# yongduosui/CAL

Hardware: AMD Instinct MI355X
Metric: graphs/sec (train step) on SPMotif b=0.9 batch=128 (higher is better)
Workload: dtype f32; 1 GPU; spmotif_b0.9_causalgcn_h128_l3_bs128; model=CausalGCN, batch_per_gpu=128, global_batch=128, hidden=128, layers=3, node_num=7, launch=graph(8 steps per graph launch, remainder 3), parallelism=dp1, resident_batches=8

## Files before the change

cal_amd/csrc/engine.hip:

```cpp
#include <string.h>
#include <hip/hip_ext.h>

#include <algorithm>
#include <type_traits>
#include <vector>

#include "engine_kernels.hpp"
#include "engine_readout.hpp"
#include "engine_gconv.hpp"
#include "engine_gconv_bwd.hpp"
#include "engine_ggat.hpp"
#include "engine_plan.hpp"
#include "engine_attbwd.hpp"
#include "engine_ro_step.hpp"
#include "engine_gin.hpp"
#include "engine_ggin.hpp"
#include "engine_feat.hpp"
#include "engine_gwide.hpp"
#include "engine_attwide.hpp"

namespace cal {

constexpr int MAX_LAYERS = 6;
constexpr int MAX_SLABS = 24;
constexpr int MAX_COMMITS = 64;

struct FinishArgs {
    SlabTask st[MAX_SLABS];
    CommitTask ct[MAX_COMMITS];
    int nst, nct;
    float* stats;
    float wc, wo, wco;
    float* tick;
    float* ticked;
    unsigned long long* perm_ctr;
    AdamArgs adam;
    AdamRange ar[MAX_ADAM_RANGES];
    int nar;
    double* bn0z; int bn0z_n;
    int* dirty;
    int* host_status;
    const int* status;
    int blk0[MAX_SLABS + MAX_COMMITS + MAX_ADAM_RANGES + 1];
};
__global__ void __launch_bounds__(256) k_finish(const FinishArgs fa, float* __restrict__ grad) {
    int task = 0;
    const int ntask = fa.nst + fa.nct + fa.nar;
    AdamArgs A = fa.adam;
    float adam_t = 0.f, adam_lr = 0.f;
    const bool flagged = fa.status && (fa.status[0] | fa.status[1]) != 0;
    if (fa.ticked && flagged && blockIdx.x == 0 && threadIdx.x == 0) fa.ticked[0] -= 1.f;
    if (A.on && flagged) A.on = 0;
    if (A.on) { adam_t = A.step[0]; adam_lr = A.lr[0]; }
    while (task + 1 < ntask && (int)blockIdx.x >= fa.blk0[task + 1]) ++task;
    const int bx = blockIdx.x - fa.blk0[task], nbx = fa.blk0[task + 1] - fa.blk0[task];
    if (fa.stats && blockIdx.x == 0 && threadIdx.x == 0)
        fa.stats[0] = fa.wc * fa.stats[1] + fa.wo * fa.stats[2] + fa.wco * fa.stats[3];
    if (fa.tick && !flagged && blockIdx.x == 0 && threadIdx.x == 0) fa.tick[0] += 1.f;
    if (fa.perm_ctr && blockIdx.x == 0 && threadIdx.x == 0) fa.perm_ctr[0] += 1;
    if (fa.bn0z && blockIdx.x == 0) {
        for (int i = threadIdx.x; i < fa.bn0z_n; i += 256) fa.bn0z[i] = 0.0;
        if (threadIdx.x == 0) *fa.dirty = 0;
    }
    if (fa.host_status && fa.status && blockIdx.x == 0 && threadIdx.x == 0)
        __hip_atomic_store(fa.host_status, fa.status[0] | fa.status[1], __ATOMIC_RELAXED, __HIP_MEMORY_SCOPE_SYSTEM);
    if (task < fa.nst) {
        const SlabTask t = fa.st[task];
        __shared__ float sred[256];
        const int el = threadIdx.x & 63, grp = threadIdx.x >> 6;
        const int per = (t.S + 3) / 4, z_lo = grp * per, z_hi = min(t.S, z_lo + per);
        for (int i0 = bx * 64; i0 < t.n; i0 += nbx * 64) {
            const int i = min(i0 + el, t.n - 1);
            float s0 = 0.f, s1 = 0.f;
            for (int z0 = z_lo; z0 < z_hi; z0 += 8) {
                float v[8];
#pragma unroll
                for (int u = 0; u < 8; ++u) v[u] = t.slabs[(size_t)max(min(z0 + u, z_hi - 1), 0) * t.n + i];
#pragma unroll
                for (int u = 0; u < 8; ++u) asm volatile("" : "+v"(v[u]));
#pragma unroll
                for (int u = 0; u < 8; u += 2) {
                    s0 += z0 + u < z_hi ? v[u] : 0.f;
                    s1 += z0 + u + 1 < z_hi ? v[u + 1] : 0.f;
                }
            }
            sred[threadIdx.x] = s0 + s1;
            __syncthreads();
            if (grp == 0 && i0 + el < t.n) {
                const float gsum = (sred[el] + sred[64 + el]) + (sred[128 + el] + sred[192 + el]);
                t.dst[i] = gsum;
                if (A.on) adam_update(A, (t.dst - grad) + i, gsum, adam_t, adam_lr);
            }
            __syncthreads();
        }
    } else if (task - fa.nst < fa.nct) {
        const CommitTask t = fa.ct[task - fa.nst];
        __shared__ double red[256];
        const int pl = threadIdx.x >> 4, cl = threadIdx.x & 15;
        for (int c0 = bx * 16; c0 < t.n; c0 += nbx * 16) {
            const int c = c0 + cl, cc = min(c, t.n - 1);
            double sacc = 0.0;
            for (int q0 = pl; q0 < t.P; q0 += 16 * 8) {
                double v[8];
#pragma unroll
                for (int u = 0; u < 8; ++u) v[u] = t.src[(size_t)max(min(q0 + 16 * u, t.P - 1), 0) * t.stride + cc];
#pragma unroll
                for (int u = 0; u < 8; ++u) asm volatile("" : "+v"(v[u]));
#pragma unroll
                for (int u = 0; u < 8; ++u) sacc += q0 + 16 * u < t.P ? v[u] : 0.0;
            }
            red[threadIdx.x] = sacc;
            __syncthreads();
            if (pl == 0 && c < t.n) {
                double tot = 0.0;
#pragma unroll
                for (int k = 0; k < 16; ++k) tot += red[k * 16 + cl];
                const float gv = t.scale * (float)tot;
                grad[t.dst + c] = gv;
                if (A.on) adam_update(A, t.dst + c, gv, adam_t, adam_lr);
            }
            __syncthreads();
        }
    } else if (A.on) {
        const AdamRange r = fa.ar[task - fa.nst - fa.nct];
        const int64_t i = r.begin + (int64_t)bx * 256 + threadIdx.x;
        if (i < r.end) adam_update(A, i, grad[i], adam_t, adam_lr);
    }
}

struct BNSlot { int gamma, beta; int width; float* rm; float* rv; int64_t* nbt; int arena; };

struct Engine {
    int F, H, C, L;
    int cat;
    int no_node_att, no_edge_att;
    int gin;
    int o_gin_w2[MAX_LAYERS], o_gin_b2[MAX_LAYERS];
    float *gagg, *gt1, *gy, *ones;
    float loop_w;
    float *P, *G, *M1, *M2, *step, *lr;
    int64_t nparam;
    float beta1, beta2, eps, wd;
    unsigned long long perm_seed; unsigned long long* perm_ctr;
    int64_t* perm_dev;
    P2PArgs p2p; int p2p_on;
    int num_cus;
    int* host_status;
    int* p2p_host_status;
    int p2p_max_polls;
    float grad_scale;
    int o_feat_w;
    int o_conv_w[MAX_LAYERS], o_conv_b[MAX_LAYERS];
    int o_eatt_w, o_eatt_b, o_natt_w, o_natt_b;
    int o_cw, o_cb, o_ow, o_ob;
    int o_fc1_w[3], o_fc1_b[3], o_fc2_w[3], o_fc2_b[3];
    BNSlot bn[MAX_LAYERS + 9];
    int nbn;
    int a_convb[MAX_LAYERS], a_cb, a_ob, a_dwn, a_dwe, a_db1, a_db2, a_sync, arena_n, bn_plane;
    char* ws; size_t ws_bytes;
    int64_t capN, capE, capB;
    float *h, *z, *zco, *hco, *anode, *pq, *att, *dis_unit, *dis_co, *pooled, *pcnt, *xco, *y1, *zl, *logp, *stats, *zpart;
    int adam_fused;
    int ro_rows;
    int striped;
    int fold_zero;
    int bn0_dirty_host;
    int gwide;
    int ro_step;
    float *dzl, *dyh1, *dy1, *dxh, *dpool, *dZco, *gn, *gself, *ddeg, *dl, *dzco, *dXhco, *dZ, *dzi, *dXh, *slabs;
    size_t slab_floats;
    double* arena;
    double* parts; size_t parts_doubles;
    hipStream_t side; hipEvent_t ev_fork[24], ev_join[24];
    int *rowptr_dst, *nbr_dst, *eid_dst, *rowptr_src, *nbr_src, *eid_src, *row32, *col32, *work, *status, *gptr, *iperm, *eptr;
    float* wslot;
    float* coef_src;
    float* coef;
    int max_nodes, max_edges;
    const int64_t *node_ptr, *edge_ptr;
    const int64_t* tile_gptr; int ntiles;
    int K; float gat_p, gat_slope;
    uint64_t gat_seed[MAX_LAYERS];
    unsigned long long* gat_ctr;
    int o_conv_att[MAX_LAYERS];
    float *gz, *gsc, *gws;
};

static size_t al(size_t n) { return (n + 63) / 64 * 64; }

}

using namespace cal;

namespace cal {
int gat_forward(const int32_t* rowptr_dst, const int32_t* nbr_dst, const int32_t* eid_dst, const float* z,
                const float* att, const float* bias, int relu, float slope, float p, uint64_t seed, const uint64_t* ctr,
                float* out, float* adst, float* asrc, float* mx, float* den, int64_t N, int64_t E,
                int64_t K, int64_t D, hipStream_t stream);
int gat_backward(const int32_t* rowptr_dst, const int32_t* nbr_dst, const int32_t* eid_dst,
                 const int32_t* rowptr_src, const int32_t* nbr_src, const int32_t* eid_src, const float* z,
                 const float* att, const float* adst, const float* asrc, const float* mx, const float* den,
                 const float* gout, float slope, float p, uint64_t seed, const uint64_t* ctr, float* dz, float* datt,
                 float* ws, int64_t N, int64_t E, int64_t K, int64_t D, hipStream_t stream, float* part_out, int* nparts);
int gat_datt_parts(int64_t N);
int plan_build(const int64_t* edge_index, int64_t E, int64_t N, int32_t* rowptr_dst, int32_t* nbr_dst, int32_t* eid_dst,
               int32_t* rowptr_src, int32_t* nbr_src, int32_t* eid_src, int32_t* row32, int32_t* col32, int32_t* work,
               int32_t* status, bool prezeroed, hipStream_t stream);
int plan_rank(int64_t E, int64_t N, const int32_t* rowptr_dst, int32_t* nbr_dst, int32_t* eid_dst, const int32_t* rowptr_src,
              int32_t* nbr_src, int32_t* eid_src, const int32_t* row32, const int32_t* col32, const int32_t* scratch,
              hipStream_t stream);
}

extern "C" int64_t cal_gat_bwd_ws(int64_t N, int64_t E, int64_t K, int64_t D);

CAL_EXPORT void* cal_engine_create(int64_t F, int64_t H, int64_t C, int64_t L) {
    if (H % 4 != 0 || H > 256 || H < 4 || L < 0 || L > MAX_LAYERS || F < 1 || C < 1 || C > 64) {
        set_error("cal_engine_create: unsupported shape (need hidden %% 4 == 0, hidden <= 256, layers <= %d, classes <= 64)", MAX_LAYERS);
        return nullptr;
    }
    Engine* e = new Engine();
    memset(e, 0, sizeof(Engine));
    if (hipHostMalloc((void**)&e->host_status, 64, hipHostMallocMapped | hipHostMallocCoherent) == hipSuccess) *e->host_status = 0;
    else { (void)hipGetLastError(); e->host_status = nullptr; }
    { const char* v = getenv("CAL_AMD_RO_STEP"); e->ro_step = !(v && v[0] == '0'); }
    { const char* v = getenv("CAL_AMD_RO_ROWS"); e->ro_rows = !(v && v[0] == '0'); }
    { const char* v = getenv("CAL_AMD_STRIPED"); e->striped = !(v && v[0] == '0'); }
    { const char* v = getenv("CAL_AMD_GWIDE"); e->gwide = !(v && v[0] == '0'); }
    { const char* v = getenv("CAL_AMD_FOLD_ZERO"); e->fold_zero = !(v && v[0] == '0'); }
    e->bn0_dirty_host = 1;
    {
        int dev = 0, cus = 0;
        if (hipGetDevice(&dev) != hipSuccess || hipDeviceGetAttribute(&cus, hipDeviceAttributeMultiprocessorCount, dev) != hipSuccess) cus = 0;
        if (cus < 3 * ((int)H / RO_CW) + 8) e->ro_step = 0;
        e->num_cus = cus > 0 ? cus : 256;
        if (cus < 3 * ((int)H / RO_CW) * RBK_MAXRB + 8) e->ro_rows = 0;
    }
    { const char* v = getenv("CAL_AMD_ADAM_FUSED"); e->adam_fused = !(v && v[0] == '0'); }
    e->F = (int)F; e->H = (int)H; e->C = (int)C; e->L = (int)L;
    e->loop_w = 1.f;
    e->grad_scale = 1.f;
    e->p2p_max_polls = 1 << 22;
    e->nbn = (int)L + 9;
    if (hipStreamCreateWithFlags(&e->side, hipStreamNonBlocking) != hipSuccess) { set_error("cal_engine_create: side stream"); delete e; return nullptr; }
    for (int i = 0; i < 24; ++i) {
        hipEventCreateWithFlags(&e->ev_fork[i], hipEventDisableTiming);
        hipEventCreateWithFlags(&e->ev_join[i], hipEventDisableTiming);
    }
    return e;
}

CAL_EXPORT void cal_engine_destroy(void* h) {
    Engine* e = (Engine*)h;
    if (!e) return;
    for (int i = 0; i < 24; ++i) { hipEventDestroy(e->ev_fork[i]); hipEventDestroy(e->ev_join[i]); }
    hipStreamDestroy(e->side);
    if (e->p2p_host_status) hipHostFree(e->p2p_host_status);
    if (e->host_status) hipHostFree(e->host_status);
    delete e;
}

CAL_EXPORT int64_t cal_engine_num_param_slots(void* h) { Engine* e = (Engine*)h; return 3 + (e->gin ? 6 : 4) * e->L + 12 + 24; }
CAL_EXPORT int64_t cal_engine_num_bn(void* h) { return ((Engine*)h)->nbn; }

CAL_EXPORT int cal_engine_bind(void* h, float* P, float* G, float* M1, float* M2, float* step, float* lr,
                               int64_t nparam, const int64_t* offs, const int64_t* bn_ptrs, float beta1, float beta2,
                               float eps, float weight_decay) {
    Engine* e = (Engine*)h;
    e->P = P; e->G = G; e->M1 = M1; e->M2 = M2; e->step = step; e->lr = lr; e->nparam = nparam;
    e->beta1 = beta1; e->beta2 = beta2; e->eps = eps; e->wd = weight_decay;
    const int L = e->L, H = e->H, F = e->F, C = e->C;
    int s = 0;
    int bn_g[MAX_LAYERS + 9], bn_b[MAX_LAYERS + 9], bn_w[MAX_LAYERS + 9];
    int k = 0;
    bn_g[k] = (int)offs[s++]; bn_b[k] = (int)offs[s++]; bn_w[k] = F; ++k;
    e->o_feat_w = (int)offs[s++];
    for (int i = 0; i < L; ++i) {
        bn_g[k] = (int)offs[s++]; bn_b[k] = (int)offs[s++]; bn_w[k] = H; ++k;
        e->o_conv_w[i] = (int)offs[s++]; e->o_conv_b[i] = (int)offs[s++];
        if (e->gin) { e->o_gin_w2[i] = (int)offs[s++]; e->o_gin_b2[i] = (int)offs[s++]; }
    }
    e->o_eatt_w = (int)offs[s++]; e->o_eatt_b = (int)offs[s++];
    e->o_natt_w = (int)offs[s++]; e->o_natt_b = (int)offs[s++];
    bn_g[k] = (int)offs[s++]; bn_b[k] = (int)offs[s++]; bn_w[k] = H; ++k;
    bn_g[k] = (int)offs[s++]; bn_b[k] = (int)offs[s++]; bn_w[k] = H; ++k;
    e->o_cw = (int)offs[s++]; e->o_cb = (int)offs[s++];
    e->o_ow = (int)offs[s++]; e->o_ob = (int)offs[s++];
    for (int hd = 0; hd < 3; ++hd) {
        bn_g[k] = (int)offs[s++]; bn_b[k] = (int)offs[s++]; bn_w[k] = (hd == 2 && e->cat) ? 2 * H : H; ++k;
        e->o_fc1_w[hd] = (int)offs[s++]; e->o_fc1_b[hd] = (int)offs[s++];
        bn_g[k] = (int)offs[s++]; bn_b[k] = (int)offs[s++]; bn_w[k] = H; ++k;
        e->o_fc2_w[hd] = (int)offs[s++]; e->o_fc2_b[hd] = (int)offs[s++];
    }
    int a = 0;
    for (int i = 0; i < L; ++i) { e->a_convb[i] = a; a += H; }
    e->a_cb = a; a += H;
    e->a_ob = a; a += H;
    e->a_dwn = a; a += H + 4;
    e->a_dwe = a; a += 2 * H + 4;
    e->a_db1 = a; a += 3 * H;
    e->a_db2 = a; a += (3 * C + 3) / 4 * 4;
    e->a_sync = a; a += (RBK_SYNC_INTS + 1) / 2 + 2;
    a = (a + 3) / 4 * 4;
    const int a_bn = a;
    for (int i = 0; i < e->nbn; ++i) {
        BNSlot& b = e->bn[i];
        b.gamma = bn_g[i]; b.beta = bn_b[i]; b.width = bn_w[i];
        b.rm = (float*)bn_ptrs[3 * i]; b.rv = (float*)bn_ptrs[3 * i + 1]; b.nbt = (int64_t*)bn_ptrs[3 * i + 2];
        b.arena = a;
        a += 4 * ((b.width + 3) / 4 * 4);
    }
    e->bn_plane = a - a_bn;
    a = a_bn + NSTRIPE * e->bn_plane;
    e->arena_n = a;
    (void)C;
    return 0;
}

static size_t engine_layout(Engine* e, int64_t N, int64_t E, int64_t B, bool assign) {
    const size_t H = e->H, C = e->C, L = e->L, F = e->F;
    size_t off = 0;
    auto F32 = [&](float*& p, size_t n) { if (assign) p = (float*)(e->ws) + off; off += al(n); };
    auto I32 = [&](int*& p, size_t n) { if (assign) p = (int*)(e->ws) + off; off += al(n); };
    F32(e->h, (L + 1) * N * H); F32(e->z, N * H); F32(e->zco, 2 * N * H); F32(e->hco, 2 * N * H);
    F32(e->anode, 2 * N); F32(e->pq, 4 * N); F32(e->att, 2 * E); F32(e->dis_unit, N); F32(e->dis_co, 2 * N);
    F32(e->pooled, 2 * B * H); F32(e->pcnt, 2 * B * H); F32(e->xco, 2 * B * H); F32(e->y1, 3 * B * H); F32(e->zl, 3 * B * C); F32(e->logp, 3 * B * C);
    F32(e->stats, 8); F32(e->zpart, 3 * ((H + 15) / 16) * B * C);
    F32(e->dzl, 3 * B * C); F32(e->dyh1, 3 * B * H); F32(e->dy1, 3 * B * H); F32(e->dxh, 4 * B * H); F32(e->dpool, 2 * B * H);
    F32(e->dZco, 2 * N * H); F32(e->gn, 4 * E); F32(e->gself, 4 * N); F32(e->ddeg, 2 * N); F32(e->dl, E);
    F32(e->dzco, 2 * N * H); F32(e->dXhco, 2 * N * H); F32(e->dZ, N * H); F32(e->dzi, (L > 0 ? L : 1) * N * H); F32(e->dXh, N * H);
    size_t slab = 0;
    auto slab_of = [&](size_t M, size_t Nn) {
        const size_t big = gemm_wres_grad((int)M, (int)Nn, (int)N) ? (size_t)gemm_wres_grad_splits((int)N, 1) * M * Nn
                         : gemm_big_grad((int)M, (int)Nn, (int)N) ? (size_t)gemm_big_grad_splits((int)N) * M * Nn : 0;
        return std::max<size_t>(std::max<size_t>(512 * 64 * 64, (size_t)B * M * Nn), big) + 2 * M * Nn;
    };
    slab += slab_of(F, H) + (L + 2) * slab_of(H, H) + 2 * slab_of(H, H) + slab_of(H, 2 * H) + 3 * slab_of(C, H);
    if (e->gin) slab += L * slab_of(H, H);
    if (e->K > 0) slab += L * (size_t)1024 * H;
    if (assign) e->slab_floats = slab;
    F32(e->slabs, slab);
    {
        float* tmp = nullptr;
        F32(tmp, 2 * (size_t)e->arena_n);
        if (assign) e->arena = (double*)tmp;
        size_t pcap = std::max<size_t>((N + 15) / 16 + 1, (std::min<int64_t>(N, 16384) + 7) / 8 + 1);
        size_t pd = pcap * (size_t)H * 2 * (3 * L + 20);
        F32(tmp, 2 * pd);
        if (assign) { e->parts = (double*)tmp; e->parts_doubles = pd; }
    }
    I32(e->rowptr_dst, N + 1); I32(e->nbr_dst, E); I32(e->eid_dst, E);
    I32(e->rowptr_src, N + 1); I32(e->nbr_src, E); I32(e->eid_src, E);
    I32(e->row32, E); I32(e->col32, E); I32(e->work, 4 * (N + 1) + 4 * E); I32(e->status, 4); I32(e->gptr, B + 1);
    I32(e->iperm, B);
    { int* tmp = nullptr; I32(tmp, 2 * B + 2); if (assign) e->perm_dev = (int64_t*)tmp; }
    I32(e->eptr, B + 1);
    F32(e->coef, 3 * E);
    F32(e->coef_src, E);
    F32(e->wslot, 2 * E);
    if (e->gin) {
        const size_t Lg = L > 0 ? L : 1;
        F32(e->gagg, Lg * N * H); F32(e->gt1, Lg * N * H); F32(e->gy, Lg * N * H); F32(e->ones, N);
    }
    if (e->K > 0) {
        const size_t K = e->K;
        F32(e->gz, (L > 0 ? L : 1) * N * H); F32(e->gsc, (L > 0 ? L : 1) * 4 * al(N * K));
        F32(e->gws, (size_t)cal_gat_bwd_ws(N, E, K, H / K));
    }
    return off * 4;
}

CAL_EXPORT int cal_engine_set_gat(void* h, int64_t heads, float p, float slope, const int64_t* att_offs,
                                  const uint64_t* seeds, void* ctr) {
    Engine* e = (Engine*)h;
    CAL_REQUIRE(heads > 0 && e->H % heads == 0, "heads must divide hidden");
    const int64_t D = e->H / heads;
    CAL_REQUIRE(D % 4 == 0 && ((D / 4) & (D / 4 - 1)) == 0, "head dim must be 4 * a power of two");
    CAL_REQUIRE(p >= 0.f && p < 1.f, "dropout p must be in [0,1)");
    e->K = (int)heads; e->gat_p = p; e->gat_slope = slope; e->gat_ctr = (unsigned long long*)ctr;
    for (int i = 0; i < e->L; ++i) { e->o_conv_att[i] = (int)att_offs[i]; e->gat_seed[i] = seeds[i]; }
    return 0;
}

CAL_EXPORT int64_t cal_engine_workspace_bytes(void* h, int64_t N, int64_t E, int64_t B) {
    return (int64_t)engine_layout((Engine*)h, N, E, B, false) + 256;
}

CAL_EXPORT int cal_engine_set_workspace(void* h, void* ws, int64_t bytes, int64_t capN, int64_t capE, int64_t capB) {
    Engine* e = (Engine*)h;
    CAL_REQUIRE(((uintptr_t)ws & 255) == 0, "workspace must be 256-byte aligned");
    e->ws = (char*)ws;
    e->capN = capN; e->capE = capE; e->capB = capB;
    size_t need = engine_layout(e, capN, capE, capB, true);
    CAL_REQUIRE((int64_t)need <= bytes, "workspace too small");
    e->ws_bytes = bytes;
    e->bn0_dirty_host = 1;
    return 0;
}

CAL_EXPORT int64_t cal_engine_buffer_offset(void* h, const char* name) {
    Engine* e = (Engine*)h;
    struct { const char* n; void* p; } tab[] = {
        {"h", e->h}, {"z", e->z}, {"zco", e->zco}, {"hco", e->hco}, {"anode", e->anode}, {"pq", e->pq}, {"att", e->att},
        {"dis_unit", e->dis_unit}, {"dis_co", e->dis_co}, {"pooled", e->pooled}, {"xco", e->xco}, {"y1", e->y1},
        {"zl", e->zl}, {"logp", e->logp}, {"stats", e->stats}, {"dzl", e->dzl}, {"dyh1", e->dyh1}, {"dy1", e->dy1},
        {"dxh", e->dxh}, {"dpool", e->dpool}, {"dZco", e->dZco}, {"gn", e->gn}, {"gself", e->gself}, {"ddeg", e->ddeg},
        {"dl", e->dl}, {"dzco", e->dzco}, {"dXhco", e->dXhco}, {"dZ", e->dZ}, {"dzi", e->dzi}, {"dXh", e->dXh},
        {"arena", e->arena}, {"gptr", e->gptr}, {"status", e->status}, {"eptr", e->eptr},
        {"gt1", e->gin ? e->gt1 : nullptr}, {"gy", e->gin ? e->gy : nullptr},
        {"rowptr_dst", e->rowptr_dst}, {"nbr_dst", e->nbr_dst}, {"eid_dst", e->eid_dst},
        {"rowptr_src", e->rowptr_src}, {"nbr_src", e->nbr_src}, {"eid_src", e->eid_src}, {"perm", e->perm_dev}, {"ones", e->ones},
    };
    for (auto& t : tab)
        if (!strcmp(t.n, name)) return t.p ? ((char*)t.p - e->ws) / 4 : -1;
    return -1;
}

namespace {

enum class Plan { Node, Graph256, Graph1024, Big };
enum class Conv { Node, Graph64, Graph128, Wide };
enum class Att { Node, Graph, Wide };
enum class FeatFwd { Gemm, Rows };
enum class FeatBwd { Gemm, Rows, Units };
enum class Readout { Gemm, FourKernel, OneLaunch, Rows };
struct Route {
    Plan plan;
    bool plan_stats;
    bool plan_coef;
    FeatFwd feat_fwd;
    FeatBwd feat_bwd;
    bool feat_chunks;
    Conv bb_fwd, bb_bwd;
    int gw_cols_bb, gw_cols_co;
    int nsplit_bb, nsplit_co;
    bool lean_bb, lean_co;
    Att att_fwd, att_bwd;
    int ag_split;
    Conv co_fwd, co_bwd;
    Readout ro;
    bool st_feat;
    bool st_bb;
    bool st_bb1;
    bool st_co;
    bool st_node;
};

struct Ctx {
    Engine* e;
    hipStream_t st;
    int N, B;
    const int64_t* batch;
    int T;
    int64_t E;
    int training;
    int rpb_n, rpb_b;
    int nfork;
    const int64_t* y; const int64_t* perm; float wc, wo, wco; int want_grad;
    int draw_perm;
    int tick_in_finish;
    int adam_in_finish;
    size_t parts_off;
    FinalArgs fin;
    Route r;
};

struct Deferred { double* p; int P; int stride; };
struct Bwd {
    FinishArgs fa;
    size_t slab_off;
    Deferred d_convb[MAX_LAYERS], d_gin_b1[MAX_LAYERS], d_cb, d_ob, d_dwn, d_dwe, d_bn0;
};

BNRef bnref(const Ctx& c, int k, int rows, int update) {
    const Engine* e = c.e;
    const BNSlot& b = e->bn[k];
    BNRef r;
    const int wp = (b.width + 3) / 4 * 4;
    r.sum = e->arena + b.arena; r.sq = e->arena + b.arena + wp;
    r.gamma = e->P + b.gamma; r.beta = e->P + b.beta;
    r.inv_n = 1.0 / (double)rows; r.eps = 1e-5f;
    r.run_mean = b.rm; r.run_var = b.rv; r.nbt = b.nbt;
    r.unbias = rows > 1 ? (float)rows / (float)(rows - 1) : 1.f;
    r.update = (update && c.training) ? 1 : 0;
    r.use_running = c.training ? 0 : 1;
    r.ss = e->bn_plane;
    return r;
}
double* bn_stsum(const Ctx& c, int k) { return c.e->arena + c.e->bn[k].arena; }
double* bn_stsq(const Ctx& c, int k) { return c.e->arena + c.e->bn[k].arena + (c.e->bn[k].width + 3) / 4 * 4; }
double* bn_dsum(const Ctx& c, int k) { return c.e->arena + c.e->bn[k].arena + 2 * ((c.e->bn[k].width + 3) / 4 * 4); }
double* bn_dprod(const Ctx& c, int k) { return c.e->arena + c.e->bn[k].arena + 3 * ((c.e->bn[k].width + 3) / 4 * 4); }

double* parts_alloc(Ctx& c, size_t n) {
    n = (n + 1) & ~(size_t)1;
    if (c.parts_off + n > c.e->parts_doubles) return nullptr;
    double* p = c.e->parts + c.parts_off;
    c.parts_off += n;
    return p;
}
void final_task(Ctx& c, const double* parts, int P, int stride, int n, double* dst) {
    c.fin.t[c.fin.nt++] = FinalTask{parts, P, stride, n, dst};
}
int flush_finals(Ctx& c) {
    if (c.fin.nt == 0) return 0;
    int nmax = 0;
    for (int i = 0; i < c.fin.nt; ++i) nmax = std::max(nmax, c.fin.t[i].n);
    hipLaunchKernelGGL(k_stats_final, dim3(cdiv(nmax, 8), c.fin.nt), dim3(256), 0, c.st, c.fin);
    c.fin.nt = 0;
    cal::g_last_launch = "k_stats_final";
    hipError_t e_ = hipGetLastError();
    if (e_ != hipSuccess) { set_error("k_stats_final: %s", hipGetErrorString(e_)); return 1; }
    return 0;
}
int spmm_rpb(int H, bool stats, int N = 1 << 30) {
    const int rows = 256 / group_for(H, 4);
    return stats && N > 16384 ? std::min(8, std::max(2, N / (rows * 4096))) * rows : rows;
}
Acc spmm_acc(Ctx& c, double* dst, int cols, int rpb) {
    const int P = cdiv(c.N, rpb);
    double* p = parts_alloc(c, (size_t)P * cols);
    if (!p) return Acc(dst);
    final_task(c, p, P, cols, cols, dst);
    return Acc(dst, p, cols);
}

Acc node_acc(Ctx& c, double* dst, int cols) {
    const int P = cdiv(c.N, c.rpb_n);
    if ((size_t)P * cols <= 4096) return Acc(dst);
    double* p = parts_alloc(c, (size_t)P * cols);
    if (!p) return Acc(dst);
    final_task(c, p, P, cols, cols, dst);
    return Acc(dst, p, cols);
}
bool use_ks(int M) { return M <= 2048; }
int fwd_gemm(Ctx& c, bool transB, const GemmArgs& a, int nbatch) {
    return use_ks(a.M) ? launch_gemm_ks(transB, a, nbatch, c.st) : launch_gemm(false, transB, a, nbatch, c.st);
}
void gemm_stats(Ctx& c, GemmProb& pr, int M, int N, double* d0, double* d1, bool dot, int K = 0, bool st = false) {
    if (dot) { pr.dot_sum = d0; pr.dot_prod = d1; } else { pr.st_sum = d0; pr.st_sq = d1; }
    if (st && (use_ks(M) || (!gemm_wres_rows(M, N, K) && !gemm_big_rows(M, K)))) { pr.st_ss = c.e->bn_plane; return; }
    const int P = use_ks(M) ? gemm_ks_row_tiles(M) : gemm_row_tiles(M, N, K);
    if ((size_t)P * N * 2 <= 4096) return;
    double* p = parts_alloc(c, (size_t)P * 2 * N);
    if (!p) return;
    pr.parts = p;
    final_task(c, p, P, 2 * N, N, d0);
    final_task(c, p + N, P, 2 * N, N, d1);
}

GemmArgs gemm_args(int M, int N, int K, bool transA, bool transB, int relu) {
    GemmArgs a;
    memset(&a, 0, sizeof(a));
    a.M = M; a.N = N; a.K = K;
    a.lda = transA ? M : K; a.ldb = transB ? K : N; a.ldc = N;
    a.relu = relu;
    gemm_set_split(a, 1);
    return a;
}

template <typename F>
int with_g(int H, F f) {
    int g = group_for(H, 4);
    if (g <= 8) return f(std::integral_constant<int, 8>());
    if (g == 16) return f(std::integral_constant<int, 16>());
    if (g == 32) return f(std::integral_constant<int, 32>());
    return f(std::integral_constant<int, 64>());
}

int pow2ceil(int v) { int p = 1; while (p < v) p <<= 1; return p; }

int launch_espmm(hipStream_t st, const CSR& csr, const SpmmBranch2& bb, int nbranch, int relu, float loop_w, int N, int H, int rpb);

#define RC(x) do { int rc_ = (x); if (rc_) return rc_; } while (0)
int no_parts() { set_error("engine: partial-row workspace exhausted"); return 2; }
int no_slabs() { set_error("engine: slab workspace exhausted"); return 2; }
float* slab_take(Ctx& c, Bwd& b, size_t need, float* dst, int n, int S) {
    if (b.slab_off + need > c.e->slab_floats || b.fa.nst >= MAX_SLABS) return nullptr;
    float* p = c.e->slabs + b.slab_off;
    b.fa.st[b.fa.nst++] = SlabTask{p, dst, n, S};
    b.slab_off += need;
    return p;
}
Acc defer(Ctx& c, Deferred& d, int P, int cols) {
    d.p = parts_alloc(c, (size_t)P * cols); d.P = P; d.stride = cols;
    return d.p ? Acc(nullptr, d.p, cols) : Acc();
}
int grad_slabs(Ctx& c, Bwd& b, GemmArgs& a, int nbatch, float** dst) {
    gemm_set_split(a, splitk_for(a.M, a.N, a.K, nbatch));
    for (int q = 0; q < nbatch; ++q) {
        a.p[q].C = a.nsplit > 1 ? slab_take(c, b, (size_t)a.nsplit * a.M * a.N, dst[q], a.M * a.N, a.nsplit) : dst[q];
        if (!a.p[q].C) return no_slabs();
    }
    return 0;
}
int grad_gemm(Ctx& c, Bwd& b, GemmArgs& a, int nbatch, float** dst) {
    RC(grad_slabs(c, b, a, nbatch, dst));
    hipStream_t s = c.st;
    constexpr bool kForkWeightGrads = false;
    if (kForkWeightGrads && c.nfork < 24) {
        hipEventRecord(c.e->ev_fork[c.nfork], c.st);
        hipStreamWaitEvent(c.e->side, c.e->ev_fork[c.nfork], 0);
        s = c.e->side;
    }
    int rc = launch_gemm(true, false, a, nbatch, s);
    if (s != c.st) { hipEventRecord(c.e->ev_join[c.nfork], s); c.nfork++; }
    return rc;
}
void join_side(Ctx& c) {
    for (int i = 0; i < c.nfork; ++i) hipStreamWaitEvent(c.st, c.e->ev_join[i], 0);
    c.nfork = 0;
}

int dual_gemm(Ctx& c, Bwd& b, GemmArgs& ax, int nbx, GemmArgs& aw, int nbw, float** dst) {
    if (use_ks(ax.M)) {
        RC(grad_gemm(c, b, aw, nbw, dst));
        return fwd_gemm(c, true, ax, nbx);
    }
    RC(grad_slabs(c, b, aw, nbw, dst));
    return launch_gemm_dual(ax, nbx, aw, nbw, c.st);
}

struct ProfRec { hipEvent_t e0, e1; int cls; double work; };
static bool g_prof_on = false;
static std::vector<ProfRec> g_prof;
struct ProfScope;
static ProfScope* g_prof_cur = nullptr;
struct ProfScope {
    hipStream_t st; bool on, single, used; ProfRec r;
    ProfScope(hipStream_t s, int cls, double work, bool single_kernel = false) : st(s), on(g_prof_on), single(single_kernel), used(false) {
        if (!on) return;
        r.cls = cls; r.work = work;
        hipEventCreate(&r.e0); hipEventCreate(&r.e1);
        if (single) g_prof_cur = this; else hipEventRecord(r.e0, st);
    }
    ~ProfScope() {
        if (!on) return;
        if (single) { g_prof_cur = nullptr; if (used) g_prof.push_back(r); }
        else { hipEventRecord(r.e1, st); g_prof.push_back(r); }
    }
};
#define PROF_LAUNCH(kernel, grid, block, shmem, stream, ...) do { \
        if (g_prof_cur) { hipExtLaunchKernelGGL(kernel, grid, block, shmem, stream, g_prof_cur->r.e0, g_prof_cur->r.e1, 0, __VA_ARGS__); g_prof_cur->used = true; } \
        else hipLaunchKernelGGL(kernel, grid, block, shmem, stream, __VA_ARGS__); } while (0)

int launch_espmm(hipStream_t st, const CSR& csr, const SpmmBranch2& bb, int nbranch, int relu, float loop_w, int N, int H, int rpb) {
    const bool wt = bb.b[0].w != nullptr, stt = bb.b[0].st_sum.on(), sd = bb.b[0].sd_z != nullptr;
    if (wt != (bb.b[nbranch - 1].w != nullptr) || stt != bb.b[nbranch - 1].st_sum.on() || sd != (bb.b[nbranch - 1].sd_z != nullptr) || rpb % 4 != 0 || H > 256) {
        set_error("k_espmm: branches differ in kind"); return 2;
    }
    const dim3 grid(cdiv(N, rpb), nbranch);
    if (sd) {
        if (!wt || stt) { set_error("k_espmm: the fused SDDMM is built for the weighted branches without statistics"); return 2; }
        const bool pb = bb.b[0].pb_g != nullptr;
        if (pb != (bb.b[nbranch - 1].pb_g != nullptr)) { set_error("k_espmm: branches differ in kind"); return 2; }
        return with_g(H, [&](auto g) {
            constexpr int G = decltype(g)::value;
            if (pb) PROF_LAUNCH((k_espmm<4, G, true, false, true, true>), grid, dim3(256), 0, st, csr, bb, relu, loop_w, N, H, rpb);
            else PROF_LAUNCH((k_espmm<4, G, true, false, true>), grid, dim3(256), 0, st, csr, bb, relu, loop_w, N, H, rpb);
            return 0;
        });
    }
    return with_g(H, [&](auto g) {
        constexpr int G = decltype(g)::value;
        if (wt && stt) PROF_LAUNCH((k_espmm<4, G, true, true>), grid, dim3(256), 0, st, csr, bb, relu, loop_w, N, H, rpb);
        else if (wt) PROF_LAUNCH((k_espmm<4, G, true, false>), grid, dim3(256), 0, st, csr, bb, relu, loop_w, N, H, rpb);
        else if (stt) PROF_LAUNCH((k_espmm<4, G, false, true>), grid, dim3(256), 0, st, csr, bb, relu, loop_w, N, H, rpb);
        else PROF_LAUNCH((k_espmm<4, G, false, false>), grid, dim3(256), 0, st, csr, bb, relu, loop_w, N, H, rpb);
        return 0;
    });
}

Acc graph_acc(Ctx& c, double* dst, int cols, bool st = false) {
    if (st) return Acc(dst, nullptr, c.e->bn_plane);
    double* p = parts_alloc(c, (size_t)c.T * cols);
    if (!p) return Acc(dst);
    final_task(c, p, c.T, cols, cols, dst);
    return Acc(dst, p, cols);
}
CSR csr_dst(const Ctx& c) { return CSR{c.e->rowptr_dst, c.e->nbr_dst, c.e->eid_dst, (int)c.E}; }
CSR csr_src(const Ctx& c) { return CSR{c.e->rowptr_src, c.e->nbr_src, c.e->eid_src, (int)c.E}; }

template <typename Args>
int bn_bwd_sums(Ctx& c, Args& a, int P, double* dsum, double* dprod, bool st) {
    if (st) { a.dacc_sum = dsum; a.dacc_prod = dprod; a.dacc_ss = c.e->bn_plane; return 0; }
    const int H = c.e->H;
    double* p = parts_alloc(c, (size_t)P * 2 * H);
    if (!p) return no_parts();
    a.dot_parts = p;
    final_task(c, p, P, 2 * H, H, dsum);
    final_task(c, p + H, P, 2 * H, H, dprod);
    return 0;
}

int gconv_bwd(Ctx& c, Bwd& b, GconvBwdBranch* gb, int nb, float** dst, double** dsum, double** dprod, bool st) {
    Engine* e = c.e;
    const bool co = nb == 2;
    const bool wide = (co ? c.r.co_bwd : c.r.bb_bwd) == Conv::Wide;
    const int nsplit = co ? c.r.nsplit_co : c.r.nsplit_bb;
    const bool lean = co ? c.r.lean_co : c.r.lean_bb;
    const int H = e->H, B = c.T, nsl = H / GC_N;
    const int np2 = nsplit == 4 ? 2 : 1;
    for (int k = 0; k < nb; ++k) {
        gb[k].batch = c.batch; gb[k].tile_gptr = e->ntiles > 0 ? e->tile_gptr : nullptr;
        gb[k].slab = slab_take(c, b, (size_t)B * H * H, dst[k], H * H, B);
        if (!gb[k].slab) return no_slabs();
        RC(bn_bwd_sums(c, gb[k], B * nsl * np2, dsum[k], dprod[k], st));
    }
    const GconvBwdBranch2 b2{{gb[0], gb[nb - 1]}};
    if (wide) {
        const CSR gs = csr_src(c);
        const dim3 gridw(B, nsl * nsplit, nb);
        if (co) PROF_LAUNCH((k_gw_bwd<true, 2>), gridw, dim3(GW_NT), 0, c.st, gs, e->gptr, e->eptr, b2, e->loop_w, c.N, H, H, nsplit, e->status);
        else if (gb[0].dout) PROF_LAUNCH((k_gw_bwd<false, 0>), gridw, dim3(GW_NT), 0, c.st, gs, e->gptr, e->eptr, b2, e->loop_w, c.N, H, H, nsplit, e->status);
        else PROF_LAUNCH((k_gw_bwd<false, 1>), gridw, dim3(GW_NT), 0, c.st, gs, e->gptr, e->eptr, b2, e->loop_w, c.N, H, H, nsplit, e->status);
        CAL_CHECK_LAUNCH("k_gw_bwd");
        return 0;
    }
    const CSR gd = csr_dst(c);
    const dim3 grid(B, nsl, nb);
    if (co && lean && e->ntiles > 0) PROF_LAUNCH((k_gconv_bwd<true, 2, true, true>), grid, dim3(GB_NT), 0, c.st, gd, e->gptr, e->eptr, b2, e->loop_w, c.N, H, H, e->status);
    else if (co && lean) PROF_LAUNCH((k_gconv_bwd<true, 2, false, true>), grid, dim3(GB_NT), 0, c.st, gd, e->gptr, e->eptr, b2, e->loop_w, c.N, H, H, e->status);
    else if (co && e->ntiles > 0) PROF_LAUNCH((k_gconv_bwd<true, 2, true>), grid, dim3(GB_NT), 0, c.st, gd, e->gptr, e->eptr, b2, e->loop_w, c.N, H, H, e->status);
    else if (co) PROF_LAUNCH((k_gconv_bwd<true, 2>), grid, dim3(GB_NT), 0, c.st, gd, e->gptr, e->eptr, b2, e->loop_w, c.N, H, H, e->status);
    else if (gb[0].dout && lean) PROF_LAUNCH((k_gconv_bwd<false, 0, false, true>), grid, dim3(GB_NT), 0, c.st, gd, e->gptr, e->eptr, b2, e->loop_w, c.N, H, H, e->status);
    else if (gb[0].dout) PROF_LAUNCH((k_gconv_bwd<false, 0>), grid, dim3(GB_NT), 0, c.st, gd, e->gptr, e->eptr, b2, e->loop_w, c.N, H, H, e->status);
    else if (lean) PROF_LAUNCH((k_gconv_bwd<false, 1, false, true>), grid, dim3(GB_NT), 0, c.st, gd, e->gptr, e->eptr, b2, e->loop_w, c.N, H, H, e->status);
    else PROF_LAUNCH((k_gconv_bwd<false, 1>), grid, dim3(GB_NT), 0, c.st, gd, e->gptr, e->eptr, b2, e->loop_w, c.N, H, H, e->status);
    CAL_CHECK_LAUNCH("k_gconv_bwd");
    return 0;
}

RoArgs make_ro(const Ctx& c) {
    Engine* e = c.e;
    const int L = e->L, H = e->H, C = e->C, B = c.B;
    RoArgs a;
    memset(&a, 0, sizeof(a));
    for (int hd = 0; hd < 3; ++hd) {
        RoHead& h = a.h[hd];
        const int k1 = L + 3 + 2 * hd, k2 = L + 4 + 2 * hd;
        h.W1 = e->P + e->o_fc1_w[hd]; h.b1 = e->P + e->o_fc1_b[hd];
        h.W2 = e->P + e->o_fc2_w[hd]; h.b2 = e->P + e->o_fc2_b[hd];
        h.bn1 = bnref(c, k1, B, 1); h.bn2 = bnref(c, k2, B, 1);
        h.st2_sum = bn_stsum(c, k2); h.st2_sq = bn_stsq(c, k2);
        h.d1_sum = bn_dsum(c, k1); h.d1_prod = bn_dprod(c, k1);
        h.d2_sum = bn_dsum(c, k2); h.d2_prod = bn_dprod(c, k2);
        h.db1 = e->arena + e->a_db1 + hd * H; h.db2 = e->arena + e->a_db2 + hd * C;
        h.gW1 = e->G + e->o_fc1_w[hd]; h.gW2 = e->G + e->o_fc2_w[hd];
    }
    a.pooled = e->pooled; a.perm = c.perm; a.iperm = e->iperm; a.xco = e->xco; a.y1 = e->y1;
    a.zl = e->zl; a.logp = e->logp; a.dzl = e->dzl; a.dy1 = e->dy1; a.dxin = e->dxh;
    a.rowloss = e->dyh1;
    a.y = c.y; a.stats = e->stats; a.B = B; a.H = H; a.C = C;
    a.wc = c.wc; a.wo = c.wo; a.wco = c.wco; a.training = c.training; a.want_grad = c.want_grad;
    return a;
}

static int g_stop_after = 0;
static int g_stage = 0;
static std::vector<const char*> g_stage_names;
#define STAGE() do { if (g_stop_after == 0) g_stage_names.push_back(cal::g_last_launch); \
                     if (g_stop_after > 0 && ++g_stage >= g_stop_after) return -12345; } while (0)

int gin_rows(Ctx& c, int mode, const GinRowArgs& ga) {
    const int N = c.N, H = c.e->H;
    hipStream_t st = c.st;
    return with_g(H, [&](auto g) {
        constexpr int G = decltype(g)::value;
        const dim3 grid(cdiv(N, c.rpb_n));
        if (mode == 0) hipLaunchKernelGGL((k_gin_rows<4, G, 0>), grid, dim3(256), 0, st, ga, N, H, c.rpb_n);
        else if (mode == 1) hipLaunchKernelGGL((k_gin_rows<4, G, 1>), grid, dim3(256), 0, st, ga, N, H, c.rpb_n);
        else if (mode == 2) hipLaunchKernelGGL((k_gin_rows<4, G, 2>), grid, dim3(256), 0, st, ga, N, H, c.rpb_n);
        else hipLaunchKernelGGL((k_gin_rows<4, G, 3>), grid, dim3(256), 0, st, ga, N, H, c.rpb_n);
        return 0;
    });
}

template <typename Fn>
int with_g_fp(int H, int F, Fn f) {
    return with_g(H, [&](auto g) {
        constexpr int G = decltype(g)::value;
        if constexpr (G >= FEAT_FMAX) {
            if (F <= 4) return f(g, std::integral_constant<int, 4>());
            if (F <= 8) return f(g, std::integral_constant<int, 8>());
            if (F <= 12) return f(g, std::integral_constant<int, 12>());
            return f(g, std::integral_constant<int, 16>());
        } else {
            set_error("feature row kernels: hidden width too small"); return 2;
        }
    });
}

int pool2_slices(int N, int B) { return std::max(1, std::min(32, N / std::max(1, B * 128))); }
int launch_pool2(hipStream_t st, const float* hc, const float* ho, const int* gptr, float* pooled, float* cnt, float* slices,
                 int N, int B, int H) {
    const int tc = std::min(256, pow2ceil(H / 4));
    const int S = pool2_slices(N, B);
    hipLaunchKernelGGL((k_pool2<4>), dim3(B, 2, S), dim3(256), 0, st, hc, ho, gptr, pooled, pooled + (size_t)B * H, H, tc, slices, cnt);
    CAL_CHECK_LAUNCH("k_pool2");
    if (S > 1) {
        hipLaunchKernelGGL(k_pool2_sum, dim3(cdiv(4 * (int64_t)B * H, 256)), dim3(256), 0, st, slices, S, 2 * (int64_t)B * H, pooled, cnt);
        CAL_CHECK_LAUNCH("k_pool2_sum");
    }
    return 0;
}
int launch_pool2(Ctx& c) {
    Engine* e = c.e;
    const size_t NH = (size_t)c.N * e->H;
    return launch_pool2(c.st, e->hco, e->hco + NH, e->gptr, e->pooled, e->pcnt, e->dZco, (int)c.N, (int)c.B, e->H);
}
int launch_pool_cnt(hipStream_t st, const float* hc, const float* ho, const int64_t* batch, float* cnt, int N, int B, int H, int rpb_n) {
    hipLaunchKernelGGL(k_zero_f32, dim3(cdiv(2 * (int64_t)B * H, 256)), dim3(256), 0, st, cnt, 2 * (int64_t)B * H);
    CAL_CHECK_LAUNCH("k_zero_f32");
    return with_g(H, [&](auto g) {
        constexpr int G = decltype(g)::value;
        hipLaunchKernelGGL((k_pool_cnt<4, G>), dim3(cdiv(N, rpb_n), 2), dim3(256), 0, st, hc, ho, batch, cnt, N, B, H, rpb_n);
        CAL_CHECK_LAUNCH("k_pool_cnt");
        return 0;
    });
}
int launch_pool_cnt(Ctx& c) {
    Engine* e = c.e;
    const size_t NH = (size_t)c.N * e->H;
    return launch_pool_cnt(c.st, e->hco, e->hco + NH, c.batch, e->pcnt, (int)c.N, (int)c.B, e->H, c.rpb_n);
}

Route make_route(const Ctx& c, bool want_grad) {
    const Engine* e = c.e;
    const int N = c.N, B = c.B, T = c.T, H = e->H, F = e->F, C = e->C, L = e->L, mn = e->max_nodes, me = e->max_edges;
    const bool gin = e->gin, gat = e->K > 0, gcn = !gin && !gat;
    Route r;
    memset(&r, 0, sizeof(r));
    const bool layout = e->node_ptr && e->edge_ptr && B > 0 && mn > 0;
    if (layout && mn <= GP_T2 && me <= GP_E2) r.plan = mn > GP_T || me > GP_E ? Plan::Graph1024 : Plan::Graph256;
    else if (layout && e->ntiles == 0 && mn <= GPB_T) r.plan = Plan::Big;
    else r.plan = Plan::Node;
    const bool graph_plan = r.plan == Plan::Graph256 || r.plan == Plan::Graph1024;
    r.plan_stats = r.plan != Plan::Node && c.training && F <= 64;
    const bool gc = mn > 0 && mn <= GC_T && me <= GC_E && H % GC_N == 0 && H <= GC_K && B > 0;
    const bool small = mn <= 64 && me <= gc_edge_cap(64);
    const bool gcb = gc && small && T <= 128 * 4;
    const bool gw = e->gwide && mn > GC_T && mn <= GW_T && me <= GW_E && H % GC_N == 0 && H <= GW_K && B > 0 && e->ntiles == 0 && gcn;
    r.plan_coef = graph_plan && gw;
    if (gin) {
        r.bb_fwd = gc && small && (!c.training || (gcb && me <= GB_E)) ? Conv::Graph64 : Conv::Node;
        r.bb_bwd = gcb && me <= GB_E ? Conv::Graph64 : Conv::Node;
    } else if (gat) {
        const int D = H / e->K;
        r.bb_fwd = gc && small && (D == 32 || D == 64) && me <= GG_E ? Conv::Graph64 : Conv::Node;
        r.bb_bwd = gcb && (D == 32 || D == 64) && me <= GGB_E ? Conv::Graph64 : Conv::Node;
    } else {
        r.bb_fwd = gw ? Conv::Wide : !gc ? Conv::Node : small ? Conv::Graph64 : Conv::Graph128;
        r.bb_bwd = gw ? Conv::Wide : gcb ? Conv::Graph64 : Conv::Node;
    }
    r.co_fwd = gw ? Conv::Wide : !gc ? Conv::Node : small ? Conv::Graph64 : Conv::Graph128;
    r.co_bwd = gw ? Conv::Wide : gcb ? Conv::Graph64 : Conv::Node;
    const int64_t w1 = (int64_t)T * (H / GC_N), w2 = 2 * w1;
    r.gw_cols_bb = w1 * 2 <= e->num_cus ? 32 : 64;
    r.gw_cols_co = w2 * 2 <= e->num_cus ? 32 : 64;
    auto nsplit = [&](int64_t w) { return !gw ? 1 : w * 4 <= e->num_cus ? 4 : w * 2 <= e->num_cus ? 2 : 1; };
    r.nsplit_bb = nsplit(w1); r.nsplit_co = nsplit(w2);
    const bool aw = gw && e->node_ptr && e->edge_ptr && mn <= AW_T && me <= AW_E && H <= 256 && T <= 512;
    const bool ag = gc && mn <= 4 * (512 / group_for(H, 4)) && me <= GP_E;
    r.att_fwd = aw && 3 * T >= e->num_cus ? Att::Wide : ag ? Att::Graph : Att::Node;
    r.att_bwd = aw ? Att::Wide : gcb && T <= 256 ? Att::Graph : Att::Node;
    r.ag_split = aw ? std::max(1, std::min(8, e->num_cus / std::max(T, 1))) : 2;
    r.lean_bb = w1 > e->num_cus;
    r.lean_co = w2 > e->num_cus && r.att_bwd == Att::Graph;
    const bool feat_rows = F <= FEAT_FMAX && N > 16384 && H % 4 == 0 && H <= 256 && group_for(H, 4) >= FEAT_FMAX;
    r.feat_fwd = feat_rows ? FeatFwd::Rows : FeatFwd::Gemm;
    r.feat_chunks = r.bb_bwd == Conv::Wide;
    const bool rides = H <= FB_H && (r.feat_chunks ? F <= FB_F : F <= FM_F);
    if (L == 0) r.feat_bwd = FeatBwd::Gemm;
    else if (r.bb_bwd != Conv::Node) r.feat_bwd = rides ? FeatBwd::Units : FeatBwd::Gemm;
    else r.feat_bwd = feat_rows && !gin ? FeatBwd::Rows : FeatBwd::Gemm;
    const bool st = e->striped && c.training;
    r.st_bb = st && r.bb_fwd == r.bb_bwd && r.bb_bwd != Conv::Node;
    r.st_bb1 = r.st_bb && (gin || gw || r.feat_bwd == FeatBwd::Units);
    r.st_node = st && gcn && !gc && N > 0 && N < 16384;
    r.st_feat = (r.st_bb && !gin && !gw && r.feat_bwd == FeatBwd::Units) || r.st_node;
    r.st_co = gw ? st : st && ag && gcb && T <= 256;
    const int B4 = (B + 15) & ~15;
    const bool ro = !e->cat && (size_t)B4 * (H + 4) <= (size_t)RO_LDS && B * H <= 16384 && H % RO_CW == 0 && B4 <= 256 && H <= 256 &&
                    B * C <= 2048 && C <= 64;
    const bool ro_rows = e->ro_rows && e->ro_step && !e->cat && B > RS_B && B <= RBK_MAXRB * RS_B && H <= RS_K && H % RO_CW == 0 &&
                         RS_B * C <= 2048 && C <= 64 && (size_t)3 * cdiv(B, RS_B) * ((size_t)H * H + (size_t)C * H) <= e->slab_floats;
    const bool step = want_grad && c.training;
    r.ro = ro && step && B <= RS_B && H <= RS_K && e->ro_step ? Readout::OneLaunch : ro_rows && step ? Readout::Rows
         : ro ? Readout::FourKernel : Readout::Gemm;
    return r;
}

int fwd_plan(Ctx& c, const float* x0, const int64_t* edge_index) {
    Engine* e = c.e;
    const Route& r = c.r;
    const int N = c.N, B = c.B, T = c.T, F = e->F;
    const int64_t E = c.E;
    hipStream_t st = c.st;
    const bool graph_plan = r.plan == Plan::Graph256 || r.plan == Plan::Graph1024;
    const bool fold = e->fold_zero && graph_plan && c.training && c.want_grad && !e->bn0_dirty_host && g_stop_after == 0;
    if (c.training) e->bn0_dirty_host = 1;
    if (!fold) {
        const int64_t ni = r.plan != Plan::Node ? 0 : 4 * ((int64_t)N + 1);
        hipLaunchKernelGGL(k_zero_f64, dim3(cdiv(std::max<int64_t>(e->arena_n, ni), 256) + (c.draw_perm ? cdiv(B, ZP_EPB) : 0)), dim3(256), 0, st,
                           e->arena, (int64_t)e->arena_n, e->work, ni, e->status, (e->K > 0 && c.training) ? e->gat_ctr : nullptr,
                           c.draw_perm ? e->perm_dev : nullptr, B, e->perm_seed, e->perm_ctr, c.adam_in_finish ? e->step : nullptr,
                           c.training ? e->status + 3 : nullptr);
        CAL_CHECK_LAUNCH("k_zero_f64"); STAGE();
    }
    if (graph_plan) {
        const bool wide = r.plan == Plan::Graph1024;
        auto kern = wide ? k_plan_graph<GP_T2, GP_E2, 1024> : k_plan_graph<GP_T, GP_E, 256>;
        const int nt = wide ? 1024 : 256;
        PlanFold pf;
        memset(&pf, 0, sizeof(pf));
        if (fold) {
            const int wp0 = (e->bn[0].width + 3) / 4 * 4;
            pf.on = 1; pf.arena = e->arena; pf.n = e->arena_n; pf.skip_lo = e->bn[0].arena; pf.skip_hi = e->bn[0].arena + 2 * wp0;
            pf.gat_tick = e->K > 0 ? e->gat_ctr : nullptr; pf.adam_step = c.adam_in_finish ? e->step : nullptr;
            pf.perm = c.draw_perm ? e->perm_dev : nullptr; pf.permB = B; pf.seed = e->perm_seed; pf.perm_ctr = e->perm_ctr;
            pf.dirty = e->status + 3;
        }
        hipLaunchKernelGGL(kern, dim3(T + ((fold && c.draw_perm) ? cdiv(B, nt / 4) : 0)), dim3(nt), 0, st, edge_index, E, N, T, e->node_ptr, e->edge_ptr,
                           c.batch, e->ntiles > 0 ? e->tile_gptr : nullptr, B, e->loop_w,
                           e->rowptr_dst, e->nbr_dst, e->eid_dst, e->rowptr_src, e->nbr_src, e->eid_src, e->row32, e->col32,
                           e->gptr, e->eptr, e->dis_unit, e->status, r.plan_stats ? x0 : nullptr, F, bn_stsum(c, 0), bn_stsq(c, 0),
                           r.plan_coef ? e->coef : nullptr, r.plan_coef ? e->coef_src : nullptr, pf);
        CAL_CHECK_LAUNCH("k_plan_graph"); STAGE();
    } else if (r.plan == Plan::Big) {
        int* scratch = e->work + 4 * ((size_t)e->capN + 1);
        hipLaunchKernelGGL(k_plan_big, dim3(B, 2), dim3(1024), 0, st, edge_index, E, N, B, e->node_ptr, e->edge_ptr, c.batch, e->loop_w,
                           e->rowptr_dst, e->rowptr_src, e->row32, e->col32, e->gptr, e->eptr, e->dis_unit, e->status, scratch,
                           r.plan_stats ? x0 : nullptr, F, bn_stsum(c, 0), bn_stsq(c, 0));
        CAL_CHECK_LAUNCH("k_plan_big"); STAGE();
        RC(plan_rank(E, N, e->rowptr_dst, e->nbr_dst, e->eid_dst, e->rowptr_src, e->nbr_src, e->eid_src, e->row32, e->col32, scratch, st)); STAGE();
    } else {
        RC(plan_build(edge_index, E, N, e->rowptr_dst, e->nbr_dst, e->eid_dst, e->rowptr_src, e->nbr_src, e->eid_src,
                      e->row32, e->col32, e->work, e->status, true, st)); STAGE();
        hipLaunchKernelGGL(k_gptr_dis, dim3(cdiv(N + 1, 256)), dim3(256), 0, st, c.batch, N, B, e->gptr, e->rowptr_src, e->loop_w,
                           e->dis_unit, e->status, e->rowptr_dst, e->eptr);
        CAL_CHECK_LAUNCH("k_gptr_dis"); STAGE();
    }
    return 0;
}

int fwd_feat(Ctx& c, const float* x0) {
    Engine* e = c.e;
    const int N = c.N, H = e->H, F = e->F, L = e->L;
    hipStream_t st = c.st;
    if (c.training && !c.r.plan_stats) {
        int tc = std::min(256, pow2ceil(F));
        const bool wide = (size_t)cdiv(N, 32) * F > 16384;
        int rpb = wide ? std::max(32, cdiv(N, 1024)) : std::max(128, cdiv(N, 256));
        const Acc a0 = wide ? spmm_acc(c, bn_stsum(c, 0), F, rpb) : Acc(bn_stsum(c, 0));
        const Acc a1 = wide ? spmm_acc(c, bn_stsq(c, 0), F, rpb) : Acc(bn_stsq(c, 0));
        hipLaunchKernelGGL(k_colstats, dim3(cdiv(N, rpb)), dim3(256), 0, st, x0, N, F, tc, rpb, a0, a1);
        CAL_CHECK_LAUNCH("k_colstats"); STAGE();
        if (wide) { RC(flush_finals(c)); STAGE(); }
    }
    if (c.r.feat_fwd == FeatFwd::Rows) {
        FeatFwdArgs fw;
        fw.x0 = x0; fw.W = e->P + e->o_feat_w; fw.out = e->h; fw.bn0 = bnref(c, 0, N, 1);
        if (c.training && L > 0 && !e->gin) { fw.st_sum = node_acc(c, bn_stsum(c, 1), H); fw.st_sq = node_acc(c, bn_stsq(c, 1), H); }
        RC(with_g_fp(H, F, [&](auto g, auto fp) {
            hipLaunchKernelGGL((k_feat_fwd_rows<decltype(g)::value, decltype(fp)::value>), dim3(cdiv(N, c.rpb_n)), dim3(256), 0, st, fw, N, H, F, c.rpb_n);
            return 0;
        }));
        CAL_CHECK_LAUNCH("k_feat_fwd_rows"); STAGE();
    } else {
        GemmArgs a = gemm_args(N, H, F, false, false, 1);
        a.p[0].A = x0; a.p[0].B = e->P + e->o_feat_w; a.p[0].C = e->h;
        a.p[0].xa.has_bn = 1; a.p[0].xa.bn = bnref(c, 0, N, 1);
        if (c.training && L > 0 && !e->gin) gemm_stats(c, a.p[0], N, H, bn_stsum(c, 1), bn_stsq(c, 1), false, F, c.r.st_feat);
        RC(fwd_gemm(c, false, a, 1)); STAGE();
    }
    RC(flush_finals(c)); STAGE();
    return 0;
}

int fwd_backbone(Ctx& c) {
    Engine* e = c.e;
    const Route& r = c.r;
    const int N = c.N, T = c.T, H = e->H, L = e->L;
    const int64_t E = c.E;
    hipStream_t st = c.st;
    const size_t NH = (size_t)N * H;
    const CSR gd = csr_dst(c);
    for (int i = 1; i <= L; ++i) {
        const float* hin = e->h + (size_t)(i - 1) * NH;
        float* hout = e->h + (size_t)i * NH;
        if (e->gin && r.bb_fwd == Conv::Graph64) {
            float* t1 = e->gt1 + (size_t)(i - 1) * NH;
            GginFwdArgs ga;
            memset(&ga, 0, sizeof(ga));
            ga.x = hin; ga.W = e->P + e->o_conv_w[i - 1]; ga.bias = e->P + e->o_conv_b[i - 1]; ga.out = t1;
            if (c.training) { ga.st_sum = graph_acc(c, bn_stsum(c, i), H, r.st_bb); ga.st_sq = graph_acc(c, bn_stsq(c, i), H, r.st_bb); }
            {
                ProfScope ps(st, 9, 2.0 * N * H * H + 2.0 * (double)(E + N) * H, true);
                PROF_LAUNCH((k_ggin_fwd<1>), dim3(T, H / GC_N), dim3(512), 0, st, gd, e->gptr, e->eptr, ga, H, H, e->status);
            }
            CAL_CHECK_LAUNCH("k_ggin_fwd<1>"); STAGE();
            RC(flush_finals(c)); STAGE();
            memset(&ga, 0, sizeof(ga));
            ga.x = t1; ga.W = e->P + e->o_gin_w2[i - 1]; ga.bias = e->P + e->o_gin_b2[i - 1]; ga.out = hout;
            ga.bn = bnref(c, i, N, 1);
            hipLaunchKernelGGL((k_ggin_fwd<2>), dim3(T, H / GC_N), dim3(512), 0, st, gd, e->gptr, e->eptr, ga, H, H, e->status);
            CAL_CHECK_LAUNCH("k_ggin_fwd<2>"); STAGE();
        } else if (e->gin) {
            float* agg = e->gagg + (size_t)(i - 1) * NH;
            float* t1 = e->gt1 + (size_t)(i - 1) * NH;
            float* yy = e->gy + (size_t)(i - 1) * NH;
            {
                SpmmBranch br{hin, agg, nullptr, nullptr, e->ones, Acc(), Acc(), nullptr, nullptr, nullptr};
                RC(launch_espmm(st, gd, SpmmBranch2{{br, br}}, 1, 0, 1.0f, N, H, spmm_rpb(H, false)));
                CAL_CHECK_LAUNCH("k_espmm(gin)"); STAGE();
            }
            {
                GemmArgs a = gemm_args(N, H, H, false, true, 0);
                a.p[0].A = agg; a.p[0].B = e->P + e->o_conv_w[i - 1]; a.p[0].bias = e->P + e->o_conv_b[i - 1]; a.p[0].C = t1;
                if (c.training) gemm_stats(c, a.p[0], N, H, bn_stsum(c, i), bn_stsq(c, i), false, H);
                RC(fwd_gemm(c, true, a, 1)); STAGE();
                RC(flush_finals(c)); STAGE();
            }
            {
                GinRowArgs ga;
                memset(&ga, 0, sizeof(ga));
                ga.a = t1; ga.out = yy; ga.bn = bnref(c, i, N, 1);
                RC(gin_rows(c, 0, ga));
                CAL_CHECK_LAUNCH("k_gin_bn_relu"); STAGE();
            }
            {
                GemmArgs a = gemm_args(N, H, H, false, true, 1);
                a.p[0].A = yy; a.p[0].B = e->P + e->o_gin_w2[i - 1]; a.p[0].bias = e->P + e->o_gin_b2[i - 1]; a.p[0].C = hout;
                RC(fwd_gemm(c, true, a, 1)); STAGE();
            }
        } else if (e->K > 0) {
            const int K = e->K, D = H / K;
            float* zi = e->gz + (size_t)(i - 1) * NH;
            const size_t nk = al((size_t)e->capN * K);
            float* sc = e->gsc + (size_t)(i - 1) * 4 * nk;
            if (r.bb_fwd == Conv::Graph64) {
                GgatArgs ga;
                memset(&ga, 0, sizeof(ga));
                ga.x = hin; ga.W = e->P + e->o_conv_w[i - 1]; ga.bias = e->P + e->o_conv_b[i - 1];
                ga.att = e->P + e->o_conv_att[i - 1]; ga.bn = bnref(c, i, N, 1); ga.out = hout; ga.z = zi;
                ga.adst = sc; ga.asrc = sc + nk; ga.mx = sc + 2 * nk; ga.den = sc + 3 * nk;
                if (c.training && i < L) { ga.st_sum = graph_acc(c, bn_stsum(c, i + 1), H, r.st_bb); ga.st_sq = graph_acc(c, bn_stsq(c, i + 1), H, r.st_bb); }
                ga.heads = K; ga.D = D; ga.slope = e->gat_slope; ga.p = c.training ? e->gat_p : 0.f;
                ga.seed = e->gat_seed[i - 1]; ga.ctr = (const uint64_t*)e->gat_ctr; ga.E = E;
                {
                    ProfScope ps(st, 7, 2.0 * N * H * H + 2.0 * (double)(E + N) * H, true);
                    PROF_LAUNCH(k_ggat_fwd, dim3(T, H / GC_N), dim3(256), 0, st, gd, e->gptr, e->eptr, ga, H, H, e->status);
                }
                CAL_CHECK_LAUNCH("k_ggat_fwd"); STAGE();
                RC(flush_finals(c)); STAGE();
                continue;
            }
            GemmArgs a = gemm_args(N, H, H, false, false, 0);
            a.p[0].A = hin; a.p[0].B = e->P + e->o_conv_w[i - 1]; a.p[0].C = zi;
            a.p[0].xa.has_bn = 1; a.p[0].xa.bn = bnref(c, i, N, 1);
            { ProfScope ps(st, 0, 2.0 * N * H * H); RC(fwd_gemm(c, false, a, 1)); } STAGE();
            {
                ProfScope ps(st, 5, 2.0 * N * H * 4 + (double)(E + N) * (8 + 12.0 * K) + (N + 1) * 4.0);
                RC(gat_forward(e->rowptr_dst, e->nbr_dst, e->eid_dst, zi, e->P + e->o_conv_att[i - 1], e->P + e->o_conv_b[i - 1], 1,
                               e->gat_slope, c.training ? e->gat_p : 0.f, e->gat_seed[i - 1], (const uint64_t*)e->gat_ctr, hout,
                               sc, sc + nk, sc + 2 * nk, sc + 3 * nk, N, E, K, D, st));
            }
            STAGE();
            if (c.training && i < L) {
                int tc = std::min(256, pow2ceil(H));
                int rpb = std::max(32, cdiv(N, 1024));
                if (H == 256 && aligned16(hout))
                    hipLaunchKernelGGL(k_colstats4, dim3(cdiv(N, rpb)), dim3(256), 0, st, hout, N, rpb, Acc(bn_stsum(c, i + 1)), Acc(bn_stsq(c, i + 1)));
                else
                    hipLaunchKernelGGL(k_colstats, dim3(cdiv(N, rpb)), dim3(256), 0, st, hout, N, H, tc, rpb, Acc(bn_stsum(c, i + 1)), Acc(bn_stsq(c, i + 1)));
                CAL_CHECK_LAUNCH("k_colstats"); STAGE();
            }
        } else if (r.bb_fwd != Conv::Node) {
            GconvBranch gb;
            memset(&gb, 0, sizeof(gb));
            gb.x = hin; gb.W = e->P + e->o_conv_w[i - 1]; gb.bias = e->P + e->o_conv_b[i - 1];
            gb.dis = e->dis_unit; gb.bn = bnref(c, i, N, 1); gb.out = hout;
            if (i == 1 && !r.plan_coef) gb.coef_out = e->coef; else gb.coef_in = e->coef;
            if (c.training && i < L) { gb.st_sum = graph_acc(c, bn_stsum(c, i + 1), H, r.st_bb); gb.st_sq = graph_acc(c, bn_stsq(c, i + 1), H, r.st_bb); }
            const GconvBranch2 b2{{gb, gb}};
            {
                ProfScope ps(st, 2, 2.0 * N * H * H + 2.0 * (double)(E + N) * H, true);
                if (r.bb_fwd == Conv::Wide && r.gw_cols_bb == 32) PROF_LAUNCH((k_gw_fwd<false, 32>), dim3(T, H / 32, 1), dim3(GW_NT), 0, st, gd, e->gptr, e->eptr, b2, 1, e->loop_w, H, H, e->status);
                else if (r.bb_fwd == Conv::Wide) PROF_LAUNCH((k_gw_fwd<false, 64>), dim3(T, H / GC_N, 1), dim3(GW_NT), 0, st, gd, e->gptr, e->eptr, b2, 1, e->loop_w, H, H, e->status);
                else if (r.bb_fwd == Conv::Graph64) PROF_LAUNCH((k_gconv_fwd<false, 64, 512>), dim3(T, H / GC_N, 1), dim3(512), 0, st, gd, e->gptr, e->eptr, b2, 1, e->loop_w, H, H, e->status);
                else PROF_LAUNCH((k_gconv_fwd<false, GC_T>), dim3(T, H / GC_N, 1), dim3(256), 0, st, gd, e->gptr, e->eptr, b2, 1, e->loop_w, H, H, e->status);
            }
            CAL_CHECK_LAUNCH(r.bb_fwd == Conv::Wide ? "k_gw_fwd" : "k_gconv_fwd"); STAGE();
            RC(flush_finals(c)); STAGE();
        } else {
            GemmArgs a = gemm_args(N, H, H, false, false, 0);
            a.p[0].A = hin; a.p[0].B = e->P + e->o_conv_w[i - 1]; a.p[0].C = e->z;
            a.p[0].xa.has_bn = 1; a.p[0].xa.bn = bnref(c, i, N, 1);
            { ProfScope ps(st, 0, 2.0 * N * H * H); RC(fwd_gemm(c, false, a, 1)); } STAGE();
            SpmmBranch br{e->z, hout, e->P + e->o_conv_b[i - 1], nullptr, e->dis_unit, Acc(), Acc(), nullptr, nullptr, nullptr};
            const bool wst = c.training && i < L;
            const int rpb = spmm_rpb(H, wst, N);
            if (wst) { br.st_sum = spmm_acc(c, bn_stsum(c, i + 1), H, rpb); br.st_sq = spmm_acc(c, bn_stsq(c, i + 1), H, rpb); }
            {
                ProfScope ps(st, 1, 2.0 * N * H * 4 + (double)(E + N) * 8 + (N + 1) * 4.0, true);
                RC(launch_espmm(st, gd, SpmmBranch2{{br, br}}, 1, 1, e->loop_w, N, H, rpb));
            }
            CAL_CHECK_LAUNCH("k_espmm"); STAGE();
            RC(flush_finals(c)); STAGE();
        }
    }
    return 0;
}

int fwd_att(Ctx& c) {
    Engine* e = c.e;
    const Route& r = c.r;
    const int N = c.N, H = e->H, L = e->L;
    const int64_t E = c.E;
    hipStream_t st = c.st;
    const float* x = e->h + (size_t)L * N * H;
    const CSR gs = csr_src(c);
    if (r.att_fwd != Att::Node) {
        const bool wide = r.att_fwd == Att::Wide;
        const Acc a0 = graph_acc(c, bn_stsum(c, L + 1), H, r.st_co), a1 = graph_acc(c, bn_stsq(c, L + 1), H, r.st_co);
        const Acc a2 = graph_acc(c, bn_stsum(c, L + 2), H, r.st_co), a3 = graph_acc(c, bn_stsq(c, L + 2), H, r.st_co);
        auto launch = [&](auto kernel_of) {
            return with_g(H, [&](auto g) {
                hipLaunchKernelGGL(kernel_of(g), dim3(c.T), dim3(512), 0, st, e->gptr, gs, x, e->P + e->o_natt_w, e->P + e->o_natt_b,
                                   e->P + e->o_eatt_w, e->P + e->o_eatt_b, e->anode, e->pq, e->att, e->dis_co, e->dis_co + N, a0, a1, a2, a3,
                                   e->loop_w, H, E, e->status, e->no_node_att ? 0.f : 1.f, e->no_edge_att ? 0.f : 1.f, e->eptr);
                return 0;
            });
        };
        if (wide) RC(launch([](auto g) { return k_att_fwd_wide<4, decltype(g)::value>; }));
        else RC(launch([](auto g) { return k_att_fwd_graph<4, decltype(g)::value>; }));
        CAL_CHECK_LAUNCH(wide ? "k_att_fwd_wide" : "k_att_fwd_graph"); STAGE();
        RC(flush_finals(c)); STAGE();
        return 0;
    }
    const Acc a0 = node_acc(c, bn_stsum(c, L + 1), H), a1 = node_acc(c, bn_stsq(c, L + 1), H);
    const Acc a2 = node_acc(c, bn_stsum(c, L + 2), H), a3 = node_acc(c, bn_stsq(c, L + 2), H);
    RC(with_g(H, [&](auto g) {
        constexpr int G = decltype(g)::value;
        hipLaunchKernelGGL((k_node_att_fwd<4, G>), dim3(cdiv(N, c.rpb_n)), dim3(256), 0, st, x, e->P + e->o_natt_w,
                           e->P + e->o_natt_b, e->P + e->o_eatt_w, e->anode, e->pq, a0, a1, a2, a3, N, H, c.rpb_n, e->no_node_att ? 0.f : 1.f);
        return 0;
    }));
    CAL_CHECK_LAUNCH("k_node_att_fwd"); STAGE();
    RC(flush_finals(c)); STAGE();
    hipLaunchKernelGGL(k_edge_att_deg, dim3(cdiv(N, 32)), dim3(256), 0, st, gs, e->pq, e->P + e->o_eatt_b, e->att, e->dis_co,
                       e->dis_co + N, e->loop_w, N, E, e->no_edge_att ? 0.f : 1.f);
    CAL_CHECK_LAUNCH("k_edge_att_deg"); STAGE();
    return 0;
}

int fwd_co(Ctx& c) {
    Engine* e = c.e;
    const Route& r = c.r;
    const int N = c.N, B = c.B, T = c.T, H = e->H, L = e->L;
    const int64_t E = c.E;
    hipStream_t st = c.st;
    const size_t NH = (size_t)N * H;
    const float* x = e->h + (size_t)L * NH;
    const CSR gd = csr_dst(c);
    if (r.co_fwd != Conv::Node) {
        const bool wide = r.co_fwd == Conv::Wide;
        const int64_t* tgp = e->ntiles > 0 ? e->tile_gptr : nullptr;
        GconvBranch gb[2];
        memset(gb, 0, sizeof(gb));
        for (int k = 0; k < 2; ++k) {
            gb[k].x = x; gb[k].W = e->P + (k ? e->o_ow : e->o_cw); gb[k].bias = e->P + (k ? e->o_ob : e->o_cb);
            gb[k].ew = e->att + (size_t)k * E; gb[k].dis = e->dis_co + (size_t)k * N;
            gb[k].rs = e->anode + k; gb[k].rs_stride = 2; gb[k].bn = bnref(c, L + 1 + k, N, 1);
            gb[k].out = e->hco + (size_t)k * NH; gb[k].z = e->zco + (size_t)k * NH; gb[k].pooled = e->pooled + (size_t)k * B * H;
            if (wide) continue;
            gb[k].coef_out = e->coef + (size_t)(1 + k) * E;
            gb[k].w_out = e->wslot + (size_t)k * E;
            gb[k].batch = c.batch; gb[k].tile_gptr = tgp;
        }
        const GconvBranch2 b2{{gb[0], gb[1]}};
        if (tgp) hipLaunchKernelGGL((k_gconv_fwd<true, 64, 512, true>), dim3(T, H / GC_N, 2), dim3(512), 0, st, gd, e->gptr, e->eptr, b2, 1, e->loop_w, H, H, e->status);
        else if (r.co_fwd == Conv::Graph64) hipLaunchKernelGGL((k_gconv_fwd<true, 64, 512>), dim3(T, H / GC_N, 2), dim3(512), 0, st, gd, e->gptr, e->eptr, b2, 1, e->loop_w, H, H, e->status);
        else if (r.co_fwd == Conv::Graph128) hipLaunchKernelGGL((k_gconv_fwd<true, GC_T>), dim3(T, H / GC_N, 2), dim3(256), 0, st, gd, e->gptr, e->eptr, b2, 1, e->loop_w, H, H, e->status);
        else if (r.gw_cols_co == 32) hipLaunchKernelGGL((k_gw_fwd<true, 32>), dim3(T, H / 32, 2), dim3(GW_NT), 0, st, gd, e->gptr, e->eptr, b2, 1, e->loop_w, H, H, e->status);
        else hipLaunchKernelGGL((k_gw_fwd<true, 64>), dim3(T, H / GC_N, 2), dim3(GW_NT), 0, st, gd, e->gptr, e->eptr, b2, 1, e->loop_w, H, H, e->status);
        CAL_CHECK_LAUNCH(wide ? "k_gw_fwd(co)" : "k_gconv_fwd(co)"); STAGE();
        return 0;
    }
    GemmArgs a = gemm_args(N, H, H, false, false, 0);
    for (int k = 0; k < 2; ++k) {
        a.p[k].A = x; a.p[k].B = e->P + (k ? e->o_ow : e->o_cw); a.p[k].C = e->zco + (size_t)k * NH;
        a.p[k].xa.rs = e->anode + k; a.p[k].xa.rs_stride = 2;
        a.p[k].xa.has_bn = 1; a.p[k].xa.bn = bnref(c, L + 1 + k, N, 1);
    }
    RC(fwd_gemm(c, false, a, 2)); STAGE();
    SpmmBranch b0{e->zco, e->hco, e->P + e->o_cb, e->att, e->dis_co, Acc(), Acc(), nullptr, nullptr, nullptr};
    SpmmBranch b1{e->zco + NH, e->hco + NH, e->P + e->o_ob, e->att + E, e->dis_co + N, Acc(), Acc(), nullptr, nullptr, nullptr};
    RC(launch_espmm(st, gd, SpmmBranch2{{b0, b1}}, 2, 1, e->loop_w, N, H, spmm_rpb(H, false)));
    CAL_CHECK_LAUNCH("k_espmm(co)"); STAGE();
    RC(launch_pool2(c)); STAGE();
    return 0;
}

int fwd_readout(Ctx& c) {
    Engine* e = c.e;
    const int B = c.B, H = e->H, C = e->C, L = e->L;
    hipStream_t st = c.st;
    if (c.r.ro == Readout::OneLaunch || c.r.ro == Readout::Rows) {
        RoStepArgs sa;
        memset(&sa, 0, sizeof(sa));
        sa.a = make_ro(c); sa.zpart = e->zpart; sa.sync = reinterpret_cast<int*>(e->arena + e->a_sync); sa.status = e->status;
        if (c.r.ro == Readout::OneLaunch) {
            hipLaunchKernelGGL(k_ro_step<false>, dim3(3, H / RO_CW), dim3(256), 0, st, sa);
        } else {
            const int nrb = cdiv(B, RS_B), nch = H / RO_CW;
            sa.nrb = nrb;
            sa.xch = parts_alloc(c, (size_t)3 * nch * RBK_XCH);
            if (!sa.xch) return no_parts();
            sa.gw1_slab = e->slabs; sa.gw2_slab = e->slabs + (size_t)3 * nrb * H * H;
            hipLaunchKernelGGL(k_ro_step<true>, dim3(3, nch, nrb), dim3(256), 0, st, sa);
        }
        CAL_CHECK_LAUNCH("k_ro_step"); STAGE();
        return 0;
    }
    if (c.r.ro == Readout::FourKernel) {
        const RoArgs ra = make_ro(c);
        hipLaunchKernelGGL(k_ro_fwd_a, dim3(3, H / RO_CW), dim3(256), 0, st, ra);
        CAL_CHECK_LAUNCH("k_ro_fwd_a"); STAGE();
        hipLaunchKernelGGL(k_ro_fwd_b, dim3(3, cdiv(B, RO_RB)), dim3(256), 0, st, ra);
        CAL_CHECK_LAUNCH("k_ro_fwd_b"); STAGE();
        if (!c.want_grad) {
            hipLaunchKernelGGL(k_ro_loss, dim3(3), dim3(256), 0, st, ra);
            CAL_CHECK_LAUNCH("k_ro_loss");
        }
        return 0;
    }
    const int bn_fc1 = L + 3, bn_fc2 = L + 4;
    {
        int tc = std::min(256, pow2ceil(H));
        hipLaunchKernelGGL(k_readout_prep, dim3(cdiv(B, c.rpb_b)), dim3(256), 0, st, e->pooled, c.perm, e->iperm, e->xco, B, H, tc,
                           c.rpb_b, bn_stsum(c, bn_fc1), bn_stsq(c, bn_fc1), bn_stsum(c, bn_fc1 + 2), bn_stsq(c, bn_fc1 + 2),
                           bn_stsum(c, bn_fc1 + 4), bn_stsq(c, bn_fc1 + 4), e->cat);
        CAL_CHECK_LAUNCH("k_readout_prep"); STAGE();
    }
    const float* xin[3] = {e->pooled, e->pooled + (size_t)B * H, e->xco};
    const int Wco = e->cat ? 2 * H : H;
    {
        auto fc1 = [&](int hd0, int nh, int Kin) -> int {
            GemmArgs a = gemm_args(B, H, Kin, false, true, 1);
            for (int q = 0; q < nh; ++q) {
                const int hd = hd0 + q;
                a.p[q].A = xin[hd]; a.p[q].B = e->P + e->o_fc1_w[hd]; a.p[q].bias = e->P + e->o_fc1_b[hd];
                a.p[q].C = e->y1 + (size_t)hd * B * H;
                a.p[q].xa.has_bn = 1; a.p[q].xa.bn = bnref(c, bn_fc1 + 2 * hd, B, 1);
                if (c.training) gemm_stats(c, a.p[q], B, H, bn_stsum(c, bn_fc2 + 2 * hd), bn_stsq(c, bn_fc2 + 2 * hd), false);
            }
            return fwd_gemm(c, true, a, nh);
        };
        if (e->cat) { RC(fc1(0, 2, H)); STAGE(); RC(fc1(2, 1, Wco)); STAGE(); }
        else { RC(fc1(0, 3, H)); STAGE(); }
        RC(flush_finals(c)); STAGE();
    }
    {
        GemmArgs a = gemm_args(B, C, H, false, true, 0);
        for (int hd = 0; hd < 3; ++hd) {
            a.p[hd].A = e->y1 + (size_t)hd * B * H; a.p[hd].B = e->P + e->o_fc2_w[hd]; a.p[hd].bias = e->P + e->o_fc2_b[hd];
            a.p[hd].C = e->zl + (size_t)hd * B * C;
            a.p[hd].xa.has_bn = 1; a.p[hd].xa.bn = bnref(c, bn_fc2 + 2 * hd, B, 1);
        }
        RC(fwd_gemm(c, true, a, 3)); STAGE();
    }
    if (B > 256) hipLaunchKernelGGL(k_loss<1024>, dim3(1), dim3(1024), 0, st, e->zl, c.y, e->logp, e->dzl, e->stats, e->arena + e->a_db2, B, C, c.wc, c.wo,
                                    c.wco, c.want_grad);
    else hipLaunchKernelGGL(k_loss<256>, dim3(1), dim3(256), 0, st, e->zl, c.y, e->logp, e->dzl, e->stats, e->arena + e->a_db2, B, C, c.wc, c.wo,
                            c.wco, c.want_grad);
    CAL_CHECK_LAUNCH("k_loss"); STAGE();
    return 0;
}

int engine_forward(Ctx& c, const float* x0, const int64_t* edge_index) {
    RC(fwd_plan(c, x0, edge_index));
    RC(fwd_feat(c, x0));
    RC(fwd_backbone(c));
    RC(fwd_att(c));
    RC(fwd_co(c));
    return fwd_readout(c);
}

int bwd_readout(Ctx& c, Bwd& b) {
    Engine* e = c.e;
    const int B = c.B, H = e->H, C = e->C, L = e->L;
    const size_t BH = (size_t)B * H;
    hipStream_t st = c.st;
    FinishArgs& fa = b.fa;
    if (c.r.ro == Readout::Rows) {
        const int nrb = cdiv(B, RS_B);
        for (int hd = 0; hd < 3; ++hd) {
            fa.st[fa.nst++] = SlabTask{e->slabs + (size_t)hd * nrb * H * H, e->G + e->o_fc1_w[hd], H * H, nrb};
            fa.st[fa.nst++] = SlabTask{e->slabs + (size_t)3 * nrb * H * H + (size_t)hd * nrb * C * H, e->G + e->o_fc2_w[hd], C * H, nrb};
        }
        b.slab_off = (size_t)3 * nrb * ((size_t)H * H + (size_t)C * H);
        b.slab_off = (b.slab_off + 63) & ~(size_t)63;
    }
    if (c.r.ro != Readout::Gemm) {
        if (c.r.ro == Readout::FourKernel) {
            const RoArgs ra = make_ro(c);
            hipLaunchKernelGGL(k_ro_bwd_a, dim3(3, H / RO_CW), dim3(256), 0, st, ra);
            CAL_CHECK_LAUNCH("k_ro_bwd_a"); STAGE();
            hipLaunchKernelGGL(k_ro_bwd_b, dim3(3, H / RO_CW), dim3(256), 0, st, ra);
            CAL_CHECK_LAUNCH("k_ro_bwd_b"); STAGE();
        }
        fa.stats = e->stats; fa.wc = c.wc; fa.wo = c.wo; fa.wco = c.wco;
        return 0;
    }
    const int bn_fc1 = L + 3, bn_fc2 = L + 4;
    const float* xin[3] = {e->pooled, e->pooled + BH, e->xco};
    {
        GemmArgs a = gemm_args(C, H, B, true, false, 0);
        float* dst[3];
        for (int hd = 0; hd < 3; ++hd) {
            a.p[hd].A = e->dzl + (size_t)hd * B * C; a.p[hd].B = e->y1 + hd * BH;
            a.p[hd].xb.has_bn = 1; a.p[hd].xb.bn = bnref(c, bn_fc2 + 2 * hd, B, 0);
            dst[hd] = e->G + e->o_fc2_w[hd];
        }
        RC(grad_gemm(c, b, a, 3, dst)); STAGE();
    }
    {
        GemmArgs a = gemm_args(B, H, C, false, false, 0);
        for (int hd = 0; hd < 3; ++hd) {
            a.p[hd].A = e->dzl + (size_t)hd * B * C; a.p[hd].B = e->P + e->o_fc2_w[hd]; a.p[hd].C = e->dyh1 + hd * BH;
            a.p[hd].aux = e->y1 + hd * BH; a.p[hd].has_aux = 1; a.p[hd].aux_bn = bnref(c, bn_fc2 + 2 * hd, B, 0);
            gemm_stats(c, a.p[hd], B, H, bn_dsum(c, bn_fc2 + 2 * hd), bn_dprod(c, bn_fc2 + 2 * hd), true);
        }
        RC(fwd_gemm(c, false, a, 3)); STAGE();
        RC(flush_finals(c)); STAGE();
    }
    {
        BnBwdProb p[3];
        for (int hd = 0; hd < 3; ++hd)
            p[hd] = BnBwdProb{e->dyh1 + hd * BH, e->y1 + hd * BH, e->dy1 + hd * BH, bnref(c, bn_fc2 + 2 * hd, B, 0),
                              bn_dsum(c, bn_fc2 + 2 * hd), bn_dprod(c, bn_fc2 + 2 * hd), e->arena + e->a_db1 + hd * H};
        RC(with_g(H, [&](auto g) {
            constexpr int G = decltype(g)::value;
            hipLaunchKernelGGL((k_bn_bwd<4, G>), dim3(cdiv(B, c.rpb_b), 3), dim3(256), 0, st, BnBwdProb3{{p[0], p[1], p[2]}}, 1, B, H, c.rpb_b);
            return 0;
        }));
        CAL_CHECK_LAUNCH("k_bn_bwd(readout)"); STAGE();
    }
    const int Wco = e->cat ? 2 * H : H;
    float* const dxh_hd[3] = {e->dxh, e->dxh + BH, e->dxh + 2 * BH};
    {
        auto r4 = [&](int hd0, int nh, int Kin) -> int {
            GemmArgs a = gemm_args(H, Kin, B, true, false, 0);
            float* dst[3];
            for (int q = 0; q < nh; ++q) {
                const int hd = hd0 + q;
                a.p[q].A = e->dy1 + hd * BH; a.p[q].B = xin[hd];
                a.p[q].xb.has_bn = 1; a.p[q].xb.bn = bnref(c, bn_fc1 + 2 * hd, B, 0);
                dst[q] = e->G + e->o_fc1_w[hd];
            }
            return grad_gemm(c, b, a, nh, dst);
        };
        if (e->cat) { RC(r4(0, 2, H)); STAGE(); RC(r4(2, 1, Wco)); STAGE(); }
        else { RC(r4(0, 3, H)); STAGE(); }
    }
    {
        auto r5 = [&](int hd0, int nh, int Kin) -> int {
            GemmArgs a = gemm_args(B, Kin, H, false, false, 0);
            for (int q = 0; q < nh; ++q) {
                const int hd = hd0 + q;
                a.p[q].A = e->dy1 + hd * BH; a.p[q].B = e->P + e->o_fc1_w[hd]; a.p[q].C = dxh_hd[hd];
                a.p[q].aux = xin[hd]; a.p[q].has_aux = 1; a.p[q].aux_bn = bnref(c, bn_fc1 + 2 * hd, B, 0);
                gemm_stats(c, a.p[q], B, Kin, bn_dsum(c, bn_fc1 + 2 * hd), bn_dprod(c, bn_fc1 + 2 * hd), true);
            }
            return fwd_gemm(c, false, a, nh);
        };
        if (e->cat) { RC(r5(0, 2, H)); STAGE(); RC(r5(2, 1, Wco)); STAGE(); }
        else { RC(r5(0, 3, H)); STAGE(); }
        RC(flush_finals(c)); STAGE();
    }
    BnIn in[3];
    for (int hd = 0; hd < 3; ++hd)
        in[hd] = BnIn{dxh_hd[hd], xin[hd], bnref(c, bn_fc1 + 2 * hd, B, 0), bn_dsum(c, bn_fc1 + 2 * hd), bn_dprod(c, bn_fc1 + 2 * hd)};
    hipLaunchKernelGGL(k_readout_bwd_tail, dim3(cdiv((int64_t)BH, 256)), dim3(256), 0, st, in[0], in[1], in[2], e->iperm, e->dpool, B, H, e->cat);
    CAL_CHECK_LAUNCH("k_readout_bwd_tail"); STAGE();
    return 0;
}

int norm_bwd(Ctx& c, const float* gn2, const float* gself2) {
    Engine* e = c.e;
    const int N = c.N;
    const int64_t E = c.E;
    hipLaunchKernelGGL(k_normbwd_node2, dim3(cdiv(N, 32), 2), dim3(256), 0, c.st, csr_src(c), csr_dst(c), e->att, e->dis_co, e->gn, e->gself,
                       e->ddeg, e->loop_w, N, E, gn2, gself2);
    CAL_CHECK_LAUNCH("k_normbwd_node2"); STAGE();
    if (E > 0) {
        hipLaunchKernelGGL(k_normbwd_edge, dim3(cdiv(E, 256)), dim3(256), 0, c.st, e->row32, e->col32, e->att, e->dis_co, e->gn, e->ddeg,
                           e->dl, N, E, gn2, e->no_edge_att ? 0.f : 1.f);
        CAL_CHECK_LAUNCH("k_normbwd_edge"); STAGE();
    }
    return 0;
}

int bwd_co(Ctx& c, Bwd& b) {
    Engine* e = c.e;
    const Route& r = c.r;
    const int N = c.N, B = c.B, T = c.T, H = e->H, L = e->L;
    const int64_t E = c.E;
    hipStream_t st = c.st;
    const size_t NH = (size_t)N * H;
    const bool ro = r.ro != Readout::Gemm;
    const float* x = e->h + (size_t)L * NH;
    if (r.co_bwd != Conv::Node) {
        GconvBwdBranch gb[2];
        memset(gb, 0, sizeof(gb));
        float* dst[2]; double* dsum[2]; double* dprod[2];
        for (int k = 0; k < 2; ++k) {
            gb[k].x = x; gb[k].W = e->P + (k ? e->o_ow : e->o_cw);
            gb[k].y = e->hco + (size_t)k * NH; gb[k].z = e->zco + (size_t)k * NH;
            if (ro) { gb[k].gp0 = e->dxh + (size_t)k * B * H; gb[k].gp1 = e->dxh + (size_t)2 * B * H; gb[k].iperm = k == 0 ? e->iperm : nullptr; }
            else gb[k].gp0 = e->dpool + (size_t)k * B * H;
            gb[k].gn = e->gn + (size_t)k * E; gb[k].gself = e->gself + (size_t)k * N;
            gb[k].gn_stride = 2 * (size_t)E; gb[k].gself_stride = 2 * (size_t)N;
            Deferred& db = k ? b.d_ob : b.d_cb;
            if (!defer(c, db, T, H).on()) return no_parts();
            gb[k].bias_parts = db.p;
            gb[k].ew = e->att + (size_t)k * E; gb[k].dis = e->dis_co + (size_t)k * N;
            gb[k].rs = e->anode + k; gb[k].rs_stride = 2; gb[k].bn = bnref(c, L + 1 + k, N, 0);
            gb[k].dxp0 = e->dXhco + (size_t)k * NH; gb[k].dxp1 = e->dzco + (size_t)k * NH;
            gb[k].coef_in = r.co_bwd == Conv::Wide ? nullptr : e->coef + (size_t)(1 + k) * E;
            gb[k].gn_slot = r.att_bwd == Att::Graph ? 1 : 0;
            dst[k] = e->G + (k ? e->o_ow : e->o_cw); dsum[k] = bn_dsum(c, L + 1 + k); dprod[k] = bn_dprod(c, L + 1 + k);
        }
        RC(gconv_bwd(c, b, gb, 2, dst, dsum, dprod, r.st_co)); STAGE();
        RC(flush_finals(c)); STAGE();
        if (r.att_bwd == Att::Node) {
            const bool two = H > GC_N;
            RC(norm_bwd(c, two ? e->gn + 2 * (size_t)E : nullptr, two ? e->gself + 2 * (size_t)N : nullptr));
        }
        return 0;
    }
    if (r.co_fwd != Conv::Node) { RC(launch_pool_cnt(c)); STAGE(); }
    b.d_cb.p = parts_alloc(c, (size_t)B * H); b.d_cb.P = B; b.d_cb.stride = H;
    b.d_ob.p = parts_alloc(c, (size_t)B * H); b.d_ob.P = B; b.d_ob.stride = H;
    if (!b.d_cb.p || !b.d_ob.p) return no_parts();
    hipLaunchKernelGGL(k_pool_bias_grad, dim3(B, 2), dim3(256), 0, st, e->pcnt, ro ? e->dxh : e->dpool, ro ? e->dxh + 2 * (size_t)B * H : nullptr,
                       e->iperm, e->dpool, b.d_cb.p, b.d_ob.p, B, H);
    CAL_CHECK_LAUNCH("k_pool_bias_grad"); STAGE();
    {
        SpmmBranch b0{e->hco, e->dzco, nullptr, e->att, e->dis_co, Acc(), Acc(), nullptr, nullptr, nullptr};
        SpmmBranch b1{e->hco + NH, e->dzco + NH, nullptr, e->att + E, e->dis_co + N, Acc(), Acc(), nullptr, nullptr, nullptr};
        b0.sd_z = e->zco; b0.sd_gn = e->gn; b0.sd_gself = e->gself;
        b1.sd_z = e->zco + NH; b1.sd_gn = e->gn + E; b1.sd_gself = e->gself + N;
        b0.pb_g = e->dpool; b0.pb_batch = c.batch;
        b1.pb_g = e->dpool + (size_t)B * H; b1.pb_batch = c.batch;
        RC(launch_espmm(st, csr_src(c), SpmmBranch2{{b0, b1}}, 2, 0, e->loop_w, N, H, spmm_rpb(H, false)));
        CAL_CHECK_LAUNCH("k_espmm(co,T)"); STAGE();
        RC(norm_bwd(c, nullptr, nullptr));
    }
    GemmArgs aw = gemm_args(H, H, N, true, false, 0);
    float* dst[2];
    for (int k = 0; k < 2; ++k) {
        aw.p[k].A = x; aw.p[k].B = e->dzco + (size_t)k * NH;
        aw.p[k].xa.rs = e->anode + k; aw.p[k].xa.rs_stride = 2;
        aw.p[k].xa.has_bn = 1; aw.p[k].xa.bn = bnref(c, L + 1 + k, N, 0);
        dst[k] = e->G + (k ? e->o_ow : e->o_cw);
    }
    GemmArgs a = gemm_args(N, H, H, false, true, 0);
    for (int k = 0; k < 2; ++k) {
        a.p[k].A = e->dzco + (size_t)k * NH; a.p[k].B = e->P + (k ? e->o_ow : e->o_cw); a.p[k].C = e->dXhco + (size_t)k * NH;
        a.p[k].aux = x; a.p[k].aux_rs = e->anode + k; a.p[k].aux_rs_stride = 2; a.p[k].has_aux = 1;
        a.p[k].aux_bn = bnref(c, L + 1 + k, N, 0);
        gemm_stats(c, a.p[k], N, H, bn_dsum(c, L + 1 + k), bn_dprod(c, L + 1 + k), true, H, r.st_node);
    }
    RC(dual_gemm(c, b, a, 2, aw, 2, dst)); STAGE();
    RC(flush_finals(c)); STAGE();
    return 0;
}

int bwd_att(Ctx& c, Bwd& b) {
    Engine* e = c.e;
    const Route& r = c.r;
    const int N = c.N, T = c.T, H = e->H, L = e->L;
    const int64_t E = c.E;
    hipStream_t st = c.st;
    const size_t NH = (size_t)N * H;
    AttBwdArgs aa;
    aa.x = e->h + (size_t)L * NH; aa.anode = e->anode; aa.dxhc = e->dXhco; aa.dxho = e->dXhco + NH;
    const bool two = r.co_bwd != Conv::Node && H > GC_N;
    aa.dxhc2 = two ? e->dzco : nullptr; aa.dxho2 = two ? e->dzco + NH : nullptr;
    aa.bnc = bnref(c, L + 1, N, 0); aa.bno = bnref(c, L + 2, N, 0);
    aa.dsc = bn_dsum(c, L + 1); aa.dpc = bn_dprod(c, L + 1); aa.dso = bn_dsum(c, L + 2); aa.dpo = bn_dprod(c, L + 2); aa.dss = e->bn_plane;
    aa.Wn = e->P + e->o_natt_w; aa.We = e->P + e->o_eatt_w; aa.dl = e->dl;
    aa.fnode = e->no_node_att ? 0.f : 1.f; aa.fedge = e->no_edge_att ? 0.f : 1.f;
    aa.gs = csr_src(c); aa.gd = csr_dst(c); aa.dZ = e->dZ;
    const int P = r.att_bwd == Att::Node ? cdiv(N, c.rpb_n) : r.ag_split * T;
    aa.dbias = L > 0 ? defer(c, b.d_convb[L - 1], P, H) : Acc();
    aa.dWn = defer(c, b.d_dwn, P, H + 4); aa.dWe = defer(c, b.d_dwe, P, 2 * H + 4);
    if (!aa.dWn.on() || !aa.dWe.on()) return no_parts();
    if (r.att_bwd == Att::Wide) {
        AttBwdWideArgs ag;
        ag.a = aa; ag.gptr = e->gptr; ag.eptr = e->eptr; ag.row32 = e->row32; ag.col32 = e->col32; ag.att = e->att; ag.dis = e->dis_co;
        ag.gn = e->gn; ag.gn2 = two ? e->gn + 2 * (size_t)E : nullptr;
        ag.gself = e->gself; ag.gself2 = two ? e->gself + 2 * (size_t)N : nullptr;
        ag.loop_w = e->loop_w; ag.E = E; ag.N = N; ag.status = e->status;
        RC(with_g(H, [&](auto g) {
            constexpr int G = decltype(g)::value;
            hipLaunchKernelGGL((k_att_bwd_wide<4, G>), dim3(r.ag_split * T), dim3(512), 0, st, ag, 1, H, r.ag_split);
            return 0;
        }));
        CAL_CHECK_LAUNCH("k_att_bwd_wide"); STAGE();
    } else if (r.att_bwd == Att::Graph) {
        AttBwdGraphArgs ag;
        ag.a = aa; ag.gptr = e->gptr; ag.eptr = e->eptr; ag.att = e->wslot; ag.dis = e->dis_co;
        ag.gn = e->gn; ag.gn2 = two ? e->gn + 2 * (size_t)E : nullptr;
        ag.gself = e->gself; ag.gself2 = two ? e->gself + 2 * (size_t)N : nullptr;
        ag.loop_w = e->loop_w; ag.E = E; ag.N = N; ag.status = e->status;
        RC(with_g(H, [&](auto g) {
            constexpr int G = decltype(g)::value;
            hipLaunchKernelGGL((k_att_bwd_graph<4, G>), dim3(r.ag_split * T), dim3(512), 0, st, ag, 1, H, r.ag_split);
            return 0;
        }));
        CAL_CHECK_LAUNCH("k_att_bwd_graph"); STAGE();
    } else {
        const bool sr = r.st_node || r.st_co;
        RC(with_g(H, [&](auto g) {
            constexpr int G = decltype(g)::value;
            if (sr) hipLaunchKernelGGL((k_att_bwd<4, G, true>), dim3(cdiv(N, c.rpb_n)), dim3(256), 0, st, aa, 1, N, H, c.rpb_n);
            else hipLaunchKernelGGL((k_att_bwd<4, G>), dim3(cdiv(N, c.rpb_n)), dim3(256), 0, st, aa, 1, N, H, c.rpb_n);
            return 0;
        }));
        CAL_CHECK_LAUNCH("k_att_bwd"); STAGE();
    }
    return 0;
}

int bwd_feat_units(Ctx& c, Bwd& b, const float* x0, const float* p0, const float* p1, bool nobn) {
    Engine* e = c.e;
    const int N = c.N, H = e->H, F = e->F;
    hipStream_t st = c.st;
    FeatBwdArgs fb;
    memset(&fb, 0, sizeof(fb));
    fb.dy0 = p0; fb.dy1 = p1; fb.y = e->h;
    if (!nobn) { fb.ubn = bnref(c, 1, N, 0); fb.udot_sum = bn_dsum(c, 1); fb.udot_prod = bn_dprod(c, 1); }
    fb.x0 = x0; fb.W = e->P + e->o_feat_w; fb.bn0 = bnref(c, 0, N, 0);
    const bool chunks = c.r.feat_chunks;
    const int U = chunks ? cdiv(N, FB_T) : c.T;
    fb.slab = slab_take(c, b, (size_t)U * F * H, e->G + e->o_feat_w, F * H, U);
    if (!fb.slab) return no_slabs();
    b.d_bn0.p = parts_alloc(c, (size_t)U * 2 * F); b.d_bn0.P = U; b.d_bn0.stride = 2 * F;
    if (!b.d_bn0.p) return no_parts();
    fb.parts = b.d_bn0.p;
    const dim3 grid(U), blk(GB_NT);
    if (F <= FB_F && !nobn) {
        if (F <= 16) hipLaunchKernelGGL(k_feat_bwd<16>, grid, blk, 0, st, chunks ? (const int*)nullptr : (const int*)e->gptr, fb, H, F, e->status, N);
        else hipLaunchKernelGGL(k_feat_bwd<FB_F>, grid, blk, 0, st, chunks ? (const int*)nullptr : (const int*)e->gptr, fb, H, F, e->status, N);
    } else if (F <= 64) {
        hipLaunchKernelGGL((k_feat_bwd_mma<8, true>), grid, blk, 0, st, e->gptr, fb, H, F, e->status);
    } else {
        if (nobn) hipLaunchKernelGGL((k_feat_bwd_mma<20, true>), grid, blk, 0, st, e->gptr, fb, H, F, e->status);
        else hipLaunchKernelGGL((k_feat_bwd_mma<20, false>), grid, blk, 0, st, e->gptr, fb, H, F, e->status);
    }
    CAL_CHECK_LAUNCH("k_feat_bwd");
    return 0;
}

int bwd_backbone(Ctx& c, Bwd& b, const float* x0) {
    Engine* e = c.e;
    const Route& r = c.r;
    const int N = c.N, T = c.T, H = e->H, F = e->F, L = e->L;
    const int64_t E = c.E;
    hipStream_t st = c.st;
    const size_t NH = (size_t)N * H;
    const CSR gd = csr_dst(c), gs = csr_src(c);
    const int PN = cdiv(N, c.rpb_n);
    const bool units = r.feat_bwd == FeatBwd::Units, two = H > GC_N;
    for (int i = L; i >= 1; --i) {
        float* dzi = e->dzi + (size_t)(i - 1) * NH;
        const float* hin = e->h + (size_t)(i - 1) * NH;
        const bool st_i = i > 1 ? r.st_bb : r.st_bb1;
        if (e->gin && r.bb_bwd == Conv::Graph64) {
            const int nsl = H / GC_N;
            float* c0 = e->dXh; float* c1 = e->gy + (size_t)(i - 1) * NH;
            float* d0 = e->z; float* d1 = e->gagg + (size_t)(i - 1) * NH;
            const float* t1 = e->gt1 + (size_t)(i - 1) * NH;
            if (b.slab_off + 2 * (size_t)T * H * H > e->slab_floats || b.fa.nst + 2 > MAX_SLABS) return no_slabs();
            GginBwdArgs ga;
            memset(&ga, 0, sizeof(ga));
            if (i == L) ga.dout = e->dZ;
            else {
                ga.dy0 = e->z; ga.dy1 = two ? e->gagg + (size_t)i * NH : nullptr; ga.hmask = e->h + (size_t)i * NH;
                if (!defer(c, b.d_convb[i - 1], T, H).on()) return no_parts();
                ga.bias_parts = b.d_convb[i - 1].p;
            }
            ga.x = t1; ga.W = e->P + e->o_gin_w2[i - 1]; ga.bn = bnref(c, i, N, 0);
            ga.dxp0 = c0; ga.dxp1 = c1;
            ga.slab = slab_take(c, b, (size_t)T * H * H, e->G + e->o_gin_w2[i - 1], H * H, T);
            RC(bn_bwd_sums(c, ga, T * nsl, bn_dsum(c, i), bn_dprod(c, i), st_i));
            hipLaunchKernelGGL((k_ggin_bwd<2>), dim3(T, nsl), dim3(GB_NT), 0, st, gd, e->gptr, e->eptr, ga, N, H, H, e->status);
            CAL_CHECK_LAUNCH("k_ggin_bwd<2>"); STAGE();
            RC(flush_finals(c)); STAGE();
            memset(&ga, 0, sizeof(ga));
            ga.dy0 = c0; ga.dy1 = two ? c1 : nullptr; ga.t1 = t1;
            ga.dot_sum = bn_dsum(c, i); ga.dot_prod = bn_dprod(c, i);
            if (!defer(c, b.d_gin_b1[i - 1], T, H).on()) return no_parts();
            ga.bias_parts = b.d_gin_b1[i - 1].p;
            ga.x = hin; ga.W = e->P + e->o_conv_w[i - 1]; ga.bn = bnref(c, i, N, 0);
            ga.dxp0 = d0; ga.dxp1 = d1;
            ga.slab = slab_take(c, b, (size_t)T * H * H, e->G + e->o_conv_w[i - 1], H * H, T);
            {
                ProfScope ps(st, 10, 4.0 * N * H * H + 2.0 * (double)(E + N) * H, true);
                PROF_LAUNCH((k_ggin_bwd<1>), dim3(T, nsl), dim3(GB_NT), 0, st, gd, e->gptr, e->eptr, ga, N, H, H, e->status);
            }
            CAL_CHECK_LAUNCH("k_ggin_bwd<1>"); STAGE();
            if (i == 1 && units) {
                RC(bwd_feat_units(c, b, x0, d0, two ? d1 : nullptr, true)); STAGE();
            } else if (i == 1) {
                GinRowArgs gr;
                memset(&gr, 0, sizeof(gr));
                gr.a = d0; gr.a2 = two ? d1 : nullptr; gr.y = e->h; gr.out = e->dZ;
                RC(gin_rows(c, 3, gr));
                CAL_CHECK_LAUNCH("k_gin_mask"); STAGE();
            }
            continue;
        }
        if (e->gin) {
            const float* agg = e->gagg + (size_t)(i - 1) * NH;
            const float* t1 = e->gt1 + (size_t)(i - 1) * NH;
            const float* yy = e->gy + (size_t)(i - 1) * NH;
            {
                GemmArgs a = gemm_args(H, H, N, true, false, 0);
                a.p[0].A = e->dZ; a.p[0].B = yy;
                float* dst[1] = {e->G + e->o_gin_w2[i - 1]};
                RC(grad_gemm(c, b, a, 1, dst)); STAGE();
            }
            {
                GemmArgs a = gemm_args(N, H, H, false, false, 0);
                a.p[0].A = e->dZ; a.p[0].B = e->P + e->o_gin_w2[i - 1]; a.p[0].C = e->dXh;
                RC(fwd_gemm(c, false, a, 1)); STAGE();
            }
            {
                GinRowArgs ga;
                memset(&ga, 0, sizeof(ga));
                ga.a = e->dXh; ga.y = yy; ga.t1 = t1; ga.bn = bnref(c, i, N, 0);
                ga.acc0 = node_acc(c, bn_dsum(c, i), H); ga.acc1 = node_acc(c, bn_dprod(c, i), H);
                RC(gin_rows(c, 1, ga));
                CAL_CHECK_LAUNCH("k_gin_dots"); STAGE();
                RC(flush_finals(c)); STAGE();
            }
            {
                GinRowArgs ga;
                memset(&ga, 0, sizeof(ga));
                ga.a = e->dXh; ga.y = yy; ga.t1 = t1; ga.out = dzi; ga.bn = bnref(c, i, N, 0);
                ga.dot_sum = bn_dsum(c, i); ga.dot_prod = bn_dprod(c, i);
                ga.acc0 = defer(c, b.d_gin_b1[i - 1], PN, H);
                if (!ga.acc0.on()) return no_parts();
                RC(gin_rows(c, 2, ga));
                CAL_CHECK_LAUNCH("k_gin_bn_bwd"); STAGE();
            }
            {
                GemmArgs a = gemm_args(H, H, N, true, false, 0);
                a.p[0].A = dzi; a.p[0].B = agg;
                float* dst[1] = {e->G + e->o_conv_w[i - 1]};
                RC(grad_gemm(c, b, a, 1, dst)); STAGE();
            }
            {
                GemmArgs a = gemm_args(N, H, H, false, false, 0);
                a.p[0].A = dzi; a.p[0].B = e->P + e->o_conv_w[i - 1]; a.p[0].C = e->dXh;
                RC(fwd_gemm(c, false, a, 1)); STAGE();
            }
            {
                SpmmBranch br{e->dXh, e->z, nullptr, nullptr, e->ones, Acc(), Acc(), nullptr, nullptr, nullptr};
                RC(launch_espmm(st, gs, SpmmBranch2{{br, br}}, 1, 0, 1.0f, N, H, spmm_rpb(H, false)));
                CAL_CHECK_LAUNCH("k_espmm(gin,T)"); STAGE();
            }
            {
                GinRowArgs ga;
                memset(&ga, 0, sizeof(ga));
                ga.a = e->z; ga.y = hin; ga.out = e->dZ;
                ga.acc0 = i >= 2 ? defer(c, b.d_convb[i - 2], PN, H) : Acc();
                RC(gin_rows(c, 3, ga));
                CAL_CHECK_LAUNCH("k_gin_mask"); STAGE();
            }
            continue;
        }
        float* p0 = ((L - i) & 1) ? e->z : e->dXh;
        if (r.bb_bwd != Conv::Node && i < L && !defer(c, b.d_convb[i - 1], T, H).on()) return no_parts();
        if (e->K > 0 && r.bb_bwd == Conv::Graph64) {
            const int K = e->K, D = H / K, nsl = H / GC_N;
            const size_t nk = al((size_t)e->capN * K);
            const float* sc = e->gsc + (size_t)(i - 1) * 4 * nk;
            GgatBwdArgs ga;
            memset(&ga, 0, sizeof(ga));
            ga.x = hin; ga.W = e->P + e->o_conv_w[i - 1]; ga.att = e->P + e->o_conv_att[i - 1];
            ga.z = e->gz + (size_t)(i - 1) * NH; ga.adst = sc; ga.asrc = sc + nk; ga.mx = sc + 2 * nk; ga.den = sc + 3 * nk;
            ga.bn = bnref(c, i, N, 0); ga.dxp0 = p0; ga.dxp1 = dzi;
            ga.heads = K; ga.D = D; ga.slope = e->gat_slope; ga.p = c.training ? e->gat_p : 0.f;
            ga.seed = e->gat_seed[i - 1]; ga.ctr = (const uint64_t*)e->gat_ctr; ga.E = E;
            if (i == L) ga.dout = e->dZ;
            else {
                ga.dy0 = ((L - i - 1) & 1) ? e->z : e->dXh;
                ga.dy1 = two ? e->dzi + (size_t)i * NH : nullptr;
                ga.y = e->h + (size_t)i * NH;
                ga.ubn = bnref(c, i + 1, N, 0); ga.udot_sum = bn_dsum(c, i + 1); ga.udot_prod = bn_dprod(c, i + 1);
                ga.bias_parts = b.d_convb[i - 1].p;
            }
            const size_t need_w = (size_t)T * H * H, need_a = (size_t)T * 2 * H;
            if (b.slab_off + need_w + need_a > e->slab_floats || b.fa.nst + 2 > MAX_SLABS) return no_slabs();
            ga.slab = slab_take(c, b, need_w, e->G + e->o_conv_w[i - 1], H * H, T);
            ga.att_slab = slab_take(c, b, need_a, e->G + e->o_conv_att[i - 1], 2 * H, T);
            RC(bn_bwd_sums(c, ga, T * nsl, bn_dsum(c, i), bn_dprod(c, i), st_i));
            {
                ProfScope ps(st, 8, 4.0 * N * H * H + 4.0 * (double)(E + N) * H, true);
                if (i == L) PROF_LAUNCH((k_ggat_bwd<false>), dim3(T, nsl), dim3(GB_NT), 0, st, gd, e->gptr, e->eptr, ga, N, H, H, e->status);
                else PROF_LAUNCH((k_ggat_bwd<true>), dim3(T, nsl), dim3(GB_NT), 0, st, gd, e->gptr, e->eptr, ga, N, H, H, e->status);
            }
            CAL_CHECK_LAUNCH("k_ggat_bwd"); STAGE();
            RC(flush_finals(c)); STAGE();
        } else if (r.bb_bwd != Conv::Node) {
            GconvBwdBranch gb;
            memset(&gb, 0, sizeof(gb));
            gb.x = hin; gb.W = e->P + e->o_conv_w[i - 1]; gb.dis = e->dis_unit; gb.bn = bnref(c, i, N, 0);
            gb.dxp0 = p0; gb.dxp1 = dzi;
            gb.coef_in = r.bb_bwd != Conv::Wide ? e->coef : r.plan_coef ? e->coef_src : nullptr;
            if (i == L) gb.dout = e->dZ;
            else {
                gb.dy0 = ((L - i - 1) & 1) ? e->z : e->dXh;
                gb.dy1 = two ? e->dzi + (size_t)i * NH : nullptr;
                gb.y = e->h + (size_t)i * NH;
                gb.ubn = bnref(c, i + 1, N, 0); gb.udot_sum = bn_dsum(c, i + 1); gb.udot_prod = bn_dprod(c, i + 1);
                gb.bias_parts = b.d_convb[i - 1].p;
            }
            float* dst[1] = {e->G + e->o_conv_w[i - 1]};
            double* dsum[1] = {bn_dsum(c, i)}; double* dprod[1] = {bn_dprod(c, i)};
            { ProfScope ps(st, 4, 4.0 * N * H * H + 2.0 * (double)(E + N) * H, true); RC(gconv_bwd(c, b, &gb, 1, dst, dsum, dprod, st_i)); } STAGE();
            RC(flush_finals(c)); STAGE();
        }
        auto bn_bwd_dz = [&](const float* q0, const float* q1, Acc acc, bool st_rd) -> int {
            BnBwdProb p{q0, hin, e->dZ, bnref(c, i, N, 0), bn_dsum(c, i), bn_dprod(c, i), acc, q1};
            RC(with_g(H, [&](auto g) {
                constexpr int G = decltype(g)::value;
                if (st_rd) hipLaunchKernelGGL((k_bn_bwd<4, G, true>), dim3(PN, 1), dim3(256), 0, st, BnBwdProb3{{p, p, p}}, 1, N, H, c.rpb_n);
                else hipLaunchKernelGGL((k_bn_bwd<4, G>), dim3(PN, 1), dim3(256), 0, st, BnBwdProb3{{p, p, p}}, 1, N, H, c.rpb_n);
                return 0;
            }));
            CAL_CHECK_LAUNCH("k_bn_bwd"); STAGE();
            return 0;
        };
        if (r.bb_bwd != Conv::Node) {
            if (i > 1) continue;
            if (units) { RC(bwd_feat_units(c, b, x0, p0, two ? dzi : nullptr, false)); STAGE(); }
            else RC(bn_bwd_dz(p0, two ? dzi : nullptr, Acc(), r.st_bb1));
            continue;
        }
        if (e->K > 0) {
            const int K = e->K, D = H / K;
            const size_t nk = al((size_t)e->capN * K);
            const float* sc = e->gsc + (size_t)(i - 1) * 4 * nk;
            ProfScope ps(st, 6, 4.0 * N * H * 4 + (double)(E + N) * (16 + 24.0 * K));
            const size_t need = (size_t)gat_datt_parts(N) * 2 * H;
            if (b.slab_off + need > e->slab_floats || b.fa.nst >= MAX_SLABS) return no_slabs();
            float* part = e->slabs + b.slab_off;
            int nparts = 0;
            RC(gat_backward(e->rowptr_dst, e->nbr_dst, e->eid_dst, e->rowptr_src, e->nbr_src, e->eid_src,
                            e->gz + (size_t)(i - 1) * NH, e->P + e->o_conv_att[i - 1], sc, sc + nk, sc + 2 * nk, sc + 3 * nk, e->dZ,
                            e->gat_slope, c.training ? e->gat_p : 0.f, e->gat_seed[i - 1], (const uint64_t*)e->gat_ctr, dzi,
                            e->G + e->o_conv_att[i - 1], e->gws, N, E, K, D, st, part, &nparts));
            b.fa.st[b.fa.nst++] = SlabTask{part, e->G + e->o_conv_att[i - 1], 2 * H, nparts};
            b.slab_off += need;
        } else {
            SpmmBranch br{e->dZ, dzi, nullptr, nullptr, e->dis_unit, Acc(), Acc(), nullptr, nullptr, nullptr};
            ProfScope ps(st, 1, 2.0 * N * H * 4 + (double)(E + N) * 8 + (N + 1) * 4.0, true);
            RC(launch_espmm(st, gs, SpmmBranch2{{br, br}}, 1, 0, e->loop_w, N, H, spmm_rpb(H, false)));
            CAL_CHECK_LAUNCH("k_espmm(T)");
        }
        STAGE();
        {
            GemmArgs aw = gemm_args(H, H, N, true, false, 0);
            aw.p[0].A = hin; aw.p[0].B = dzi;
            aw.p[0].xa.has_bn = 1; aw.p[0].xa.bn = bnref(c, i, N, 0);
            float* dst[1] = {e->G + e->o_conv_w[i - 1]};
            GemmArgs a = gemm_args(N, H, H, false, true, 0);
            a.p[0].A = dzi; a.p[0].B = e->P + e->o_conv_w[i - 1]; a.p[0].C = e->dXh;
            a.p[0].aux = hin; a.p[0].has_aux = 1; a.p[0].aux_bn = bnref(c, i, N, 0);
            gemm_stats(c, a.p[0], N, H, bn_dsum(c, i), bn_dprod(c, i), true, H, r.st_node);
            { ProfScope ps(st, 3, 4.0 * N * H * H); RC(dual_gemm(c, b, a, 1, aw, 1, dst)); } STAGE();
            RC(flush_finals(c)); STAGE();
        }
        if (i == 1 && r.feat_bwd == FeatBwd::Rows) {
            const int cols = (F + 1) * H;
            FeatBwdRowsArgs fb{e->dXh, hin, bnref(c, 1, N, 0), bn_dsum(c, 1), bn_dprod(c, 1), x0, bnref(c, 0, N, 0), parts_alloc(c, (size_t)PN * cols)};
            double* sums = parts_alloc(c, cols);
            b.d_bn0.p = parts_alloc(c, 2 * (size_t)F); b.d_bn0.P = 1; b.d_bn0.stride = 2 * F;
            if (!fb.parts || !sums || !b.d_bn0.p) return no_parts();
            float* dw = slab_take(c, b, (size_t)F * H, e->G + e->o_feat_w, F * H, 1);
            if (!dw) return no_slabs();
            RC(with_g_fp(H, F, [&](auto g, auto fp) {
                hipLaunchKernelGGL((k_bn_bwd_feat<decltype(g)::value, decltype(fp)::value>), dim3(PN), dim3(256), 0, st, fb, N, H, F, c.rpb_n);
                return 0;
            }));
            CAL_CHECK_LAUNCH("k_bn_bwd_feat"); STAGE();
            final_task(c, fb.parts, PN, cols, cols, sums);
            RC(flush_finals(c)); STAGE();
            hipLaunchKernelGGL(k_feat_bwd_final, dim3(F), dim3(256), 0, st, sums, e->P + e->o_feat_w, bnref(c, 0, N, 0), dw, b.d_bn0.p, H, F);
            CAL_CHECK_LAUNCH("k_feat_bwd_final"); STAGE();
        } else {
            RC(bn_bwd_dz(e->dXh, nullptr, i >= 2 ? defer(c, b.d_convb[i - 2], PN, H) : Acc(), r.st_node));
        }
    }
    return 0;
}

int bwd_feat(Ctx& c, Bwd& b, const float* x0) {
    Engine* e = c.e;
    const int N = c.N, H = e->H, F = e->F;
    if (c.r.feat_bwd != FeatBwd::Gemm) return 0;
    GemmArgs aw = gemm_args(F, H, N, true, false, 0);
    aw.p[0].A = x0; aw.p[0].B = e->dZ;
    aw.p[0].xa.has_bn = 1; aw.p[0].xa.bn = bnref(c, 0, N, 0);
    float* dst[1] = {e->G + e->o_feat_w};
    GemmArgs a = gemm_args(N, F, H, false, true, 0);
    a.p[0].A = e->dZ; a.p[0].B = e->P + e->o_feat_w; a.p[0].C = nullptr;
    a.p[0].aux = x0; a.p[0].has_aux = 1; a.p[0].aux_bn = bnref(c, 0, N, 0);
    a.p[0].dot_sum = bn_dsum(c, 0); a.p[0].dot_prod = bn_dprod(c, 0);
    {
        const int P0 = use_ks(N) ? gemm_ks_row_tiles(N) : gemm_row_tiles(N, F, H, false);
        if ((size_t)P0 * F * 2 > 4096) {
            b.d_bn0.p = parts_alloc(c, (size_t)P0 * 2 * F); b.d_bn0.P = P0; b.d_bn0.stride = 2 * F;
            a.p[0].parts = b.d_bn0.p;
        }
    }
    RC(dual_gemm(c, b, a, 1, aw, 1, dst)); STAGE();
    return 0;
}

int bwd_commit(Ctx& c, Bwd& b) {
    Engine* e = c.e;
    const int H = e->H, F = e->F, C = e->C, L = e->L;
    FinishArgs& fa = b.fa;
    auto commit_p = [&](const double* src, int P, int stride, int dst, int n, float scale) {
        if (fa.nct < MAX_COMMITS) fa.ct[fa.nct] = CommitTask{src, P, stride, dst, n, scale};
        fa.nct++;
    };
    auto commit_d = [&](const Deferred& d, int col, int dst, int n, float scale) { commit_p(d.p + col, d.P, d.stride, dst, n, scale); };
    for (int k = 0; k < e->nbn; ++k) {
        const BNSlot& s = e->bn[k];
        const int wp = (s.width + 3) / 4 * 4;
        if (k == 0 && b.d_bn0.p) {
            commit_d(b.d_bn0, F, s.gamma, F, 1.f);
            commit_d(b.d_bn0, 0, s.beta, F, 1.f);
            continue;
        }
        commit_p(e->arena + s.arena + 3 * wp, NSTRIPE, e->bn_plane, s.gamma, s.width, 1.f);
        commit_p(e->arena + s.arena + 2 * wp, NSTRIPE, e->bn_plane, s.beta, s.width, 1.f);
    }
    for (int i = 0; i < L; ++i) {
        if (!b.d_convb[i].p) { set_error("engine: missing bias-gradient partials"); return 2; }
        commit_d(b.d_convb[i], 0, e->gin ? e->o_gin_b2[i] : e->o_conv_b[i], H, 1.f);
        if (e->gin) {
            if (!b.d_gin_b1[i].p) { set_error("engine: missing bias-gradient partials"); return 2; }
            commit_d(b.d_gin_b1[i], 0, e->o_conv_b[i], H, 1.f);
        }
    }
    commit_d(b.d_cb, 0, e->o_cb, H, 1.f);
    commit_d(b.d_ob, 0, e->o_ob, H, 1.f);
    commit_d(b.d_dwn, 0, e->o_natt_w, H, 1.f);
    commit_d(b.d_dwn, 0, e->o_natt_w + H, H, -1.f);
    commit_d(b.d_dwn, H, e->o_natt_b, 1, 1.f);
    commit_d(b.d_dwn, H, e->o_natt_b + 1, 1, -1.f);
    commit_d(b.d_dwe, 0, e->o_eatt_w, 2 * H, 1.f);
    commit_d(b.d_dwe, 0, e->o_eatt_w + 2 * H, 2 * H, -1.f);
    commit_d(b.d_dwe, 2 * H, e->o_eatt_b, 1, 1.f);
    commit_d(b.d_dwe, 2 * H, e->o_eatt_b + 1, 1, -1.f);
    for (int hd = 0; hd < 3; ++hd) {
        commit_p(e->arena + e->a_db1 + hd * H, 1, 0, e->o_fc1_b[hd], H, 1.f);
        commit_p(e->arena + e->a_db2 + hd * C, 1, 0, e->o_fc2_b[hd], C, 1.f);
    }
    if (fa.nct > MAX_COMMITS) { set_error("engine: too many commit tasks"); return 2; }
    join_side(c);
    if (c.adam_in_finish) {
        fa.adam = AdamArgs{e->P, e->M1, e->M2, e->step, e->lr, e->beta1, e->beta2, e->eps, e->wd, e->grad_scale, 1};
        std::vector<std::pair<int64_t, int64_t>> iv;
        for (int i = 0; i < fa.nst; ++i) iv.push_back({fa.st[i].dst - e->G, (fa.st[i].dst - e->G) + fa.st[i].n});
        for (int i = 0; i < fa.nct; ++i) iv.push_back({fa.ct[i].dst, (int64_t)fa.ct[i].dst + fa.ct[i].n});
        std::sort(iv.begin(), iv.end());
        int64_t pos = 0;
        bool ok = true;
        auto gap = [&](int64_t a, int64_t b) {
            if (b <= a) return;
            if (fa.nar >= MAX_ADAM_RANGES) { ok = false; return; }
            fa.ar[fa.nar++] = AdamRange{a, b};
        };
        for (auto& r : iv) {
            if (r.first < pos) { ok = false; break; }
            gap(pos, r.first);
            pos = r.second;
        }
        gap(pos, e->nparam);
        if (!ok || pos > e->nparam) {
            fa.adam.on = 0; fa.nar = 0; c.adam_in_finish = 2;
        }
    }
    int nblk = 0;
    for (int i = 0; i < fa.nst; ++i) { fa.blk0[i] = nblk; nblk += std::max(1, cdiv(fa.st[i].n, 64)); }
    for (int i = 0; i < fa.nct; ++i) { fa.blk0[fa.nst + i] = nblk; nblk += std::max(1, cdiv(fa.ct[i].n, 16)); }
    for (int i = 0; i < fa.nar; ++i) { fa.blk0[fa.nst + fa.nct + i] = nblk; nblk += (int)cdiv(fa.ar[i].end - fa.ar[i].begin, 256); }
    fa.blk0[fa.nst + fa.nct + fa.nar] = nblk;
    hipLaunchKernelGGL(k_finish, dim3(nblk), dim3(256), 0, c.st, fa, e->G);
    CAL_CHECK_LAUNCH("k_finish"); STAGE();
    e->bn0_dirty_host = 0;
    return 0;
}

int engine_backward(Ctx& c, const float* x0) {
    Engine* e = c.e;
    Bwd b;
    memset(&b, 0, sizeof(b));
    FinishArgs& fa = b.fa;
    fa.tick = (c.tick_in_finish && !c.adam_in_finish) ? e->step : nullptr;
    fa.ticked = c.adam_in_finish ? e->step : nullptr;
    fa.perm_ctr = c.draw_perm ? e->perm_ctr : nullptr;
    fa.status = e->status;
    fa.host_status = e->host_status;
    { const int wp0 = (e->bn[0].width + 3) / 4 * 4; fa.bn0z = e->arena + e->bn[0].arena; fa.bn0z_n = 2 * wp0; fa.dirty = e->status + 3; }
    RC(bwd_readout(c, b));
    RC(bwd_co(c, b));
    RC(bwd_att(c, b));
    RC(bwd_backbone(c, b, x0));
    RC(bwd_feat(c, b, x0));
    return bwd_commit(c, b);
}

void ctx_init(Ctx& c, Engine* e, void* stream, int64_t N, int64_t E, int64_t B, const int64_t* batch, int mode) {
    memset(&c, 0, sizeof(c));
    c.e = e; c.st = (hipStream_t)stream; c.N = (int)N; c.B = (int)B; c.E = E;
    c.T = e->ntiles > 0 ? e->ntiles : (int)B;
    c.batch = batch;
    c.training = (mode & 1) ? 1 : 0;
    c.want_grad = (mode & 2) ? 1 : 0;
    c.rpb_n = std::max(32, cdiv(N, N >= 16384 && N <= 65536 ? 512 : 1024));
    c.rpb_b = std::max(32, cdiv(B, 64));
    c.r = make_route(c, c.want_grad);
}

}

CAL_EXPORT int cal_engine_step(void* h, const float* x0, const int64_t* edge_index, const int64_t* batch, const int64_t* y,
                               const int64_t* perm, int64_t N, int64_t E, int64_t B, float wc, float wo, float wco, int mode,
                               void* stream_) {
    Engine* e = (Engine*)h;
    CAL_REQUIRE(e && e->ws, "engine has no workspace");
    CAL_REQUIRE(N <= e->capN && E <= e->capE && B <= e->capB, "batch exceeds the workspace capacity");
    CAL_REQUIRE(N > 0 && B > 0, "empty batch");
    CAL_REQUIRE(e->ntiles <= B, "more tiles than graphs (cal_engine_set_tiles belongs to another batch)");
    CAL_REQUIRE(e->ntiles == 0 || (e->H % GC_N == 0 && e->H <= GC_K && e->node_ptr && e->edge_ptr && e->max_nodes > 0 && e->max_nodes <= 64 &&
                                   e->max_edges <= gc_edge_cap(64)),
                "cal_engine_set_tiles needs the per-graph kernels: hidden in {64, 128}, the tiles' offsets (cal_engine_set_graph_ptrs) and bounds <= 64 nodes / 1024 edges");
    const int want_grad = (mode & 2) ? 1 : 0;
    CAL_REQUIRE(!(mode & 16) || (e->perm_ctr && B <= ZP_CAP && want_grad), "mode bit 16 needs cal_engine_set_perm_rng, at most 1024 graphs per batch and the backward pass (its last kernel advances the permutation counter)");
    CAL_REQUIRE((mode & 16) || perm, "perm is null and the step does not draw its own (mode bit 16)");
    CAL_REQUIRE(!(mode & 8) || want_grad, "mode bit 8 (Adam follows a gradient exchange) needs the backward pass");
    CAL_REQUIRE(!want_grad || (mode & 1), "backward needs a training-mode forward");
    CAL_REQUIRE(!(mode & 4) || want_grad, "the Adam update needs the backward pass in the same step");
    Ctx c;
    ctx_init(c, e, stream_, N, E, B, batch, mode);
    c.adam_in_finish = ((mode & 4) && e->adam_fused) ? 1 : 0;
    c.draw_perm = (mode & 16) ? 1 : 0;
    c.y = y; c.perm = c.draw_perm ? e->perm_dev : perm; c.wc = wc; c.wo = wo; c.wco = wco;
    c.tick_in_finish = (mode & (4 | 8)) ? 1 : 0;
    g_stage = 0;
    g_stage_names.clear();
    {
        int rc = engine_forward(c, x0, edge_index);
        if (rc == -12345) return 0;
        if (rc) return rc;
        if (want_grad) {
            rc = engine_backward(c, x0);
            if (rc) join_side(c);
            if (rc == -12345) return 0;
            if (rc) return rc;
        }
    }
    if ((mode & 4) && c.adam_in_finish != 1) {
        hipLaunchKernelGGL(k_adam, dim3(cdiv(e->nparam, 256)), dim3(256), 0, c.st, e->P, e->G, e->M1, e->M2, e->step, e->lr, e->beta1,
                           e->beta2, e->eps, e->wd, e->nparam, 1, e->grad_scale, e->status);
        CAL_CHECK_LAUNCH("k_adam");
    }
    return 0;
}

CAL_EXPORT int cal_engine_backward_from(void* h, const float* x0, const int64_t* batch, const float* dlogp, int64_t N,
                                        int64_t E, int64_t B, void* stream_) {
    Engine* e = (Engine*)h;
    CAL_REQUIRE(e && e->ws, "engine has no workspace");
    CAL_REQUIRE(N <= e->capN && E <= e->capE && B <= e->capB && N > 0 && B > 0, "bad batch sizes");
    CAL_REQUIRE(e->ntiles <= B, "more tiles than graphs (cal_engine_set_tiles belongs to another batch)");
    Ctx c;
    ctx_init(c, e, stream_, N, E, B, batch, 1);
    c.want_grad = 1;
    hipLaunchKernelGGL(k_logsoftmax_bwd, dim3(1), dim3(256), 0, c.st, e->logp, dlogp, e->dzl, e->arena + e->a_db2, (int)B, e->C);
    CAL_CHECK_LAUNCH("k_logsoftmax_bwd");
    g_stage = 0;
    int rc = engine_backward(c, x0);
    if (rc) join_side(c);
    return rc == -12345 ? 0 : rc;
}

CAL_EXPORT int cal_causal_loss(const float* logp, const int64_t* y, int64_t B, int64_t C, float wc, float wo, float wco, float* out,
                               float* dlogp, int32_t* flag, void* stream_) {
    CAL_REQUIRE(logp && y && out && B > 0 && C > 0 && B * C < (1ll << 30), "bad arguments");
    hipLaunchKernelGGL(k_causal_loss, dim3(1), dim3(256), 0, (hipStream_t)stream_, logp, y, (int)B, (int)C, wc, wo, wco, out, dlogp, (int*)flag);
    CAL_CHECK_LAUNCH("k_causal_loss");
    return 0;
}

CAL_EXPORT int cal_engine_set_graph_bounds(void* h, int64_t max_nodes, int64_t max_edges) {
    Engine* e = (Engine*)h;
    CAL_REQUIRE(e != nullptr && max_nodes >= 0 && max_edges >= 0, "bad arguments");
    e->max_nodes = (int)std::min<int64_t>(max_nodes, 1 << 30);
    e->max_edges = (int)std::min<int64_t>(max_edges, 1 << 30);
    return 0;
}
CAL_EXPORT int cal_engine_set_graph_ptrs(void* h, const int64_t* node_ptr, const int64_t* edge_ptr) {
    Engine* e = (Engine*)h;
    CAL_REQUIRE(e != nullptr, "bad arguments");
    e->node_ptr = node_ptr; e->edge_ptr = edge_ptr;
    return 0;
}
CAL_EXPORT int cal_engine_set_tiles(void* h, const int64_t* tile_gptr, int64_t ntiles) {
    Engine* e = (Engine*)h;
    CAL_REQUIRE(e != nullptr && ntiles >= 0 && (ntiles == 0 || tile_gptr != nullptr), "bad arguments");
    e->tile_gptr = ntiles > 0 ? tile_gptr : nullptr; e->ntiles = (int)ntiles;
    return 0;
}
CAL_EXPORT int cal_engine_set_deterministic(void* h, int on) {
    Engine* e = (Engine*)h;
    CAL_REQUIRE(e != nullptr, "bad arguments");
    e->striped = on ? 0 : 1;
    return 0;
}
CAL_EXPORT int cal_engine_debug_stop(int k) { g_stop_after = k; return 0; }
CAL_EXPORT const char* cal_engine_stage_name(int k) {
    return k >= 1 && k <= (int)g_stage_names.size() ? g_stage_names[k - 1] : "";
}

CAL_EXPORT int cal_sparse_probe_espmm(const int64_t* iv, void* const* pv, const double* dv, void* stream_) {
    CAL_REQUIRE(iv && pv && dv, "description missing");
    const int64_t nnz = iv[0], nbranch = iv[1], N = iv[3], H = iv[4], rpb = iv[5];
    CAL_REQUIRE(nbranch == 1 || nbranch == 2, "one or two branches");
    CAL_REQUIRE(H % 4 == 0 && H >= 4 && H <= 256, "hidden must be a multiple of 4 in [4, 256]");
    CAL_REQUIRE(N >= 1 && N < (1ll << 31) && nnz >= 0 && nnz < (1ll << 31) && rpb >= 1 && rpb < (1ll << 31), "sizes out of range");
    CSR csr;
    csr.ptr = (const int*)pv[0]; csr.nbr = (const int*)pv[1]; csr.eid = (const int*)pv[2]; csr.nnz = (int)nnz;
    SpmmBranch2 bb;
    for (int b = 0; b < 2; ++b) {
        const int64_t* ib = iv + 6 + 2 * std::min<int64_t>(b, nbranch - 1);
        void* const* pb = pv + 3 + 14 * std::min<int64_t>(b, nbranch - 1);
        SpmmBranch& br = bb.b[b];
        br.h = (const float*)pb[0]; br.out = (float*)pb[1]; br.bias = (const float*)pb[2]; br.w = (const float*)pb[3];
        br.dis = (const float*)pb[4];
        br.st_sum = Acc((double*)pb[5], (double*)pb[6], (int)ib[0]);
        br.st_sq = Acc((double*)pb[7], (double*)pb[8], (int)ib[1]);
        br.sd_z = (const float*)pb[9]; br.sd_gn = (float*)pb[10]; br.sd_gself = (float*)pb[11];
        br.pb_g = (const float*)pb[12]; br.pb_batch = (const int64_t*)pb[13];
    }
    RC(launch_espmm((hipStream_t)stream_, csr, bb, (int)nbranch, (int)iv[2], (float)dv[0], (int)N, (int)H, (int)rpb));
    CAL_CHECK_LAUNCH("k_espmm(probe)");
    return 0;
}
CAL_EXPORT int cal_sparse_probe_edge_att(const int* ptr, const int* nbr, const int* eid, int64_t nnz, const float* pq, const float* be,
                                         float* att, float* dis_c, float* dis_o, double loop_w, int64_t N, int64_t E, double fedge,
                                         void* stream_) {
    CAL_REQUIRE(ptr && nbr && eid && pq && be && att && dis_c && dis_o, "null argument");
    CAL_REQUIRE(N >= 1 && N < (1ll << 31) && E >= 0 && nnz >= 0 && nnz < (1ll << 31), "sizes out of range");
    CSR gs;
    gs.ptr = ptr; gs.nbr = nbr; gs.eid = eid; gs.nnz = (int)nnz;
    hipLaunchKernelGGL(k_edge_att_deg, dim3(cdiv(N, 32)), dim3(256), 0, (hipStream_t)stream_, gs, pq, be, att, dis_c, dis_o,
                       (float)loop_w, (int)N, E, (float)fedge);
    CAL_CHECK_LAUNCH("k_edge_att_deg(probe)");
    return 0;
}
CAL_EXPORT int cal_sparse_probe_pool(int sel, const float* hc, const float* ho, const int* gptr, const int64_t* batch, float* pooled,
                                     float* cnt, float* slices, int64_t N, int64_t B, int64_t H, int64_t rpb_n, int64_t* S_out,
                                     void* stream_) {
    CAL_REQUIRE(sel >= 0 && sel <= 3 && S_out != nullptr, "bad selector");
    CAL_REQUIRE(H % 4 == 0 && H >= 4 && H <= 256, "hidden must be a multiple of 4 in [4, 256]");
    CAL_REQUIRE(N >= 1 && N < (1ll << 31) && B >= 1 && B < (1ll << 31), "sizes out of range");
    const int S = pool2_slices((int)N, (int)B);
    *S_out = S;
    if (sel == 3) return 0;
    CAL_REQUIRE(hc && ho && (sel == 2 ? batch != nullptr && cnt != nullptr && rpb_n >= 1 && rpb_n < (1ll << 31) : gptr != nullptr && pooled != nullptr),
                "null argument");
    if (sel == 2) return launch_pool_cnt((hipStream_t)stream_, hc, ho, batch, cnt, (int)N, (int)B, (int)H, (int)rpb_n);
    CAL_REQUIRE(S == 1 || slices != nullptr, "row slices without a slice buffer");
    return launch_pool2((hipStream_t)stream_, hc, ho, gptr, pooled, sel == 0 ? cnt : nullptr, slices, (int)N, (int)B, (int)H);
}
#ifdef CAL_BLK_CLOCKS
CAL_EXPORT int cal_debug_blk_clocks(long long* out) {
    return (int)hipMemcpyFromSymbol(out, HIP_SYMBOL(cal::g_blk_clk), sizeof(long long) * 8192);
}
#endif
#ifdef CAL_RO_CLOCKS
CAL_EXPORT int cal_debug_ro_clocks(long long* out) {
    return (int)hipMemcpyFromSymbol(out, HIP_SYMBOL(cal::g_ro_clk), sizeof(long long) * 64);
}
#endif

CAL_EXPORT int cal_engine_profile(int on) {
    g_prof_on = on != 0;
    if (on) {
        for (auto& r : g_prof) { hipEventDestroy(r.e0); hipEventDestroy(r.e1); }
        g_prof.clear();
    }
    return 0;
}
CAL_EXPORT int64_t cal_engine_profile_read(double* out, int64_t cap) {
    int64_t n = 0;
    for (auto& r : g_prof) {
        if (n >= cap) break;
        float ms = 0.f;
        if (hipEventElapsedTime(&ms, r.e0, r.e1) != hipSuccess) ms = -1.f;
        out[3 * n] = r.cls; out[3 * n + 1] = ms; out[3 * n + 2] = r.work;
        ++n;
    }
    return n;
}

CAL_EXPORT int cal_engine_adam(void* h, void* stream_) {
    Engine* e = (Engine*)h;
    hipStream_t st = (hipStream_t)stream_;
    hipLaunchKernelGGL(k_adam, dim3(cdiv(e->nparam, 256)), dim3(256), 0, st, e->P, e->G, e->M1, e->M2, e->step, e->lr, e->beta1,
                       e->beta2, e->eps, e->wd, e->nparam, 0, e->grad_scale, e->status);
    CAL_CHECK_LAUNCH("k_adam");
    hipLaunchKernelGGL(k_adam_tick, dim3(1), dim3(1), 0, st, e->step);
    CAL_CHECK_LAUNCH("k_adam_tick");
    return 0;
}
CAL_EXPORT int cal_engine_adam_ticked(void* h, void* stream_) {
    Engine* e = (Engine*)h;
    hipStream_t st = (hipStream_t)stream_;
    hipLaunchKernelGGL(k_adam, dim3(cdiv(e->nparam, 256)), dim3(256), 0, st, e->P, e->G, e->M1, e->M2, e->step, e->lr, e->beta1,
                       e->beta2, e->eps, e->wd, e->nparam, 1, e->grad_scale, e->status);
    CAL_CHECK_LAUNCH("k_adam");
    return 0;
}
CAL_EXPORT int cal_p2p_alloc(int64_t bytes, void** out) {
    CAL_REQUIRE(bytes > 0 && out, "bad arguments");
    void* p = nullptr;
    hipError_t rc = hipExtMallocWithFlags(&p, (size_t)bytes, hipDeviceMallocFinegrained);
    if (rc != hipSuccess || !p) { (void)hipGetLastError(); set_error("cal_p2p_alloc: hipExtMallocWithFlags(fine-grained, %lld bytes): %s", (long long)bytes, hipGetErrorString(rc)); return 3; }
    rc = hipMemset(p, 0, (size_t)bytes);
    if (rc == hipSuccess) rc = hipDeviceSynchronize();
    if (rc != hipSuccess) { (void)hipGetLastError(); (void)hipFree(p); set_error("cal_p2p_alloc: zeroing failed: %s", hipGetErrorString(rc)); return 3; }
    *out = p;
    return 0;
}
CAL_EXPORT int cal_p2p_free(void* p) {
    if (p && hipFree(p) != hipSuccess) { (void)hipGetLastError(); set_error("cal_p2p_free failed"); return 3; }
    return 0;
}
CAL_EXPORT int cal_p2p_export(void* p, void* handle64) {
    CAL_REQUIRE(p && handle64, "bad arguments");
    static_assert(sizeof(hipIpcMemHandle_t) == 64, "IPC handle size");
    hipIpcMemHandle_t hd;
    hipError_t rc = hipIpcGetMemHandle(&hd, p);
    if (rc != hipSuccess) { (void)hipGetLastError(); set_error("cal_p2p_export: hipIpcGetMemHandle: %s", hipGetErrorString(rc)); return 3; }
    memcpy(handle64, &hd, 64);
    return 0;
}
CAL_EXPORT int cal_p2p_open(const void* handle64, void** out) {
    CAL_REQUIRE(handle64 && out, "bad arguments");
    hipIpcMemHandle_t hd;
    memcpy(&hd, handle64, 64);
    void* p = nullptr;
    hipError_t rc = hipIpcOpenMemHandle(&p, hd, hipIpcMemLazyEnablePeerAccess);
    if (rc != hipSuccess || !p) { (void)hipGetLastError(); set_error("cal_p2p_open: hipIpcOpenMemHandle: %s", hipGetErrorString(rc)); return 3; }
    *out = p;
    return 0;
}
CAL_EXPORT int cal_p2p_close(void* p) {
    if (p && hipIpcCloseMemHandle(p) != hipSuccess) { (void)hipGetLastError(); set_error("cal_p2p_close failed"); return 3; }
    return 0;
}
CAL_EXPORT int64_t cal_engine_p2p_region_bytes(void* h) {
    Engine* e = (Engine*)h;
    const int64_t np = (e->nparam + 63) / 64 * 64;
    return (2 * np + 64) * 4;
}
CAL_EXPORT int cal_engine_p2p_bind(void* h, void* const* peer_bases, const int64_t* peer_devices, int64_t world, int64_t rank) {
    Engine* e = (Engine*)h;
    CAL_REQUIRE(e && e->P && world >= 1 && world <= P2P_MAX_WORLD && rank >= 0 && rank < world && peer_bases, "bad arguments (bind the parameters first; at most 8 ranks)");
    int dev = 0;
    hipGetDevice(&dev);
    memset(&e->p2p, 0, sizeof(e->p2p));
    for (int r = 0; r < world; ++r) {
        CAL_REQUIRE(peer_bases[r] != nullptr, "null peer region");
        e->p2p.region[r] = (float*)peer_bases[r];
        if (peer_devices && (int)peer_devices[r] != dev) {
            hipError_t rc = hipDeviceEnablePeerAccess((int)peer_devices[r], 0);
            if (rc != hipSuccess && rc != hipErrorPeerAccessAlreadyEnabled) { set_error("cal_engine_p2p_bind: no peer access to device %d", (int)peer_devices[r]); return 3; }
            (void)hipGetLastError();
        }
    }
    if (!e->p2p_host_status) {
        hipError_t rc = hipHostMalloc((void**)&e->p2p_host_status, 64, hipHostMallocMapped | hipHostMallocCoherent);
        if (rc != hipSuccess) { (void)hipGetLastError(); e->p2p_host_status = nullptr; set_error("cal_engine_p2p_bind: hipHostMalloc failed"); return 3; }
    }
    *e->p2p_host_status = 0;
    e->p2p.host_status = e->p2p_host_status; e->p2p.max_polls = e->p2p_max_polls;
    e->p2p.rank = (int)rank; e->p2p.world = (int)world; e->p2p.np = (e->nparam + 63) / 64 * 64;
    e->p2p_on = 1;
    return 0;
}
CAL_EXPORT int cal_engine_p2p_set_timeout(void* h, int64_t max_polls) {
    Engine* e = (Engine*)h;
    CAL_REQUIRE(e && max_polls >= 1 && max_polls <= (1ll << 30), "bad arguments");
    e->p2p_max_polls = (int)max_polls; e->p2p.max_polls = (int)max_polls;
    return 0;
}
CAL_EXPORT int64_t cal_engine_peek_status(void* h) {
    Engine* e = (Engine*)h;
    if (!e || !e->host_status) return 0;
    return (int64_t)__atomic_load_n(e->host_status, __ATOMIC_ACQUIRE);
}
CAL_EXPORT int64_t cal_engine_p2p_status(void* h) {
    Engine* e = (Engine*)h;
    if (!e || !e->p2p_host_status) return 0;
    return (int64_t)__atomic_load_n(e->p2p_host_status, __ATOMIC_ACQUIRE);
}
CAL_EXPORT int cal_engine_p2p_adam(void* h, void* stream_) {
    Engine* e = (Engine*)h;
    CAL_REQUIRE(e && e->p2p_on && e->ws, "cal_engine_p2p_bind first");
    const AdamArgs A{e->P, e->M1, e->M2, e->step, e->lr, e->beta1, e->beta2, e->eps, e->wd, e->grad_scale, 1};
    const int nb = (int)std::min<int64_t>(P2P_BLOCKS, cdiv(e->nparam, 256));
    hipLaunchKernelGGL(k_p2p_adam, dim3(nb), dim3(256), 0, (hipStream_t)stream_, e->p2p, e->G, A, e->nparam, e->status);
    CAL_CHECK_LAUNCH("k_p2p_adam");
    return 0;
}
CAL_EXPORT int cal_engine_set_options(void* h, int cat, int no_node_att, int no_edge_att) {
    Engine* e = (Engine*)h;
    CAL_REQUIRE(e != nullptr, "bad arguments");
    e->cat = cat ? 1 : 0; e->no_node_att = no_node_att ? 1 : 0; e->no_edge_att = no_edge_att ? 1 : 0;
    return 0;
}
CAL_EXPORT int cal_engine_set_gin(void* h, int on) {
    Engine* e = (Engine*)h;
    CAL_REQUIRE(e != nullptr && (!on || e->K == 0), "bad arguments");
    e->gin = on ? 1 : 0;
    return 0;
}
CAL_EXPORT int cal_engine_set_perm_rng(void* h, uint64_t seed, uint64_t* counter) {
    Engine* e = (Engine*)h;
    CAL_REQUIRE(e != nullptr, "bad arguments");
    e->perm_seed = seed; e->perm_ctr = (unsigned long long*)counter;
    return 0;
}
CAL_EXPORT int cal_engine_set_adam(void* h, float beta1, float beta2, float eps, float weight_decay) {
    Engine* e = (Engine*)h;
    CAL_REQUIRE(e != nullptr && beta1 >= 0.f && beta1 < 1.f && beta2 >= 0.f && beta2 < 1.f && eps >= 0.f && weight_decay >= 0.f, "bad arguments");
    e->beta1 = beta1; e->beta2 = beta2; e->eps = eps; e->wd = weight_decay;
    return 0;
}
CAL_EXPORT int cal_engine_set_grad_scale(void* h, float scale) {
    Engine* e = (Engine*)h;
    CAL_REQUIRE(e != nullptr && scale > 0.f, "bad arguments");
    e->grad_scale = scale;
    return 0;
}
```

cal_amd/csrc/engine_gconv_bwd.hpp:

```cpp
#pragma once
#include "engine_gconv.hpp"

namespace cal {

constexpr int GB_NT = 512;
constexpr int GB_T = 64;
constexpr int GB_E = 1024;
constexpr int GB_LDJ = GB_T + 1;
constexpr int GB_LDD = GC_N + 4;
constexpr int GB_LDW = GC_K + 1;
constexpr int GB_LDX = GC_K + 4;

struct GconvBwdBranch {
    const float* dout;
    const float* x;
    const float* W;
    const float* ew;
    const float* dis;
    const float* rs;
    int rs_stride;
    BNRef bn;
    float* dxp0; float* dxp1;
    float* slab;
    double* dot_parts;
    double* dacc_sum; double* dacc_prod; int dacc_ss;
    const float* coef_in;
    const float* dy0; const float* dy1;
    const float* y;
    BNRef ubn;
    const double* udot_sum; const double* udot_prod;
    double* bias_parts;
    const float* gp0; const float* gp1; const int* iperm;
    const float* z;
    float* gn; float* gself;
    size_t gn_stride, gself_stride;
    int gn_slot;
    const int64_t* batch;
    const int64_t* tile_gptr;
};

struct GconvBwdBranch2 { GconvBwdBranch b[2]; };

template <bool RS, int MODE, bool TILED = false, bool LEAN = false>
__global__ void __launch_bounds__(GB_NT, (LEAN ? 4 : 1)) k_gconv_bwd(const CSR g, const int* __restrict__ gptr, const int* __restrict__ eptr,
                                                   const GconvBwdBranch2 bb, float loop_w, int N, int H,
                                                   int K, int* __restrict__ status) {
    constexpr int LDX = LEAN ? GC_K : GB_LDX;
    __shared__ __attribute__((aligned(16))) float Ab[GB_T * GB_LDJ];
    __shared__ __attribute__((aligned(16))) float Ds[GB_T * GB_LDD];
    __shared__ __attribute__((aligned(16))) float Ws[LEAN ? 4 : GC_K * GB_LDD];
    __shared__ __attribute__((aligned(16))) float Xs[GB_T * LDX];
    __shared__ float mean_s[GC_K], rstd_s[GC_K], gam_s[GC_K], bet_s[GC_K];
    __shared__ int ptr_s[GB_T + 4];
    __shared__ float dis_s[GB_T], rs_s[GB_T];
    __shared__ unsigned char en[GB_E];
    __shared__ float ec[GB_E];
    __shared__ float um_s[MODE == 1 ? GC_N : 1], ur_s[MODE == 1 ? GC_N : 1], ug_s[MODE == 1 ? GC_N : 1], u1_s[MODE == 1 ? GC_N : 1], u2_s[MODE == 1 ? GC_N : 1];
    __shared__ float bs_s[GB_NT / 64][16][4];
    __shared__ __attribute__((aligned(16))) float Zr_own[(MODE == 2 && !LEAN) ? GB_T * GB_LDD : 4];
    float* const Zr = (MODE == 2 && LEAN) ? Xs : Zr_own;
    __shared__ float gv_s[TILED ? GC_TILE_GRAPHS * GC_N : GC_N];
    __shared__ unsigned char bg_s[TILED ? GB_T : 4];
    __shared__ int ee[(MODE == 2 && !LEAN) ? GB_E : 1];
    __shared__ unsigned char er[GB_E];
    constexpr bool UP = MODE == 1, POOL = MODE == 2;
    static_assert(!TILED || MODE == 2, "only the POOL variant looks at the graphs inside a tile");
    BLK_CLK(0);
    warm_kernargs<sizeof(CSR) + 2 * sizeof(void*) + sizeof(GconvBwdBranch2) + 32>();
    const GconvBwdBranch& br = bb.b[blockIdx.z];
    const int b = blockIdx.x, sl = blockIdx.y, ns0 = sl * GC_N, t = threadIdx.x;
    const int g0 = gptr[b], rows = gptr[b + 1] - g0, e0 = eptr[b], ne = eptr[b + 1] - e0;
    const int pb = (MODE == 2 && !TILED && br.iperm) ? br.iperm[b] : b;
    const int tg0 = TILED ? (int)br.tile_gptr[b] : b, ng = TILED ? (int)br.tile_gptr[b + 1] - tg0 : 1;
    const int lane = t & 63, li = lane & 31, lk = lane >> 5;
    const int w = __builtin_amdgcn_readfirstlane(t >> 6);
    double* parts = br.dot_parts + ((size_t)sl * gridDim.x + b) * (2 * K);
    float* slab = br.slab + (size_t)b * K * H;
    if (rows <= 0 || rows > GB_T || ne > GB_E || ne < 0 || (TILED && (ng < 1 || ng > GC_TILE_GRAPHS))) {
        if (rows > 0 && t == 0) atomicOr(status, 8);
        if (!br.dacc_sum) for (int i = t; i < 2 * K; i += GB_NT) parts[i] = 0.0;
        if ((UP || POOL) && t < GC_N) br.bias_parts[(size_t)b * H + ns0 + t] = 0.0;
        for (int i = t; i < K * GC_N; i += GB_NT) slab[(size_t)(i / GC_N) * H + ns0 + i % GC_N] = 0.f;
        return;
    }
    const bool hasw = br.ew != nullptr;
    const int rowsP = (rows + 31) & ~31, R = rowsP >> 5, K4 = K >> 2;
    RoBatch<float4, 2> bd, bd1, by;
    RoBatch<float4, 4> bx, bw;
    RoBatch<float4, 2> bz;
    float gv = 0.f, gv1 = 0.f;
    int pbq = 0;
    long long bgv = 0;
    if (POOL) {
        ro_issue<GB_NT>(by, rows, 16, [&](int j, int n4) { return *reinterpret_cast<const float4*>(br.y + (size_t)(g0 + j) * H + ns0 + 4 * n4); });
        ro_issue<GB_NT>(bz, rows, 16, [&](int j, int n4) { return *reinterpret_cast<const float4*>(br.z + (size_t)(g0 + j) * H + ns0 + 4 * n4); });
        if (!TILED) {
            const float* gp1 = br.gp1 ? br.gp1 : br.gp0;
            gv = br.gp0[(size_t)b * H + ns0 + (t & (GC_N - 1))];
            gv1 = gp1[(size_t)pb * H + ns0 + (t & (GC_N - 1))];
        } else {
            const int gq = tg0 + min(t >> 6, ng - 1);
            gv = br.gp0[(size_t)gq * H + ns0 + (t & (GC_N - 1))];
            pbq = br.iperm ? br.iperm[gq] : gq;
            bgv = br.batch[g0 + min(t, rows - 1)];
        }
    } else {
        const float* d0 = UP ? br.dy0 : br.dout;
        ro_issue<GB_NT>(bd, rows, 16, [&](int j, int n4) { return *reinterpret_cast<const float4*>(d0 + (size_t)(g0 + j) * H + ns0 + 4 * n4); });
        if (UP) {
            const float* d1 = br.dy1 ? br.dy1 : br.dy0;
            ro_issue<GB_NT>(bd1, rows, 16, [&](int j, int n4) { return *reinterpret_cast<const float4*>(d1 + (size_t)(g0 + j) * H + ns0 + 4 * n4); });
            ro_issue<GB_NT>(by, rows, 16, [&](int j, int n4) { return *reinterpret_cast<const float4*>(br.y + (size_t)(g0 + j) * H + ns0 + 4 * n4); });
        }
    }
    ro_issue<GB_NT>(bx, rows, K4, [&](int i, int k4) { return *reinterpret_cast<const float4*>(br.x + (size_t)(g0 + i) * K + 4 * k4); });
    if (!LEAN) ro_issue<GB_NT>(bw, K, 16, [&](int k, int n4) { return *reinterpret_cast<const float4*>(br.W + (size_t)k * H + ns0 + 4 * n4); });
    const int pv = g.ptr[g0 + min(t, rows)];
    const int pn = g.ptr[g0 + min(t + 1, rows)];
    const float dv = br.dis[g0 + min(t, rows - 1)];
    const float rv = RS ? br.rs[(size_t)(g0 + min(t, rows - 1)) * br.rs_stride] : 1.f;
    int nv[2], ev[2];
    const int slot_hi = max(g.nnz - 1, 0);
    const float* coefp = br.coef_in ? br.coef_in : br.dis;
    const int coef_hi = br.coef_in ? slot_hi : 0;
    float cin[2];
#pragma unroll
    for (int u = 0; u < 2; ++u) {
        const int s = min(e0 + max(min(t + u * GB_NT, ne - 1), 0), slot_hi);
        nv[u] = g.nbr[s];
        ev[u] = g.eid[s];
        cin[u] = coefp[min(s, coef_hi)];
    }
    const bool ulane = UP && t >= 256;
    BNRawS braws = UP ? bn_raws_load2(br.bn, min(t, K - 1), br.ubn, ns0 + (t & (GC_N - 1)), ulane) : bn_raws_load(br.bn, min(t, K - 1));
    StripeVal ud1s, ud2s;
    if (UP) {
        const int c = ns0 + (t & (GC_N - 1));
        ud1s = stripe_load(br.udot_sum, c, br.ubn.ss); ud2s = stripe_load(br.udot_prod, c, br.ubn.ss);
    }
    bn_raws_pin(braws);
    if (UP) { stripe_pin(ud1s); stripe_pin(ud2s); }
#pragma unroll
    for (int u = 0; u < 2; ++u) asm volatile("" : "+v"(nv[u]), "+v"(ev[u]), "+v"(cin[u]));
    if (POOL && !TILED) { asm volatile("" : "+v"(gv), "+v"(gv1)); gv += br.gp1 ? gv1 : 0.f; }
    if (TILED) {
        asm volatile("" : "+v"(gv), "+v"(pbq), "+v"(bgv));
        const float* gp1 = br.gp1 ? br.gp1 : br.gp0;
        gv1 = gp1[(size_t)pbq * H + ns0 + (t & (GC_N - 1))];
    }
    if (ne <= 0) { nv[0] = g0; nv[1] = g0; ev[0] = 0; ev[1] = 0; }
    if (UP && t >= 256 && t < 256 + GC_N) {
        float m1, r1;
        const BNRaw uraw = bn_raws_sum(br.ubn, braws);
        const double ud1 = stripe_total(ud1s, br.ubn.ss), ud2 = stripe_total(ud2s, br.ubn.ss);
        bn_raw_mean_rstd(br.ubn, uraw, m1, r1);
        um_s[t - 256] = m1; ur_s[t - 256] = r1;
        ug_s[t - 256] = uraw.g * r1;
        u1_s[t - 256] = (float)(ud1 * (double)br.ubn.inv_n);
        u2_s[t - 256] = (float)(ud2 * (double)br.ubn.inv_n);
    }
    if (t < K) {
        float m1, r1;
        const BNRaw braw = bn_raws_sum(br.bn, braws);
        bn_raw_mean_rstd(br.bn, braw, m1, r1);
        mean_s[t] = m1; rstd_s[t] = r1;
        gam_s[t] = braw.g;
        bet_s[t] = braw.b;
    }
    for (int i = t; i < (rowsP * GB_LDJ + 3) / 4; i += GB_NT) reinterpret_cast<float4*>(Ab)[i] = make_float4(0.f, 0.f, 0.f, 0.f);
    float cv[2];
    if (br.coef_in) {
#pragma unroll
        for (int u = 0; u < 2; ++u) cv[u] = cin[u];
    } else {
        const float* ewp = hasw ? br.ew : br.dis;
#pragma unroll
        for (int u = 0; u < 2; ++u) {
            const float c = br.dis[nv[u]];
            const float wl = ewp[hasw ? ev[u] : 0];
            cv[u] = hasw ? c * wl : c;
        }
    }
    if (t <= rows) ptr_s[t] = pv - e0;
    if (t < rows) {
        dis_s[t] = dv; rs_s[t] = rv;
        for (int s = pv - e0; s < pn - e0; ++s) er[s] = (unsigned char)t;
    }
#pragma unroll
    for (int u = 0; u < 2; ++u) {
        const int s = t + u * GB_NT;
        if (s < ne) {
            const int loc = nv[u] - g0;
            const bool inb = loc >= 0 && loc < rows;
            en[s] = (unsigned char)(inb ? loc : 0); ec[s] = inb ? cv[u] : 0.f;
            if (POOL && !LEAN) ee[s] = ev[u];
            if (!inb) atomicOr(status, 16);
        }
    }
    if (POOL && !TILED && t < GC_N) gv_s[t] = gv;
    if (TILED) {
        if (t < ng * GC_N) gv_s[t] = gv + (br.gp1 ? gv1 : 0.f);
        if (t < rows) bg_s[t] = (unsigned char)min(max((int)(bgv - tg0), 0), ng - 1);
    }
    if (MODE == 0) ro_commit<GB_NT>(bd, rows, 16, [&](int j, int n4, const float4 v) { *reinterpret_cast<float4*>(Ds + j * GB_LDD + 4 * n4) = v; });
    if (!LEAN) ro_commit<GB_NT>(bw, K, 16, [&](int k, int n4, const float4 v) { *reinterpret_cast<float4*>(Ws + k * GB_LDD + 4 * n4) = v; });
    __syncthreads();
    auto commit_x = [&]() {
        ro_commit<GB_NT>(bx, rows, K4, [&](int i, int k4, float4 v) {
            const float s = RS ? rs_s[i] : 1.f;
            const int k = 4 * k4;
            v.x = (v.x * s - mean_s[k]) * rstd_s[k]; v.y = (v.y * s - mean_s[k + 1]) * rstd_s[k + 1];
            v.z = (v.z * s - mean_s[k + 2]) * rstd_s[k + 2]; v.w = (v.w * s - mean_s[k + 3]) * rstd_s[k + 3];
            *reinterpret_cast<float4*>(Xs + i * LDX + k) = v;
        });
    };
    if (!(POOL && LEAN)) commit_x();
    if (POOL) {
        float cs[4] = {0.f, 0.f, 0.f, 0.f};
#pragma unroll
        for (int u = 0; u < 2; ++u) { ro_pin(by.v[u]); ro_pin(bz.v[u]); }
        const int c = 4 * (t & 15);
#pragma unroll
        for (int u = 0; u < 2; ++u) {
            const int j = (t >> 4) + u * (GB_NT / 16);
            if (j < rows) {
                const float4 yv = by.v[u];
                const float* gvr = gv_s + (TILED ? bg_s[j] * GC_N : 0);
                const float4 o = make_float4(yv.x > 0.f ? gvr[c] : 0.f, yv.y > 0.f ? gvr[c + 1] : 0.f,
                                             yv.z > 0.f ? gvr[c + 2] : 0.f, yv.w > 0.f ? gvr[c + 3] : 0.f);
                cs[0] += o.x; cs[1] += o.y; cs[2] += o.z; cs[3] += o.w;
                *reinterpret_cast<float4*>(Ds + j * GB_LDD + c) = o;
                *reinterpret_cast<float4*>(Zr + j * GB_LDD + c) = bz.v[u];
            }
        }
#pragma unroll
        for (int q = 0; q < 4; ++q) {
            cs[q] += __shfl_xor(cs[q], 16, 64);
            cs[q] += __shfl_xor(cs[q], 32, 64);
        }
        if (lane < 16) {
#pragma unroll
            for (int q = 0; q < 4; ++q) bs_s[t >> 6][lane][q] = cs[q];
        }
    }
    if (UP) {
        float cs[4] = {0.f, 0.f, 0.f, 0.f};
        const bool two = br.dy1 != nullptr;
#pragma unroll
        for (int u = 0; u < 2; ++u) { ro_pin(bd.v[u]); ro_pin(bd1.v[u]); ro_pin(by.v[u]); }
        const int c = 4 * (t & 15);
#pragma unroll
        for (int u = 0; u < 2; ++u) {
            const int j = (t >> 4) + u * (GB_NT / 16);
            if (j < rows) {
                const float4 v0 = bd.v[u], v1 = bd1.v[u], yv = by.v[u];
                const float d[4] = {v0.x + (two ? v1.x : 0.f), v0.y + (two ? v1.y : 0.f), v0.z + (two ? v1.z : 0.f), v0.w + (two ? v1.w : 0.f)};
                const float yy[4] = {yv.x, yv.y, yv.z, yv.w};
                float o[4];
#pragma unroll
                for (int q = 0; q < 4; ++q) {
                    const float yn = (yy[q] - um_s[c + q]) * ur_s[c + q];
                    const float g1 = ug_s[c + q] * (d[q] - u1_s[c + q] - yn * u2_s[c + q]);
                    o[q] = yy[q] > 0.f ? g1 : 0.f;
                    cs[q] += o[q];
                }
                *reinterpret_cast<float4*>(Ds + j * GB_LDD + c) = make_float4(o[0], o[1], o[2], o[3]);
            }
        }
#pragma unroll
        for (int q = 0; q < 4; ++q) {
            cs[q] += __shfl_xor(cs[q], 16, 64);
            cs[q] += __shfl_xor(cs[q], 32, 64);
        }
        if (lane < 16) {
#pragma unroll
            for (int q = 0; q < 4; ++q) bs_s[t >> 6][lane][q] = cs[q];
        }
    }
    for (int i = t; i < (rowsP - rows) * GB_LDD; i += GB_NT) Ds[rows * GB_LDD + i] = 0.f;
    for (int i = t; i < (rowsP - rows) * LDX; i += GB_NT) Xs[rows * LDX + i] = 0.f;
    for (int s = t; s < ne; s += GB_NT) {
        const int j = er[s];
        atomicAdd(&Ab[j * GB_LDJ + en[s]], dis_s[j] * ec[s]);
    }
    if (t < rows) atomicAdd(&Ab[t * GB_LDJ + t], dis_s[t] * dis_s[t] * loop_w);
    __syncthreads();
    if ((UP || POOL) && t < GC_N) {
        double tot = 0.0;
#pragma unroll
        for (int k = 0; k < GB_NT / 64; ++k) tot += (double)bs_s[k][t >> 2][t & 3];
        br.bias_parts[(size_t)b * H + ns0 + t] = tot;
    }
    BLK_CLK(2);
    auto ident = [](float v) { return v; };
    gc_f32x16 acc[2];
    {
        const int rt = w >> 1, ct = w & 1;
#pragma unroll
        for (int i = 0; i < 16; ++i) { acc[0][i] = 0.f; acc[1][i] = 0.f; }
        if (rt < R) mma_kmajor<1, 1, GB_LDJ, GB_LDD>(Ab + rt * 32 + li, Ds + ct * 32 + li, rowsP, lk, ident, MmaIdent(), acc);
        if (POOL && w >= 4) {
            const int q4 = (t - 256) & 3, it0 = (t - 256) >> 2;
            float* gn = br.gn + (size_t)sl * br.gn_stride;
            float* gs = br.gself + (size_t)sl * br.gself_stride;
            for (int it = it0; it - it0 < ne + rows; it += 64) {
                const bool ok = it < ne + rows, isedge = it < ne;
                const int itc = ok ? it : 0;
                const int jd = isedge ? er[itc] : itc - ne, js = isedge ? en[itc] : itc - ne;
                const float4* a = reinterpret_cast<const float4*>(Ds + (ok ? jd : 0) * GB_LDD + 16 * q4);
                const float4* bsrc = reinterpret_cast<const float4*>(Zr + (ok ? js : 0) * GB_LDD + 16 * q4);
                float p = 0.f;
#pragma unroll
                for (int k = 0; k < 4; ++k) p = dot4(a[k], bsrc[k], p);
                p += __shfl_xor(p, 1, 64);
                p += __shfl_xor(p, 2, 64);
                if (ok && q4 == 0) {
                    if (isedge) gn[(LEAN || br.gn_slot) ? e0 + itc : ee[itc]] = p; else gs[g0 + itc - ne] = p;
                }
            }
        }
        __syncthreads();
        if (POOL && LEAN) commit_x();
        if (rt < R) {
#pragma unroll
            for (int r = 0; r < 16; ++r) {
                const int row = mma_row(r, lk, rt * 32);
                Ds[row * GB_LDD + ct * 32 + li] = acc[0][r];
            }
        }
        __syncthreads();
    }
    if (w < 4 && w * 32 < K) {
#pragma unroll
        for (int i = 0; i < 16; ++i) { acc[0][i] = 0.f; acc[1][i] = 0.f; }
        const float* wrow = LEAN ? br.W + (size_t)min(w * 32 + li, K - 1) * H + ns0 : Ws + (w * 32 + li) * GB_LDD;
        if (R == 2) mma_rowk<true>(Ds + li * GB_LDD, Ds + (32 + li) * GB_LDD, wrow, GC_N, lk, acc[0], acc[1]);
        else mma_rowk<false>(Ds + li * GB_LDD, nullptr, wrow, GC_N, lk, acc[0], acc[1]);
        const int k = w * 32 + li;
        float* dxp = sl ? br.dxp1 : br.dxp0;
        float xh[2][16];
#pragma unroll
        for (int q = 0; q < 2; ++q)
#pragma unroll
            for (int r = 0; r < 16; ++r) xh[q][r] = Xs[(mma_row(r, lk, q * 32)) * LDX + k];
#pragma unroll
        for (int q = 0; q < 2; ++q)
#pragma unroll
            for (int r = 0; r < 16; ++r) { asm volatile("" : "+v"(xh[q][r])); if (q >= R) xh[q][r] = 0.f; }
        float f1[4] = {0.f, 0.f, 0.f, 0.f}, f2[4] = {0.f, 0.f, 0.f, 0.f};
#pragma unroll
        for (int q = 0; q < 2; ++q) {
#pragma unroll
            for (int r = 0; r < 16; ++r) {
                const int i = mma_row(r, lk, q * 32);
                const float v = acc[q][r];
                f1[r & 3] += v;
                f2[r & 3] = fmaf(v, xh[q][r], f2[r & 3]);
            }
        }
        gc_store_tile<gc_site(WT_DXP)>(acc[0], dxp + (size_t)g0 * K + w * 32, K, rows, li, lk, MmaIdent(), (rows * K - w * 32) * 4);
        if (R == 2) gc_store_tile<gc_site(WT_DXP)>(acc[1], dxp + (size_t)(g0 + 32) * K + w * 32, K, rows - 32, li, lk, MmaIdent(), ((rows - 32) * K - w * 32) * 4);
        double s1 = ((double)f1[0] + (double)f1[1]) + ((double)f1[2] + (double)f1[3]);
        double s2 = ((double)f2[0] + (double)f2[1]) + ((double)f2[2] + (double)f2[3]);
        s1 += __shfl_xor(s1, 32, 64);
        s2 += __shfl_xor(s2, 32, 64);
        if (lk == 0) {
            if (br.dacc_sum) {
                const size_t po = (size_t)stripe_of_block() * br.dacc_ss + k;
                atomicAdd(br.dacc_sum + po, s1); atomicAdd(br.dacc_prod + po, s2);
            } else { parts[k] = s1; parts[K + k] = s2; }
        }
    }
    BLK_CLK(3);
    if (w >= 4 && (w - 4) * 32 < K) {
        const int wq = w - 4, k = wq * 32 + li;
        const float gam = gam_s[k], bet = bet_s[k];
        auto affine = [&](float v) { return fmaf(v, gam, bet); };
#pragma unroll
        for (int i = 0; i < 16; ++i) { acc[0][i] = 0.f; acc[1][i] = 0.f; }
        mma_kmajor<1, 2, LDX, GB_LDD>(Xs + wq * 32 + li, Ds + li, rowsP, lk, affine, MmaIdent(), acc);
#pragma unroll
        for (int q = 0; q < 2; ++q) {
            const int off = wq * 32 * H + ns0 + q * 32;
            gc_store_tile<gc_site(WT_DW)>(acc[q], slab + off, H, 32, li, lk, MmaIdent(), (K * H - off) * 4);
        }
    }
    BLK_CLK(1);
}

constexpr int FB_T = 64, FB_F = 64, FB_H = 128;
struct FeatBwdArgs {
    const float* dy0; const float* dy1;
    const float* y;
    BNRef ubn; const double* udot_sum; const double* udot_prod;
    const float* x0;
    const float* W;
    BNRef bn0;
    float* slab;
    double* parts;
};
template <int FMAX>
__global__ void __launch_bounds__(GB_NT) k_feat_bwd(const int* __restrict__ gptr, const FeatBwdArgs a, int H, int F,
                                                  int* __restrict__ status, int N) {
    __shared__ __attribute__((aligned(16))) float Dz[FB_T * (FB_H + 4)];
    __shared__ float Xn[FB_T * FMAX];
    __shared__ __attribute__((aligned(16))) float Ws[FMAX * (FB_H + 4)];
    __shared__ float um_s[FB_H], ur_s[FB_H], ug_s[FB_H], u1_s[FB_H], u2_s[FB_H];
    __shared__ float m0_s[FMAX], r0_s[FMAX], g0_s[FMAX], b0_s[FMAX];
    __shared__ float dX0[FB_T * FMAX];
    BLK_CLK(0);
    warm_kernargs<sizeof(FeatBwdArgs) + 32>();
    const int b = blockIdx.x, t = threadIdx.x, LDZ = FB_H + 4;
    const int g0 = gptr ? gptr[b] : b * FB_T, rows = gptr ? gptr[b + 1] - g0 : min(FB_T, N - g0);
    float* slab = a.slab + (size_t)b * F * H;
    double* parts = a.parts + (size_t)b * 2 * F;
    if (rows <= 0 || rows > FB_T) {
        if (rows > 0 && t == 0) atomicOr(status, 8);
        for (int i = t; i < F * H; i += GB_NT) slab[i] = 0.f;
        for (int i = t; i < 2 * F; i += GB_NT) parts[i] = 0.0;
        return;
    }
    const int H4 = H >> 2;
    RoBatch<float4, 4> b0, b1, by, bwt;
    const float* d1 = a.dy1 ? a.dy1 : a.dy0;
    ro_issue<GB_NT>(b0, rows, H4, [&](int j, int c) { return *reinterpret_cast<const float4*>(a.dy0 + (size_t)(g0 + j) * H + 4 * c); });
    ro_issue<GB_NT>(b1, rows, H4, [&](int j, int c) { return *reinterpret_cast<const float4*>(d1 + (size_t)(g0 + j) * H + 4 * c); });
    ro_issue<GB_NT>(bwt, F, H4, [&](int f, int c) { return *reinterpret_cast<const float4*>(a.W + (size_t)f * H + 4 * c); });
    ro_issue<GB_NT>(by, rows, H4, [&](int j, int c) { return *reinterpret_cast<const float4*>(a.y + (size_t)(g0 + j) * H + 4 * c); });
    float xr[8];
#pragma unroll
    for (int u = 0; u < 8; ++u) xr[u] = a.x0[(size_t)g0 * F + min(t + u * GB_NT, rows * F - 1)];
    const int uc = min(t, H - 1), fc = min(max(t - 128, 0), F - 1);
    BNRawS uraws = bn_raws_load(a.ubn, uc);
    BNRaw raw0 = bn_raw_load(a.bn0, fc);
    StripeVal ud1s = stripe_load(a.udot_sum, uc, a.ubn.ss), ud2s = stripe_load(a.udot_prod, uc, a.ubn.ss);
    bn_raws_pin(uraws); bn_raw_pin(raw0);
    stripe_pin(ud1s); stripe_pin(ud2s);
    if (t < H) {
        float m1, r1;
        const BNRaw uraw = bn_raws_sum(a.ubn, uraws);
        const double ud1 = stripe_total(ud1s, a.ubn.ss), ud2 = stripe_total(ud2s, a.ubn.ss);
        bn_raw_mean_rstd(a.ubn, uraw, m1, r1);
        um_s[t] = m1; ur_s[t] = r1;
        ug_s[t] = uraw.g * r1;
        u1_s[t] = (float)(ud1 * (double)a.ubn.inv_n);
        u2_s[t] = (float)(ud2 * (double)a.ubn.inv_n);
    } else if (t - 128 < F && t >= 128) {
        const int f = t - 128;
        float m1, r1;
        bn_raw_mean_rstd(a.bn0, raw0, m1, r1);
        m0_s[f] = m1; r0_s[f] = r1;
        g0_s[f] = raw0.g;
        b0_s[f] = raw0.b;
    }
#pragma unroll
    for (int u = 0; u < 8; ++u) asm volatile("" : "+v"(xr[u]));
    ro_commit<GB_NT>(bwt, F, H4, [&](int f, int c, const float4 v) { *reinterpret_cast<float4*>(Ws + f * LDZ + 4 * c) = v; });
    __syncthreads();
    {
        const bool two = a.dy1 != nullptr;
#pragma unroll
        for (int u = 0; u < 4; ++u) { ro_pin(b1.v[u]); ro_pin(by.v[u]); }
        const int q = GB_NT / H4, r = GB_NT % H4;
        int row = t / H4, col = t % H4;
#pragma unroll
        for (int u = 0; u < 4; ++u) ro_pin(b0.v[u]);
#pragma unroll
        for (int u = 0; u < 4; ++u) {
            if (t + u * GB_NT < rows * H4) {
                const float4 v0 = b0.v[u], v1 = b1.v[u], yv = by.v[u];
                const int c = 4 * col;
                const float d[4] = {v0.x + (two ? v1.x : 0.f), v0.y + (two ? v1.y : 0.f), v0.z + (two ? v1.z : 0.f), v0.w + (two ? v1.w : 0.f)};
                const float yy[4] = {yv.x, yv.y, yv.z, yv.w};
                float o[4];
#pragma unroll
                for (int k = 0; k < 4; ++k) {
                    const float yn = (yy[k] - um_s[c + k]) * ur_s[c + k];
                    const float g1 = ug_s[c + k] * (d[k] - u1_s[c + k] - yn * u2_s[c + k]);
                    o[k] = yy[k] > 0.f ? g1 : 0.f;
                }
                *reinterpret_cast<float4*>(Dz + row * LDZ + c) = make_float4(o[0], o[1], o[2], o[3]);
            }
            row += q; col += r;
            if (col >= H4) { col -= H4; ++row; }
        }
#pragma unroll
        for (int u = 0; u < 8; ++u) {
            const int i = t + u * GB_NT;
            if (i < rows * F) { const int f = i % F; Xn[(i / F) * FMAX + f] = (xr[u] - m0_s[f]) * r0_s[f]; }
        }
    }
    __syncthreads();
    BLK_CLK(2);
    for (int o = t; o < F * H4; o += GB_NT) {
        const int f = o / H4, n = 4 * (o % H4);
        const float gam = g0_s[f], bet = b0_s[f];
        float4 acc = make_float4(0.f, 0.f, 0.f, 0.f);
#pragma unroll 4
        for (int j = 0; j < rows; ++j) {
            const float xv = fmaf(Xn[j * FMAX + f], gam, bet);
            const float4 d = *reinterpret_cast<const float4*>(Dz + j * LDZ + n);
            acc.x = fmaf(xv, d.x, acc.x); acc.y = fmaf(xv, d.y, acc.y); acc.z = fmaf(xv, d.z, acc.z); acc.w = fmaf(xv, d.w, acc.w);
        }
        *reinterpret_cast<float4*>(slab + (size_t)f * H + n) = acc;
    }
    BLK_CLK(3);
    {
        const int j = (t & 255) >> 2, qn = t & 3, nq4 = H >> 4;
        const int fh = (F + 1) >> 1, f_lo = t < 256 ? 0 : fh, f_hi = t < 256 ? fh : F;
        float4 dz[FB_H / 16];
#pragma unroll
        for (int k = 0; k < FB_H / 16; ++k)
            dz[k] = *reinterpret_cast<const float4*>(Dz + min(j, rows - 1) * LDZ + 4 * (qn * nq4 + min(k, nq4 - 1)));
#pragma unroll
        for (int k = 0; k < FB_H / 16; ++k) { ro_pin(dz[k]); if (k >= nq4) dz[k] = make_float4(0.f, 0.f, 0.f, 0.f); }
        for (int f = f_lo; f < f_hi; ++f) {
            const float4* wr = reinterpret_cast<const float4*>(Ws + f * LDZ) + qn * nq4;
            float4 wv[FB_H / 16];
#pragma unroll
            for (int k = 0; k < FB_H / 16; ++k) wv[k] = wr[min(k, nq4 - 1)];
            float p = 0.f;
#pragma unroll
            for (int k = 0; k < FB_H / 16; ++k) p = dot4(dz[k], wv[k], p);
            p += __shfl_xor(p, 1, 64);
            p += __shfl_xor(p, 2, 64);
            if (qn == 0 && j < rows) dX0[j * FMAX + f] = p;
        }
    }
    __syncthreads();
    {
        const int f = t >> 3, p = t & 7, fc = min(f, F - 1);
        float a1 = 0.f, a2 = 0.f;
        float dv[FB_T / 8], xv[FB_T / 8];
#pragma unroll
        for (int u = 0; u < FB_T / 8; ++u) {
            const int j = min(p + 8 * u, rows - 1);
            dv[u] = dX0[j * FMAX + fc]; xv[u] = Xn[j * FMAX + fc];
        }
#pragma unroll
        for (int u = 0; u < FB_T / 8; ++u) {
            const float v = p + 8 * u < rows ? dv[u] : 0.f;
            a1 += v; a2 = fmaf(v, xv[u], a2);
        }
        double s1 = (double)a1, s2 = (double)a2;
#pragma unroll
        for (int o = 1; o < 8; o <<= 1) { s1 += __shfl_xor(s1, o, 64); s2 += __shfl_xor(s2, o, 64); }
        if (p == 0 && f < F) { parts[f] = s1; parts[F + f] = s2; }
    }
    BLK_CLK(1);
}

constexpr int FM_F = 160;
template <int XU, bool NOBN>
__global__ void __launch_bounds__(GB_NT) k_feat_bwd_mma(const int* __restrict__ gptr, const FeatBwdArgs a, int H, int F,
                                                      int* __restrict__ status) {
    constexpr int FP = XU == 8 ? 64 : FM_F, LDXN = FP + 1, LDZ = FB_H + 4;
    __shared__ __attribute__((aligned(16))) float Dz[FB_T * LDZ];
    __shared__ float Xn[FB_T * LDXN];
    __shared__ float um_s[FB_H], ur_s[FB_H], ug_s[FB_H], u1_s[FB_H], u2_s[FB_H];
    __shared__ float m0_s[FP], r0_s[FP], g0_s[FP], b0_s[FP];
    __shared__ float cs_s[FB_H];
    __shared__ float csp[GB_NT / 64][32][4];
    __shared__ float s12[2][4][FP];
    __shared__ float red_s[GB_NT / 64][2][32][33];
    BLK_CLK(0);
    warm_kernargs<sizeof(FeatBwdArgs) + 32>();
    const int b = blockIdx.x, t = threadIdx.x;
    const int g0 = gptr[b], rows = gptr[b + 1] - g0;
    float* slab = a.slab + (size_t)b * F * H;
    double* parts = a.parts + (size_t)b * 2 * F;
    if (rows <= 0 || rows > FB_T) {
        if (rows > 0 && t == 0) atomicOr(status, 8);
        for (int i = t; i < F * H; i += GB_NT) slab[i] = 0.f;
        for (int i = t; i < 2 * F; i += GB_NT) parts[i] = 0.0;
        return;
    }
    const int H4 = H >> 2, rowsP = (rows + 31) & ~31, nct = H >> 5, nft = (F + 31) >> 5;
    RoBatch<float4, 4> b0, b1, by;
    const float* d1 = a.dy1 ? a.dy1 : a.dy0;
    ro_issue<GB_NT>(b0, rows, H4, [&](int j, int c) { return *reinterpret_cast<const float4*>(a.dy0 + (size_t)(g0 + j) * H + 4 * c); });
    ro_issue<GB_NT>(b1, rows, H4, [&](int j, int c) { return *reinterpret_cast<const float4*>(d1 + (size_t)(g0 + j) * H + 4 * c); });
    ro_issue<GB_NT>(by, rows, H4, [&](int j, int c) { return *reinterpret_cast<const float4*>(a.y + (size_t)(g0 + j) * H + 4 * c); });
    float xr[XU];
#pragma unroll
    for (int u = 0; u < XU; ++u) xr[u] = a.x0[(size_t)g0 * F + min(t + u * GB_NT, rows * F - 1)];
    const int lane = t & 63, li = lane & 31, lk = lane >> 5;
    const int w = __builtin_amdgcn_readfirstlane(t >> 6);
    const int ct = w % nct, fstep = (GB_NT / 64) / nct;
    float wv[16];
    auto load_w = [&](int ft) {
#pragma unroll
        for (int r = 0; r < 16; ++r) wv[r] = a.W[(size_t)min(mma_row(r, lk, ft * 32), F - 1) * H + ct * 32 + li];
    };
    load_w(w / nct);
    const int uc = min(t, H - 1), fc = min(max(t - 128, 0), F - 1);
    BNRawS uraws;
    BNRaw raw0 = bn_raw_load(a.bn0, fc);
    StripeVal ud1s, ud2s;
    if (!NOBN) { uraws = bn_raws_load(a.ubn, uc); ud1s = stripe_load(a.udot_sum, uc, a.ubn.ss); ud2s = stripe_load(a.udot_prod, uc, a.ubn.ss); bn_raws_pin(uraws); stripe_pin(ud1s); stripe_pin(ud2s); }
    bn_raw_pin(raw0);
    if (!NOBN && t < H) {
        float m1, r1;
        const double ud1 = stripe_total(ud1s, a.ubn.ss), ud2 = stripe_total(ud2s, a.ubn.ss);
        const BNRaw uraw = bn_raws_sum(a.ubn, uraws);
        bn_raw_mean_rstd(a.ubn, uraw, m1, r1);
        um_s[t] = m1; ur_s[t] = r1;
        ug_s[t] = uraw.g * r1;
        u1_s[t] = (float)(ud1 * (double)a.ubn.inv_n);
        u2_s[t] = (float)(ud2 * (double)a.ubn.inv_n);
    }
    if (t >= 128 && t - 128 < FP) {
        const int f = t - 128;
        float m1, r1;
        bn_raw_mean_rstd(a.bn0, raw0, m1, r1);
        m0_s[f] = m1; r0_s[f] = f < F ? r1 : 0.f;
        g0_s[f] = raw0.g;
        b0_s[f] = raw0.b;
    }
#pragma unroll
    for (int u = 0; u < XU; ++u) asm volatile("" : "+v"(xr[u]));
#pragma unroll
    for (int r = 0; r < 16; ++r) asm volatile("" : "+v"(wv[r]));
    for (int i = t; i < rowsP * LDXN; i += GB_NT) Xn[i] = 0.f;
    __syncthreads();
    {
        const bool two = a.dy1 != nullptr;
#pragma unroll
        for (int u = 0; u < 4; ++u) { ro_pin(b0.v[u]); ro_pin(b1.v[u]); ro_pin(by.v[u]); }
        const int col = t % H4, c = 4 * col, rstep = GB_NT / H4;
        int row = t / H4;
        float cs[4] = {0.f, 0.f, 0.f, 0.f};
#pragma unroll
        for (int u = 0; u < 4; ++u) {
            if (row < rowsP) {
                float o[4] = {0.f, 0.f, 0.f, 0.f};
                if (row < rows) {
                    const float4 v0 = b0.v[u], v1 = b1.v[u], yv = by.v[u];
                    const float d[4] = {v0.x + (two ? v1.x : 0.f), v0.y + (two ? v1.y : 0.f), v0.z + (two ? v1.z : 0.f), v0.w + (two ? v1.w : 0.f)};
                    const float yy[4] = {yv.x, yv.y, yv.z, yv.w};
#pragma unroll
                    for (int k = 0; k < 4; ++k) {
                        float g1 = d[k];
                        if (!NOBN) {
                            const float yn = (yy[k] - um_s[c + k]) * ur_s[c + k];
                            g1 = ug_s[c + k] * (d[k] - u1_s[c + k] - yn * u2_s[c + k]);
                        }
                        o[k] = yy[k] > 0.f ? g1 : 0.f;
                        cs[k] += o[k];
                    }
                }
                *reinterpret_cast<float4*>(Dz + row * LDZ + c) = make_float4(o[0], o[1], o[2], o[3]);
            }
            row += rstep;
        }
#pragma unroll
        for (int k = 0; k < 4; ++k) {
            if (H4 <= 32) cs[k] += __shfl_xor(cs[k], 32, 64);
            if (H4 <= 16) cs[k] += __shfl_xor(cs[k], 16, 64);
        }
        const int lane = t & 63;
        if (lane < H4 && lane < 32) {
#pragma unroll
            for (int k = 0; k < 4; ++k) csp[t >> 6][lane][k] = cs[k];
        }
#pragma unroll
        for (int u = 0; u < XU; ++u) {
            const int i = t + u * GB_NT;
            if (i < rows * F) { const int f = i % F; Xn[(i / F) * LDXN + f] = (xr[u] - m0_s[f]) * r0_s[f]; }
        }
    }
    __syncthreads();
    if (t < H) {
        float tot = 0.f;
#pragma unroll
        for (int k = 0; k < GB_NT / 64; ++k) tot += csp[k][t >> 2][t & 3];
        cs_s[t] = tot;
    }
    __syncthreads();
    BLK_CLK(2);
    auto ident = [](float v) { return v; };
    for (int ft = w / nct; ft < nft; ft += fstep) {
        gc_f32x16 acc[2];
#pragma unroll
        for (int i = 0; i < 16; ++i) { acc[0][i] = 0.f; acc[1][i] = 0.f; }
        mma_kmajor<1, 1, LDXN, LDZ>(Xn + ft * 32 + li, Dz + ct * 32 + li, rowsP, lk, ident, MmaIdent(), acc);
        const int h = ct * 32 + li;
        const float csh = cs_s[h];
        float wc[16];
#pragma unroll
        for (int r = 0; r < 16; ++r) wc[r] = wv[r];
        float p1[16], p2[16];
#pragma unroll
        for (int r = 0; r < 16; ++r) {
            const int f = mma_row(r, lk, ft * 32);
            const float pv = acc[0][r];
            acc[1][r] = fmaf(g0_s[min(f, FP - 1)], pv, b0_s[min(f, FP - 1)] * csh);
            p1[r] = f < F ? wc[r] * csh : 0.f;
            p2[r] = f < F ? wc[r] * pv : 0.f;
        }
#pragma unroll
        for (int r = 0; r < 16; ++r) {
            const int fl = mma_row(r, lk);
            red_s[w][0][fl][li] = p1[r];
            red_s[w][1][fl][li] = p2[r];
        }
        __builtin_amdgcn_s_waitcnt(0xc07f);
        {
            const float* rr = &red_s[w][lk][li][0];
            float v[32], tot = 0.f;
#pragma unroll
            for (int q = 0; q < 32; ++q) v[q] = rr[q];
#pragma unroll
            for (int q = 0; q < 32; ++q) tot += v[q];
            const int f = ft * 32 + li;
            if (f < FP) s12[lk][ct][f] = tot;
        }
#pragma unroll
        for (int r = 0; r < 16; ++r) {
            const int f = mma_row(r, lk, ft * 32);
            if (f < F) slab[(size_t)f * H + h] = acc[1][r];
        }
        if (ft + fstep < nft) {
            load_w(ft + fstep);
#pragma unroll
            for (int r = 0; r < 16; ++r) asm volatile("" : "+v"(wv[r]));
        }
    }
    BLK_CLK(3);
    __syncthreads();
    if (t < F) {
        double s1 = 0.0, s2 = 0.0;
        for (int k = 0; k < nct; ++k) { s1 += (double)s12[0][k][t]; s2 += (double)s12[1][k][t]; }
        parts[t] = s1; parts[F + t] = s2;
    }
    BLK_CLK(1);
}

}
```

Measured before the change: 606,600 graphs/s.

## Fold first-layer feature backward into gconv backward and finish kernel

Adds a Folded feature-backward route. The layer-1 GCN backward kernel no longer writes the full per-node dX tile. It computes per-graph partial products of the normalized input features against the ReLU-masked gradients (U, A, Bn slabs) using MFMA. The finish kernel then reduces those slabs and, in the last block selected by a ticket counter, applies the BN1 backward correction to form the feature weight, gamma and beta grads, with Adam applied in the same pass. This removes the separate feature-units backward pass and the dX round trip, at the cost of extra MFMA work, extra shared memory and a cross-block ticket reduction.

```diff
diff --git a/cal_amd/csrc/engine.hip b/cal_amd/csrc/engine.hip
--- a/cal_amd/csrc/engine.hip
+++ b/cal_amd/csrc/engine.hip
@@ -25,7 +25,22 @@
 constexpr int MAX_SLABS = 24;
 constexpr int MAX_COMMITS = 64;
 
+struct FoldTask {
+    int nblk;
+    const float* U; const float* A; const float* Bn;
+    int SU, SA;
+    int pu, pa;
+    int n;
+    double* scratch;
+    int* ticket;
+    BNRef bn1; const double* dsum; const double* dprod;
+    const float* W; const float* g0; const float* b0;
+    int o_w, o_g, o_b;
+    int F, H;
+};
+
 struct FinishArgs {
+    FoldTask fold;
     SlabTask st[MAX_SLABS];
     CommitTask ct[MAX_COMMITS];
     int nst, nct;
@@ -43,6 +58,88 @@
     const int* status;
     int blk0[MAX_SLABS + MAX_COMMITS + MAX_ADAM_RANGES + 1];
 };
+__device__ __forceinline__ void finish_fold(const FoldTask& ft, float* __restrict__ grad, const AdamArgs& A, float adam_t, float adam_lr) {
+    __shared__ double fred[256];
+    __shared__ int last_s;
+    __shared__ double gs_s[128], m1_s[128], m2_s[128];
+    __shared__ double wred[2][16][2];
+    const int bx = blockIdx.x, t = threadIdx.x;
+    const int ng = ft.n >> 6, nbu = ng * ft.pu, nba = ng * ft.pa;
+    {
+        const int set = bx < nbu ? 0 : bx < nbu + nba ? 1 : 2;
+        const int lb = bx - (set == 0 ? 0 : set == 1 ? nbu : nbu + nba);
+        const int part = lb / ng, i = (lb % ng) * 64 + (t & 63), wv = t >> 6;
+        const float* slabs = set == 0 ? ft.U : set == 1 ? ft.A : ft.Bn;
+        const int S = set == 0 ? ft.SU : ft.SA, parts = set == 0 ? ft.pu : ft.pa;
+        const int per_b = (S + parts - 1) / parts, s_lo = part * per_b, s_hi = min(S, s_lo + per_b);
+        const int per = (max(s_hi - s_lo, 0) + 3) / 4, z_lo = s_lo + wv * per, z_hi = min(s_hi, z_lo + per);
+        double s0 = 0.0, s1 = 0.0;
+        for (int z0 = z_lo; z0 < z_hi; z0 += 8) {
+            float v[8];
+#pragma unroll
+            for (int u = 0; u < 8; ++u) v[u] = slabs[(size_t)max(min(z0 + u, z_hi - 1), 0) * ft.n + i];
+#pragma unroll
+            for (int u = 0; u < 8; ++u) asm volatile("" : "+v"(v[u]));
+#pragma unroll
+            for (int u = 0; u < 8; u += 2) {
+                s0 += z0 + u < z_hi ? (double)v[u] : 0.0;
+                s1 += z0 + u + 1 < z_hi ? (double)v[u + 1] : 0.0;
+            }
+        }
+        fred[t] = s0 + s1;
+        __syncthreads();
+        if (wv == 0) __hip_atomic_store(ft.scratch + (size_t)bx * 64 + t, (fred[t] + fred[64 + t]) + (fred[128 + t] + fred[192 + t]), __ATOMIC_RELAXED, __HIP_MEMORY_SCOPE_AGENT);
+        __syncthreads();
+    }
+    if (t == 0) {
+        const int old = __hip_atomic_fetch_add(ft.ticket, 1, __ATOMIC_RELEASE, __HIP_MEMORY_SCOPE_AGENT);
+        last_s = old == ft.nblk - 1;
+        if (old == ft.nblk - 1) __hip_atomic_store(ft.ticket, 0, __ATOMIC_RELAXED, __HIP_MEMORY_SCOPE_AGENT);
+    }
+    __syncthreads();
+    if (!last_s) return;
+    __builtin_amdgcn_fence(__ATOMIC_ACQUIRE, "agent");
+    const int H = ft.H, F = ft.F;
+    if (t < H) {
+        const BNRaw raw = bn_raw_load_st(ft.bn1, t);
+        float mean, rstd;
+        bn_raw_mean_rstd(ft.bn1, raw, mean, rstd);
+        gs_s[t] = (double)(raw.g * rstd);
+        m1_s[t] = stripe_sum(ft.dsum, t, ft.bn1.ss) * ft.bn1.inv_n;
+        m2_s[t] = stripe_sum(ft.dprod, t, ft.bn1.ss) * ft.bn1.inv_n;
+    }
+    __syncthreads();
+    const int c = t % H, fp = t / H, nfp = 256 / H, ch = ((t >> 6) * 64 % H) >> 6;
+    auto total = [&](int first, int parts, int idx) {
+        double a = 0.0;
+        for (int p = 0; p < parts; ++p) a += __hip_atomic_load(ft.scratch + (size_t)(first + p * ng + (idx >> 6)) * 64 + (idx & 63), __ATOMIC_RELAXED, __HIP_MEMORY_SCOPE_AGENT);
+        return a;
+    };
+    auto pval = [&](int f) {
+        const int idx = f * H + c;
+        return gs_s[c] * (total(0, ft.pu, idx) - m1_s[c] * total(nbu, ft.pa, idx) - m2_s[c] * total(nbu + nba, ft.pa, idx));
+    };
+    const double cs = pval(F);
+    for (int f = fp; f < F; f += nfp) {
+        const double pv = pval(f), w = (double)ft.W[(size_t)f * H + c];
+        const float gv = (float)((double)ft.g0[f] * pv + (double)ft.b0[f] * cs);
+        grad[ft.o_w + f * H + c] = gv;
+        if (A.on) adam_update(A, ft.o_w + f * H + c, gv, adam_t, adam_lr);
+        double db = w * cs, dg = w * pv;
+#pragma unroll
+        for (int o = 1; o < 64; o <<= 1) { db += __shfl_xor(db, o, 64); dg += __shfl_xor(dg, o, 64); }
+        if ((t & 63) == 0) { wred[0][f][ch] = db; wred[1][f][ch] = dg; }
+    }
+    __syncthreads();
+    if (t < F) {
+        const float db = (float)(H > 64 ? wred[0][t][0] + wred[0][t][1] : wred[0][t][0]);
+        const float dg = (float)(H > 64 ? wred[1][t][0] + wred[1][t][1] : wred[1][t][0]);
+        grad[ft.o_b + t] = db; grad[ft.o_g + t] = dg;
+        if (A.on) { adam_update(A, ft.o_b + t, db, adam_t, adam_lr); adam_update(A, ft.o_g + t, dg, adam_t, adam_lr); }
+    }
+}
+
+static_assert(sizeof(FinishArgs) + sizeof(float*) <= 4096, "k_finish's arguments must fit the kernel-argument segment");
 __global__ void __launch_bounds__(256) k_finish(const FinishArgs fa, float* __restrict__ grad) {
     int task = 0;
     const int ntask = fa.nst + fa.nct + fa.nar;
@@ -64,6 +161,7 @@
     }
     if (fa.host_status && fa.status && blockIdx.x == 0 && threadIdx.x == 0)
         __hip_atomic_store(fa.host_status, fa.status[0] | fa.status[1], __ATOMIC_RELAXED, __HIP_MEMORY_SCOPE_SYSTEM);
+    if ((int)blockIdx.x < fa.fold.nblk) { finish_fold(fa.fold, grad, A, adam_t, adam_lr); return; }
     if (task < fa.nst) {
         const SlabTask t = fa.st[task];
         __shared__ float sred[256];
@@ -156,7 +254,7 @@
     int o_fc1_w[3], o_fc1_b[3], o_fc2_w[3], o_fc2_b[3];
     BNSlot bn[MAX_LAYERS + 9];
     int nbn;
-    int a_convb[MAX_LAYERS], a_cb, a_ob, a_dwn, a_dwe, a_db1, a_db2, a_sync, arena_n, bn_plane;
+    int a_convb[MAX_LAYERS], a_cb, a_ob, a_dwn, a_dwe, a_db1, a_db2, a_sync, a_fold, arena_n, bn_plane;
     char* ws; size_t ws_bytes;
     int64_t capN, capE, capB;
     float *h, *z, *zco, *hco, *anode, *pq, *att, *dis_unit, *dis_co, *pooled, *pcnt, *xco, *y1, *zl, *logp, *stats, *zpart;
@@ -164,6 +262,7 @@
     int ro_rows;
     int striped;
     int fold_zero;
+    int feat_fold;
     int bn0_dirty_host;
     int gwide;
     int ro_step;
@@ -227,6 +326,7 @@
     { const char* v = getenv("CAL_AMD_STRIPED"); e->striped = !(v && v[0] == '0'); }
     { const char* v = getenv("CAL_AMD_GWIDE"); e->gwide = !(v && v[0] == '0'); }
     { const char* v = getenv("CAL_AMD_FOLD_ZERO"); e->fold_zero = !(v && v[0] == '0'); }
+    { const char* v = getenv("CAL_AMD_FEAT_FOLD"); e->feat_fold = !(v && v[0] == '0'); }
     e->bn0_dirty_host = 1;
     {
         int dev = 0, cus = 0;
@@ -300,6 +400,7 @@
     e->a_db1 = a; a += 3 * H;
     e->a_db2 = a; a += (3 * C + 3) / 4 * 4;
     e->a_sync = a; a += (RBK_SYNC_INTS + 1) / 2 + 2;
+    e->a_fold = a; a += 2;
     a = (a + 3) / 4 * 4;
     const int a_bn = a;
     for (int i = 0; i < e->nbn; ++i) {
@@ -421,7 +522,7 @@
 enum class Conv { Node, Graph64, Graph128, Wide };
 enum class Att { Node, Graph, Wide };
 enum class FeatFwd { Gemm, Rows };
-enum class FeatBwd { Gemm, Rows, Units };
+enum class FeatBwd { Gemm, Rows, Units, Folded };
 enum class Readout { Gemm, FourKernel, OneLaunch, Rows };
 struct Route {
     Plan plan;
@@ -469,6 +570,7 @@
     FinishArgs fa;
     size_t slab_off;
     Deferred d_convb[MAX_LAYERS], d_gin_b1[MAX_LAYERS], d_cb, d_ob, d_dwn, d_dwe, d_bn0;
+    GconvFoldArgs fold;
 };
 
 BNRef bnref(const Ctx& c, int k, int rows, int update) {
@@ -692,7 +794,7 @@
     return 0;
 }
 
-int gconv_bwd(Ctx& c, Bwd& b, GconvBwdBranch* gb, int nb, float** dst, double** dsum, double** dprod, bool st) {
+int gconv_bwd(Ctx& c, Bwd& b, GconvBwdBranch* gb, int nb, float** dst, double** dsum, double** dprod, bool st, bool fold = false) {
     Engine* e = c.e;
     const bool co = nb == 2;
     const bool wide = (co ? c.r.co_bwd : c.r.bb_bwd) == Conv::Wide;
@@ -718,14 +820,20 @@
     }
     const CSR gd = csr_dst(c);
     const dim3 grid(B, nsl, nb);
-    if (co && lean && e->ntiles > 0) PROF_LAUNCH((k_gconv_bwd<true, 2, true, true>), grid, dim3(GB_NT), 0, c.st, gd, e->gptr, e->eptr, b2, e->loop_w, c.N, H, H, e->status);
-    else if (co && lean) PROF_LAUNCH((k_gconv_bwd<true, 2, false, true>), grid, dim3(GB_NT), 0, c.st, gd, e->gptr, e->eptr, b2, e->loop_w, c.N, H, H, e->status);
-    else if (co && e->ntiles > 0) PROF_LAUNCH((k_gconv_bwd<true, 2, true>), grid, dim3(GB_NT), 0, c.st, gd, e->gptr, e->eptr, b2, e->loop_w, c.N, H, H, e->status);
-    else if (co) PROF_LAUNCH((k_gconv_bwd<true, 2>), grid, dim3(GB_NT), 0, c.st, gd, e->gptr, e->eptr, b2, e->loop_w, c.N, H, H, e->status);
-    else if (gb[0].dout && lean) PROF_LAUNCH((k_gconv_bwd<false, 0, false, true>), grid, dim3(GB_NT), 0, c.st, gd, e->gptr, e->eptr, b2, e->loop_w, c.N, H, H, e->status);
-    else if (gb[0].dout) PROF_LAUNCH((k_gconv_bwd<false, 0>), grid, dim3(GB_NT), 0, c.st, gd, e->gptr, e->eptr, b2, e->loop_w, c.N, H, H, e->status);
-    else if (lean) PROF_LAUNCH((k_gconv_bwd<false, 1, false, true>), grid, dim3(GB_NT), 0, c.st, gd, e->gptr, e->eptr, b2, e->loop_w, c.N, H, H, e->status);
-    else PROF_LAUNCH((k_gconv_bwd<false, 1>), grid, dim3(GB_NT), 0, c.st, gd, e->gptr, e->eptr, b2, e->loop_w, c.N, H, H, e->status);
+    const GconvNoFold nf;
+    if (fold) {
+        PROF_LAUNCH((k_gconv_bwd<false, 1, false, false, true>), grid, dim3(GB_NT), 0, c.st, gd, e->gptr, e->eptr, b2, e->loop_w, c.N, H, H, e->status, b.fold);
+        CAL_CHECK_LAUNCH("k_gconv_bwd(fold)");
+        return 0;
+    }
+    if (co && lean && e->ntiles > 0) PROF_LAUNCH((k_gconv_bwd<true, 2, true, true>), grid, dim3(GB_NT), 0, c.st, gd, e->gptr, e->eptr, b2, e->loop_w, c.N, H, H, e->status, nf);
+    else if (co && lean) PROF_LAUNCH((k_gconv_bwd<true, 2, false, true>), grid, dim3(GB_NT), 0, c.st, gd, e->gptr, e->eptr, b2, e->loop_w, c.N, H, H, e->status, nf);
+    else if (co && e->ntiles > 0) PROF_LAUNCH((k_gconv_bwd<true, 2, true>), grid, dim3(GB_NT), 0, c.st, gd, e->gptr, e->eptr, b2, e->loop_w, c.N, H, H, e->status, nf);
+    else if (co) PROF_LAUNCH((k_gconv_bwd<true, 2>), grid, dim3(GB_NT), 0, c.st, gd, e->gptr, e->eptr, b2, e->loop_w, c.N, H, H, e->status, nf);
+    else if (gb[0].dout && lean) PROF_LAUNCH((k_gconv_bwd<false, 0, false, true>), grid, dim3(GB_NT), 0, c.st, gd, e->gptr, e->eptr, b2, e->loop_w, c.N, H, H, e->status, nf);
+    else if (gb[0].dout) PROF_LAUNCH((k_gconv_bwd<false, 0>), grid, dim3(GB_NT), 0, c.st, gd, e->gptr, e->eptr, b2, e->loop_w, c.N, H, H, e->status, nf);
+    else if (lean) PROF_LAUNCH((k_gconv_bwd<false, 1, false, true>), grid, dim3(GB_NT), 0, c.st, gd, e->gptr, e->eptr, b2, e->loop_w, c.N, H, H, e->status, nf);
+    else PROF_LAUNCH((k_gconv_bwd<false, 1>), grid, dim3(GB_NT), 0, c.st, gd, e->gptr, e->eptr, b2, e->loop_w, c.N, H, H, e->status, nf);
     CAL_CHECK_LAUNCH("k_gconv_bwd");
     return 0;
 }
@@ -875,9 +983,13 @@
     else r.feat_bwd = feat_rows && !gin ? FeatBwd::Rows : FeatBwd::Gemm;
     const bool st = e->striped && c.training;
     r.st_bb = st && r.bb_fwd == r.bb_bwd && r.bb_bwd != Conv::Node;
-    r.st_bb1 = r.st_bb && (gin || gw || r.feat_bwd == FeatBwd::Units);
+    if (e->feat_fold && r.feat_bwd == FeatBwd::Units && gcn && r.bb_bwd == Conv::Graph64 && L >= 2 && F + 1 <= GB_FF && (H == 64 || H == 128) &&
+        r.st_bb && !r.lean_bb)
+        r.feat_bwd = FeatBwd::Folded;
+    const bool units = r.feat_bwd == FeatBwd::Units || r.feat_bwd == FeatBwd::Folded;
+    r.st_bb1 = r.st_bb && (gin || gw || units);
     r.st_node = st && gcn && !gc && N > 0 && N < 16384;
-    r.st_feat = (r.st_bb && !gin && !gw && r.feat_bwd == FeatBwd::Units) || r.st_node;
+    r.st_feat = (r.st_bb && !gin && !gw && units) || r.st_node;
     r.st_co = gw ? st : st && ag && gcb && T <= 256;
     const int B4 = (B + 15) & ~15;
     const bool ro = !e->cat && (size_t)B4 * (H + 4) <= (size_t)RO_LDS && B * H <= 16384 && H % RO_CW == 0 && B4 <= 256 && H <= 256 &&
@@ -1565,6 +1677,30 @@
     return 0;
 }
 
+int feat_fold_task(Ctx& c, Bwd& b, const float* x0) {
+    Engine* e = c.e;
+    const int N = c.N, T = c.T, H = e->H, F = e->F, nsl = H / GC_N, n = GB_FF * H;
+    const size_t need = (size_t)(nsl + 2) * T * n;
+    if (b.slab_off + need > e->slab_floats) return no_slabs();
+    float* p = e->slabs + b.slab_off;
+    b.slab_off += need;
+    b.fold.x0 = x0; b.fold.bn0 = bnref(c, 0, N, 0); b.fold.F = F;
+    b.fold.U = p; b.fold.A = p + (size_t)nsl * T * n; b.fold.Bn = b.fold.A + (size_t)T * n;
+    FoldTask& ft = b.fa.fold;
+    ft.U = b.fold.U; ft.A = b.fold.A; ft.Bn = b.fold.Bn;
+    ft.SU = nsl * T; ft.SA = T; ft.n = n;
+    ft.pu = cdiv(ft.SU, 128); ft.pa = cdiv(ft.SA, 128);
+    ft.nblk = (n / 64) * (ft.pu + 2 * ft.pa);
+    ft.scratch = parts_alloc(c, (size_t)ft.nblk * 64);
+    if (!ft.scratch) return no_parts();
+    ft.ticket = reinterpret_cast<int*>(e->arena + e->a_fold);
+    ft.bn1 = bnref(c, 1, N, 0); ft.dsum = bn_dsum(c, 1); ft.dprod = bn_dprod(c, 1);
+    ft.W = e->P + e->o_feat_w; ft.g0 = e->P + e->bn[0].gamma; ft.b0 = e->P + e->bn[0].beta;
+    ft.o_w = e->o_feat_w; ft.o_g = e->bn[0].gamma; ft.o_b = e->bn[0].beta;
+    ft.F = F; ft.H = H;
+    return 0;
+}
+
 int bwd_backbone(Ctx& c, Bwd& b, const float* x0) {
     Engine* e = c.e;
     const Route& r = c.r;
@@ -1733,7 +1869,9 @@
             }
             float* dst[1] = {e->G + e->o_conv_w[i - 1]};
             double* dsum[1] = {bn_dsum(c, i)}; double* dprod[1] = {bn_dprod(c, i)};
-            { ProfScope ps(st, 4, 4.0 * N * H * H + 2.0 * (double)(E + N) * H, true); RC(gconv_bwd(c, b, &gb, 1, dst, dsum, dprod, st_i)); } STAGE();
+            const bool fold = i == 1 && r.feat_bwd == FeatBwd::Folded;
+            if (fold) RC(feat_fold_task(c, b, x0));
+            { ProfScope ps(st, 4, 4.0 * N * H * H + 2.0 * (double)(E + N) * H, true); RC(gconv_bwd(c, b, &gb, 1, dst, dsum, dprod, st_i, fold)); } STAGE();
             RC(flush_finals(c)); STAGE();
         }
         auto bn_bwd_dz = [&](const float* q0, const float* q1, Acc acc, bool st_rd) -> int {
@@ -1749,6 +1887,7 @@
         };
         if (r.bb_bwd != Conv::Node) {
             if (i > 1) continue;
+            if (r.feat_bwd == FeatBwd::Folded) continue;
             if (units) { RC(bwd_feat_units(c, b, x0, p0, two ? dzi : nullptr, false)); STAGE(); }
             else RC(bn_bwd_dz(p0, two ? dzi : nullptr, Acc(), r.st_bb1));
             continue;
@@ -1846,6 +1985,7 @@
     for (int k = 0; k < e->nbn; ++k) {
         const BNSlot& s = e->bn[k];
         const int wp = (s.width + 3) / 4 * 4;
+        if (k == 0 && fa.fold.nblk) continue;
         if (k == 0 && b.d_bn0.p) {
             commit_d(b.d_bn0, F, s.gamma, F, 1.f);
             commit_d(b.d_bn0, 0, s.beta, F, 1.f);
@@ -1883,6 +2023,11 @@
         std::vector<std::pair<int64_t, int64_t>> iv;
         for (int i = 0; i < fa.nst; ++i) iv.push_back({fa.st[i].dst - e->G, (fa.st[i].dst - e->G) + fa.st[i].n});
         for (int i = 0; i < fa.nct; ++i) iv.push_back({fa.ct[i].dst, (int64_t)fa.ct[i].dst + fa.ct[i].n});
+        if (fa.fold.nblk) {
+            iv.push_back({fa.fold.o_w, (int64_t)fa.fold.o_w + F * H});
+            iv.push_back({fa.fold.o_g, (int64_t)fa.fold.o_g + F});
+            iv.push_back({fa.fold.o_b, (int64_t)fa.fold.o_b + F});
+        }
         std::sort(iv.begin(), iv.end());
         int64_t pos = 0;
         bool ok = true;
@@ -1901,7 +2046,7 @@
             fa.adam.on = 0; fa.nar = 0; c.adam_in_finish = 2;
         }
     }
-    int nblk = 0;
+    int nblk = fa.fold.nblk;
     for (int i = 0; i < fa.nst; ++i) { fa.blk0[i] = nblk; nblk += std::max(1, cdiv(fa.st[i].n, 64)); }
     for (int i = 0; i < fa.nct; ++i) { fa.blk0[fa.nst + i] = nblk; nblk += std::max(1, cdiv(fa.ct[i].n, 16)); }
     for (int i = 0; i < fa.nar; ++i) { fa.blk0[fa.nst + fa.nct + i] = nblk; nblk += (int)cdiv(fa.ar[i].end - fa.ar[i].begin, 256); }
diff --git a/cal_amd/csrc/engine_gconv_bwd.hpp b/cal_amd/csrc/engine_gconv_bwd.hpp
--- a/cal_amd/csrc/engine_gconv_bwd.hpp
+++ b/cal_amd/csrc/engine_gconv_bwd.hpp
@@ -41,10 +41,23 @@
 
 struct GconvBwdBranch2 { GconvBwdBranch b[2]; };
 
-template <bool RS, int MODE, bool TILED = false, bool LEAN = false>
+constexpr int GB_FF = 16;
+constexpr int GB_LDA = 20;
+struct GconvFoldArgs {
+    const float* x0;
+    BNRef bn0;
+    int F;
+    float* U;
+    float* A; float* Bn;
+};
+struct GconvNoFold {};
+template <bool FOLD> struct GconvFoldSel { typedef GconvNoFold type; };
+template <> struct GconvFoldSel<true> { typedef GconvFoldArgs type; };
+
+template <bool RS, int MODE, bool TILED = false, bool LEAN = false, bool FOLD = false>
 __global__ void __launch_bounds__(GB_NT, (LEAN ? 4 : 1)) k_gconv_bwd(const CSR g, const int* __restrict__ gptr, const int* __restrict__ eptr,
                                                    const GconvBwdBranch2 bb, float loop_w, int N, int H,
-                                                   int K, int* __restrict__ status) {
+                                                   int K, int* __restrict__ status, const typename GconvFoldSel<FOLD>::type fo) {
     constexpr int LDX = LEAN ? GC_K : GB_LDX;
     __shared__ __attribute__((aligned(16))) float Ab[GB_T * GB_LDJ];
     __shared__ __attribute__((aligned(16))) float Ds[GB_T * GB_LDD];
@@ -63,10 +76,14 @@
     __shared__ unsigned char bg_s[TILED ? GB_T : 4];
     __shared__ int ee[(MODE == 2 && !LEAN) ? GB_E : 1];
     __shared__ unsigned char er[GB_E];
+    __shared__ float xa_s[FOLD ? GB_T * GB_LDA : 1];
+    __shared__ unsigned mk_s[FOLD ? GB_T * 4 : 1];
+    __shared__ float m0_s[FOLD ? GB_FF : 1], r0_s[FOLD ? GB_FF : 1];
     constexpr bool UP = MODE == 1, POOL = MODE == 2;
     static_assert(!TILED || MODE == 2, "only the POOL variant looks at the graphs inside a tile");
+    static_assert(!FOLD || (MODE == 1 && !RS && !LEAN), "the feature fold rides in the non-LEAN UP variant");
     BLK_CLK(0);
-    warm_kernargs<sizeof(CSR) + 2 * sizeof(void*) + sizeof(GconvBwdBranch2) + 32>();
+    warm_kernargs<sizeof(CSR) + 2 * sizeof(void*) + sizeof(GconvBwdBranch2) + 32 + (FOLD ? sizeof(GconvFoldArgs) : 0)>();
     const GconvBwdBranch& br = bb.b[blockIdx.z];
     const int b = blockIdx.x, sl = blockIdx.y, ns0 = sl * GC_N, t = threadIdx.x;
     const int g0 = gptr[b], rows = gptr[b + 1] - g0, e0 = eptr[b], ne = eptr[b + 1] - e0;
@@ -81,6 +98,13 @@
         if (!br.dacc_sum) for (int i = t; i < 2 * K; i += GB_NT) parts[i] = 0.0;
         if ((UP || POOL) && t < GC_N) br.bias_parts[(size_t)b * H + ns0 + t] = 0.0;
         for (int i = t; i < K * GC_N; i += GB_NT) slab[(size_t)(i / GC_N) * H + ns0 + i % GC_N] = 0.f;
+        if constexpr (FOLD) {
+            for (int i = t; i < GB_FF * K; i += GB_NT) {
+                fo.U[((size_t)sl * gridDim.x + b) * GB_FF * K + i] = 0.f;
+                if (sl == 0) fo.A[(size_t)b * GB_FF * K + i] = 0.f;
+                if (sl == (int)gridDim.y - 1) fo.Bn[(size_t)b * GB_FF * K + i] = 0.f;
+            }
+        }
         return;
     }
     const bool hasw = br.ew != nullptr;
@@ -138,8 +162,16 @@
         const int c = ns0 + (t & (GC_N - 1));
         ud1s = stripe_load(br.udot_sum, c, br.ubn.ss); ud2s = stripe_load(br.udot_prod, c, br.ubn.ss);
     }
+    float xr0[2] = {0.f, 0.f};
+    BNRaw raw0;
+    if constexpr (FOLD) {
+#pragma unroll
+        for (int u = 0; u < 2; ++u) xr0[u] = fo.x0[(size_t)g0 * fo.F + min(t + u * GB_NT, rows * fo.F - 1)];
+        raw0 = bn_raw_load(fo.bn0, min(t, fo.F - 1));
+    }
     bn_raws_pin(braws);
     if (UP) { stripe_pin(ud1s); stripe_pin(ud2s); }
+    if constexpr (FOLD) { bn_raw_pin(raw0); asm volatile("" : "+v"(xr0[0]), "+v"(xr0[1])); }
 #pragma unroll
     for (int u = 0; u < 2; ++u) asm volatile("" : "+v"(nv[u]), "+v"(ev[u]), "+v"(cin[u]));
     if (POOL && !TILED) { asm volatile("" : "+v"(gv), "+v"(gv1)); gv += br.gp1 ? gv1 : 0.f; }
@@ -167,6 +199,15 @@
         gam_s[t] = braw.g;
         bet_s[t] = braw.b;
     }
+    if constexpr (FOLD) {
+        if (t < GB_FF) {
+            float m1, r1;
+            bn_raw_mean_rstd(fo.bn0, raw0, m1, r1);
+            m0_s[t] = m1; r0_s[t] = r1;
+        }
+        for (int i = t; i < GB_T * GB_LDA; i += GB_NT) xa_s[i] = 0.f;
+        if (t < GB_T * 4) mk_s[t] = 0u;
+    }
     for (int i = t; i < (rowsP * GB_LDJ + 3) / 4; i += GB_NT) reinterpret_cast<float4*>(Ab)[i] = make_float4(0.f, 0.f, 0.f, 0.f);
     float cv[2];
     if (br.coef_in) {
@@ -209,12 +250,25 @@
         ro_commit<GB_NT>(bx, rows, K4, [&](int i, int k4, float4 v) {
             const float s = RS ? rs_s[i] : 1.f;
             const int k = 4 * k4;
+            if constexpr (FOLD) {
+                const unsigned m = (v.x > 0.f ? 1u : 0u) | (v.y > 0.f ? 2u : 0u) | (v.z > 0.f ? 4u : 0u) | (v.w > 0.f ? 8u : 0u);
+                atomicOr(&mk_s[i * 4 + (k >> 5)], m << (k & 31));
+            }
             v.x = (v.x * s - mean_s[k]) * rstd_s[k]; v.y = (v.y * s - mean_s[k + 1]) * rstd_s[k + 1];
             v.z = (v.z * s - mean_s[k + 2]) * rstd_s[k + 2]; v.w = (v.w * s - mean_s[k + 3]) * rstd_s[k + 3];
             *reinterpret_cast<float4*>(Xs + i * LDX + k) = v;
         });
     };
     if (!(POOL && LEAN)) commit_x();
+    if constexpr (FOLD) {
+        const int F = fo.F;
+#pragma unroll
+        for (int u = 0; u < 2; ++u) {
+            const int i = t + u * GB_NT;
+            if (i < rows * F) { const int f = i % F; xa_s[(i / F) * GB_LDA + f] = (xr0[u] - m0_s[f]) * r0_s[f]; }
+        }
+        if (t < rows) xa_s[t * GB_LDA + F] = 1.f;
+    }
     if (POOL) {
         float cs[4] = {0.f, 0.f, 0.f, 0.f};
 #pragma unroll
@@ -337,7 +391,7 @@
         if (R == 2) mma_rowk<true>(Ds + li * GB_LDD, Ds + (32 + li) * GB_LDD, wrow, GC_N, lk, acc[0], acc[1]);
         else mma_rowk<false>(Ds + li * GB_LDD, nullptr, wrow, GC_N, lk, acc[0], acc[1]);
         const int k = w * 32 + li;
-        float* dxp = sl ? br.dxp1 : br.dxp0;
+        [[maybe_unused]] float* dxp = sl ? br.dxp1 : br.dxp0;
         float xh[2][16];
 #pragma unroll
         for (int q = 0; q < 2; ++q)
@@ -358,8 +412,52 @@
                 f2[r & 3] = fmaf(v, xh[q][r], f2[r & 3]);
             }
         }
-        gc_store_tile<gc_site(WT_DXP)>(acc[0], dxp + (size_t)g0 * K + w * 32, K, rows, li, lk, MmaIdent(), (rows * K - w * 32) * 4);
-        if (R == 2) gc_store_tile<gc_site(WT_DXP)>(acc[1], dxp + (size_t)(g0 + 32) * K + w * 32, K, rows - 32, li, lk, MmaIdent(), ((rows - 32) * K - w * 32) * 4);
+        if constexpr (!FOLD) {
+            gc_store_tile<gc_site(WT_DXP)>(acc[0], dxp + (size_t)g0 * K + w * 32, K, rows, li, lk, MmaIdent(), (rows * K - w * 32) * 4);
+            if (R == 2) gc_store_tile<gc_site(WT_DXP)>(acc[1], dxp + (size_t)(g0 + 32) * K + w * 32, K, rows - 32, li, lk, MmaIdent(), ((rows - 32) * K - w * 32) * 4);
+        } else {
+            const bool do_a = sl == 0, do_bn = sl == (int)gridDim.y - 1;
+            float av[2][16];
+            unsigned mw[2][16];
+#pragma unroll
+            for (int q = 0; q < 2; ++q)
+#pragma unroll
+                for (int r = 0; r < 16; ++r) {
+                    const int i = mma_row(r, lk, q * 32);
+                    av[q][r] = xa_s[i * GB_LDA + (li & 15)];
+                    mw[q][r] = mk_s[i * 4 + w];
+                }
+            gc_f32x16 fu, fa, fb;
+#pragma unroll
+            for (int i = 0; i < 16; ++i) { fu[i] = 0.f; fa[i] = 0.f; fb[i] = 0.f; }
+#pragma unroll
+            for (int q = 0; q < 2; ++q) {
+                if (q < R) {
+#pragma unroll
+                    for (int r = 0; r < 16; ++r) {
+                        const bool on = (mw[q][r] >> li) & 1u;
+                        fu = __builtin_amdgcn_mfma_f32_32x32x2f32(av[q][r], on ? acc[q][r] : 0.f, fu, 0, 0, 0);
+                    }
+                    if (do_a) {
+#pragma unroll
+                        for (int r = 0; r < 16; ++r) {
+                            const bool on = (mw[q][r] >> li) & 1u;
+                            fa = __builtin_amdgcn_mfma_f32_32x32x2f32(av[q][r], on ? 1.f : 0.f, fa, 0, 0, 0);
+                        }
+                    }
+                    if (do_bn) {
+#pragma unroll
+                        for (int r = 0; r < 16; ++r) {
+                            const bool on = (mw[q][r] >> li) & 1u;
+                            fb = __builtin_amdgcn_mfma_f32_32x32x2f32(av[q][r], on ? xh[q][r] : 0.f, fb, 0, 0, 0);
+                        }
+                    }
+                }
+            }
+            gc_store_tile(fu, fo.U + ((size_t)sl * gridDim.x + b) * GB_FF * K + w * 32, K, GB_FF, li, lk);
+            if (do_a) gc_store_tile(fa, fo.A + (size_t)b * GB_FF * K + w * 32, K, GB_FF, li, lk);
+            if (do_bn) gc_store_tile(fb, fo.Bn + (size_t)b * GB_FF * K + w * 32, K, GB_FF, li, lk);
+        }
         double s1 = ((double)f1[0] + (double)f1[1]) + ((double)f1[2] + (double)f1[3]);
         double s2 = ((double)f2[0] + (double)f2[1]) + ((double)f2[2] + (double)f2[3]);
         s1 += __shfl_xor(s1, 32, 64);
```

New measurement: 572,900 graphs/s. 5.6% lower.
